# guangkun0818/speech2text

Measured on AMD Instinct MI355X. Metric: audio-seconds/sec (train step, zipformer pruned-RNN-T), higher is better.
Workload: dtype f32; 1 GPU; C3 zipformer pruned-RNN-T train step: chunk_size -1, 500 BPE, prune_range 5 (fbank+fwd+bwd+allreduce+ScaledAdam); accumulate_grad_batches=1, gemm_arith=bf16x2/3, per_gpu_batch=64, global_batch=64, labels_per_utt=50, parallelism=dp1

## Files before the change

### include/s2t_mi355.h

```cpp
#ifndef S2T_MI355_H_
#define S2T_MI355_H_

#ifdef __cplusplus
extern "C" {
#endif

int s2t_fbank_f32(const float* pcm, long pcm_stride, const long* num_samples, int batch,
                  const float* window400, const float* twiddle512, const int* mel_off,
                  const int* mel_k0, const float* mel_w, int nnz, int num_mel, float eps,
                  float scale_in, const float* cmvn_mean, const float* cmvn_istd, float* out,
                  int max_frames, long* out_frames, void* stream);

#define S2T_CTC_MAX_LABELS 1023
long s2t_ctc_workspace_floats(int B, int T, int Umax);
int s2t_ctc_loss_fwd_bwd(const float* logits, const long* targets, long tgt_stride,
                         const long* in_len, const long* tgt_len, int B, int T, int V, int Umax,
                         int blank, int zero_infinity, const float* grad_scale, float* workspace,
                         float* loss_per_utt, float* grad_logits, void* stream);

int s2t_fill_f32(float* p, long n, float v, void* stream);
int s2t_rnnt_row_exp(const float* x, long rows, int C, float* probs, float* rowmax, void* stream);
int s2t_rnnt_simple_pxpy(const float* am, const float* lm, const float* am_max,
                         const float* lm_max, const float* nrm, const long* symbols,
                         const long* boundary, int B, int S, int T, int C, int blank, float* px,
                         float* py, void* stream);
int s2t_rnnt_simple_w(const float* dpx, const float* dpy, const float* nrm, const float* gscale,
                      int B, int S, int T, float* W, void* stream);
int s2t_rnnt_simple_bwd(const float* am_probs, const float* lm_probs, const float* G_am,
                        const float* G_lm, const float* dpx, const float* dpy,
                        const float* gscale, const long* symbols, int B, int S, int T, int C,
                        int blank, float* d_am, float* d_lm, int accumulate, void* stream);
#define S2T_RNNT_SMOOTH_LM_SLAB 64
#define S2T_RNNT_SMOOTH_AM_SLAB 32
#define S2T_RNNT_SMOOTH_MAX_C 2048
int s2t_rnnt_smooth_stats(const float* am_probs, const float* lm_probs, int B, int S, int T, int C,
                          float mu, float* lm_sum, float* u_part, float* u, float* log_u,
                          float* am_dot, void* stream);
int s2t_rnnt_smooth_pxpy(const float* am, const float* lm, const float* am_max,
                         const float* lm_max, const float* nrm, const float* lm_sum,
                         const float* am_dot, const float* log_u, const long* symbols,
                         const long* boundary, int B, int S, int T, int C, int blank, float lam,
                         float mu, float* px, float* py, void* stream);
int s2t_rnnt_smooth_bwd(const float* am_probs, const float* lm_probs, const float* G_am,
                        const float* G_lm, const float* dpx, const float* dpy,
                        const float* gscale, const long* symbols, const float* lm_sum,
                        const float* am_dot, const float* u, int B, int S, int T, int C, int blank,
                        float lam, float mu, float* dlogu_part, float* v, float* d_am, float* d_lm,
                        void* stream);
#define S2T_RNNT_REGULAR 0
#define S2T_RNNT_MODIFIED 1
#define S2T_RNNT_CONSTRAINED 2
int s2t_mutual_info_fwd(const float* px, const float* py, const long* boundary, int B, int S,
                        int T, int rnnt_type, float* p, float* ans, void* stream);
int s2t_mutual_info_bwd(const float* px, const float* py, const long* boundary, const float* p,
                        const float* ans_grad, int B, int S, int T, int rnnt_type, float* px_grad,
                        float* py_grad, void* stream);
int s2t_rnnt_prune_ranges(const float* px_grad, const float* py_grad, const long* boundary, int B,
                          int S, int T, int s_range, long* ranges, void* stream);
int s2t_rnnt_pruned_fwd(const float* am, const float* lm, const long* ranges,
                        const long* symbols, const long* boundary, int B, int S, int T, int C,
                        int R, int blank, int act, int rnnt_type, float delay_penalty, float* px,
                        float* py, float* lse, void* stream);
int s2t_rnnt_pruned_bwd(const float* am, const float* lm, const long* ranges,
                        const long* symbols, const float* lse, const float* dpx, const float* dpy,
                        const float* gscale, int B, int S, int T, int C, int R, int blank, int act,
                        int rnnt_type, float* d_am, float* d_lm, int accumulate, void* stream);
int s2t_rnnt_lattice_fwd(const float* logits, const long* ranges, const long* symbols,
                         const long* boundary, int B, int S, int T, int V, int R, int blank,
                         int rnnt_type, float delay_penalty, float* px, float* py, float* lse,
                         void* stream);
int s2t_rnnt_lattice_bwd(const float* logits, const long* ranges, const long* symbols,
                         const float* lse, const float* dpx, const float* dpy,
                         const float* gscale, int B, int S, int T, int V, int R, int blank,
                         int rnnt_type, float* d_logits, void* stream);


int s2t_swoosh_fwd(const float* x, float* y, long n, float offset, float constant, void* stream);
int s2t_swoosh_bwd(const float* x, const float* g, float* d, long n, float offset, void* stream);
int s2t_biasnorm_fwd(const float* x, const float* bias, const float* log_scale, long rows, int D,
                     float* y, float* scales, void* stream);
int s2t_biasnorm_fwd_tb(const float* x, const float* bias, const float* log_scale, int T, int B, int D,
                        float* y, float* scales, void* stream);
int s2t_biasnorm_bwd_tb(const float* x, const float* bias, const float* scales, const float* g, int T,
                        int B, int D, float* dx, float* dbias, float* dls, void* stream);
int s2t_norm_bypass_fwd(const float* x, const float* bias, const float* log_scale, const float* orig,
                        const float* bypass_scale, const float* fm, int B, long rows, int D, float* out,
                        float* scales, void* stream);
int s2t_norm_bypass_bwd(const float* x, const float* bias, const float* scales, const float* orig,
                        const float* bypass_scale, const float* g, const float* fm, int B, long rows, int D,
                        float* dx, float* d_orig, float* d_bypass_scale, float* dbias, float* dls,
                        void* stream);
int s2t_biasnorm_bwd(const float* x, const float* bias, const float* scales, const float* g,
                     long rows, int D, float* dx, float* dbias, float* dls, void* stream);
long s2t_balancer_bwd_workspace_floats(void);
int s2t_balancer_bwd(const float* x, long ldx, const float* g, long ldg, long rows, int C,
                     float min_mean, float max_mean, float min_rms, float max_rms,
                     float grad_scale, float* out, long ldo, float* workspace, int parity,
                     float act_off, void* stream);
int s2t_balancer_stats(const float* x, long ldx, long rows, int C, float* stats, void* stream);
int s2t_balancer_apply(const float* x, long ldx, const float* g, long ldg, long rows, int C,
                       float min_mean, float max_mean, float min_rms, float max_rms,
                       float grad_scale, float* out, long ldo, const float* stats, float act_off,
                       void* stream);


int s2t_zipconv_fwd(const float* u, long ld, int gate_off, const unsigned char* mask, int T, int B,
                    int C, int K, int chunk, const float* wc, const float* bc, const float* wk,
                    const float* bk, const float* scale, float* y, void* stream);
int s2t_zipconv_fwd_act(const float* u, long ld, int gate_off, const unsigned char* mask, int T, int B,
                        int C, int K, int chunk, const float* wc, const float* bc, const float* wk,
                        const float* bk, const float* scale, float* y, float* y_act, int act_kind,
                        void* stream);
int s2t_zipconv_bwd(const float* u, long ld, int gate_off, const unsigned char* mask, int T, int B,
                    int C, int K, int chunk, const float* wc, const float* wk, const float* bk,
                    const float* scale, const float* dy, float* du, float* dwc, float* dbc,
                    float* dwk, float* dbk, float* dscale, float* workspace, void* stream);
int s2t_zipconv_bwd_data(const float* u, long ld, int gate_off, const unsigned char* mask, int T,
                         int B, int C, int K, int chunk, const float* wc, const float* wk,
                         const float* bk, const float* scale, const float* dy, float* du,
                         void* stream);
int s2t_zipconv_bwd_params(const float* u, long ld, int gate_off, const unsigned char* mask, int T,
                           int B, int C, int K, int chunk, const float* wc, const float* wk,
                           const float* bk, const float* scale, const float* dy, float* dwc,
                           float* dbc, float* dwk, float* dbk, float* dscale, float* workspace,
                           void* stream);
long s2t_zipconv_bwd_workspace_floats(int T, int B, int C, int K);


int s2t_relpos_attn_fwd(const float* qkp, const float* pos, const unsigned char* kpm,
                        const unsigned char* amask, int T, int B, int H, int qd, int pd, float* W,
                        void* stream);
int s2t_relpos_attn_fwd_flag(const float* qkp, const float* pos, const unsigned char* kpm,
                             const unsigned char* amask, int T, int B, int H, int qd, int pd,
                             float* W, float pen_limit, float* pen_flag, void* stream);
int s2t_relpos_attn_bwd(const float* qkp, const float* pos, const unsigned char* kpm,
                        const unsigned char* amask, int T, int B, int H, int qd, int pd,
                        const float* W, const float* dW, const float* dW0, const float* dO1,
                        const float* V1, int dv1, const float* dO2, const float* V2, int dv2,
                        int delta_given, float* delta_ws, float* dqkp, float* dpos,
                        float* workspace, void* stream);
long s2t_relpos_attn_bwd_workspace_floats(int T, int B, int H, int pd);
int s2t_attn_apply(const float* W, const float* v, int T, int B, int H, int dv, int transpose,
                   float* out, void* stream);


long s2t_linear_wgrad_workspace_floats(int R, int N, int M);
int s2t_linear_wgrad(const float* g, long ldg, const float* a, long lda, int R, int N, int M,
                     float* dW, float* db, int accumulate, float* workspace, void* stream);

int s2t_whiten_metric(float* xtx, float* colsum, long n, int G, int cg, float* cov, float* mean,
                      float* scal, float* host_metric, float* workspace, void* stream);
int s2t_whiten_prep(const float* cov, const float* mean, const float* scal, int G, int cg, float* dcov,
                    float* bias, float* sums64, void* stream);
int s2t_gemm_x3p_sq(const float* A, long lda, const unsigned short* Bp, int N, int K, float* C, long ldc,
                    int M, const float* bias, const float* other, long ld_other, float* sums, int tile,
                    void* stream);
int s2t_sumsq64(const float* g, long numel, float* sums64, void* stream);
int s2t_whiten_combine64(const float* g, const float* pg, long numel, float grad_scale,
                         const float* sums64, float* out, void* stream);
int s2t_whiten_dcov(const float* cov, const float* mean, const float* scal, int G, int cg,
                    float* dcov, float* bias, float* sums, void* stream);
int s2t_whiten_apply(const float* g, const float* pg, long numel, float grad_scale, float* sums,
                     float* out, void* stream);
int s2t_limit_param_grad(const float* x, const float* g, float lo, float hi, long n, float* out,
                         void* stream);

int s2t_bestrq_labels(const float* feats, int B, int T, int F, const float* proj, int D,
                      const float* codebooks, int ncb, int K, int T2, long* labels, void* stream);


int s2t_col2im3x3_nhwc(const float* dc, int B, int H, int W, int C, int Ho, int Wo, int sh, int sw,
                       float* dx, void* stream);

int s2t_conv3x3_c1(int mode, const float* x, const float* w, const float* bias, const float* g, int B,
                   int H, int W, int pw, int CO, float* y, float* dw, float* db, float* dx,
                   void* stream);

int s2t_conv3x3_s2(int mode, const float* x, const float* w, const float* bias, const float* g, int B,
                   int H, int W, int CI, int CO, float* y, float* dx, void* stream);

int s2t_conv3x3_gemm(int mode, const float* x, int B, int H, int W, int C, int sh, int sw, int CO,
                     const float* w2_or_g, const float* bias, float* out, float* db, void* stream);

int s2t_dwconv2d_nhwc_fwd(const float* x, const float* wgt, const float* bias, int N, int H, int W,
                          int C, int KH, int KW, int flip, float* y, void* stream);
int s2t_dwconv2d_nhwc_fwd_add(const float* x, const float* wgt, const float* bias, const float* add,
                              int N, int H, int W, int C, int KH, int KW, int flip, float* y,
                              void* stream);
long s2t_dwconv2d_wgrad_workspace_floats(int N, int H, int C, int KH, int KW);
int s2t_dwconv2d_nhwc_wgrad(const float* x, const float* dy, int N, int H, int W, int C, int KH,
                            int KW, float* workspace, float* dw, float* db, void* stream);

int s2t_optim_chunk_elems(void);
int s2t_optim_segc_floats(void);
int s2t_seg_stats(const float* p, const float* g, const int* chunk_off, const int* chunk_len,
                  int nchunks, float* partial, void* stream);
int s2t_scaled_adam_coef(const float* partial, const int* seg_chunk_begin, const int* seg_len,
                         int nchunks_all, int seg_lo, int seg_hi, float lr, float beta1,
                         float beta2, float eps, float scalar_lr_scale, float param_min_rms,
                         float param_max_rms, float scalar_max, float clip_val,
                         float clipping_scale, int step, int size_update_period,
                         int clipping_update_period, float bc2, float bc2_size, float beta2c,
                         float* param_rms, float* scale_exp_avg_sq, float* scale_grads,
                         float* model_norms, float* fstate, int* istate, float* segstat,
                         float* segc, const float* skip, void* stream);
int s2t_scaled_adam_apply(float* p, float* g, float* delta, float* exp_avg_sq,
                          const int* chunk_off, const int* chunk_len, const int* chunk_seg,
                          int nchunks, const float* segc, int zero_grad, void* stream);

int s2t_gemm_f32(int mode, const float* A, long lda, const float* B, long ldb, float* C, long ldc,
                 int M, int N, int K, const float* bias, const float* resid, long ldr,
                 const float* act_src, long lds, int act_kind, int pro_a, int pro_b, float* colsum,
                 int accumulate, void* stream);

int s2t_gemm_f32_batched(int mode, const float* A, long lda, long sA, const float* B, long ldb, long sB,
                         float* C, long ldc, long sC, int M, int N, int K, int batch, void* stream);

int s2t_gemm_f32_sq(int mode, const float* A, long lda, const float* B, long ldb, float* C, long ldc,
                    int M, int N, int K, const float* bias, const float* other, long ld_other,
                    float* sums, void* stream);
int s2t_whiten_combine(const float* g, const float* pg, long numel, float grad_scale, const float* sums,
                       float* out, void* stream);

int s2t_gemm_f32_tiled(int mode, const float* A, long lda, const float* B, long ldb, float* C,
                       long ldc, int M, int N, int K, const float* bias, const float* resid,
                       long ldr, int tile, void* stream);

int s2t_tn_x3(int set);
int s2t_tn_w(int set);
int s2t_nn_x3(int set);

int s2t_gemm_xtx(const float* x, long ldx, int R, int C, int cg, float* xtx, long ldc,
                 float* colsum, void* stream);

typedef struct S2tTnProblem {
  const float* A;
  long lda;
  const float* B;
  long ldb;
  float* C;
  long ldc;
  int M, N, K;
  float* colsum;
  float alpha;
// ... 16 lines not shown
                              long* tokens, long* out_len, void* stream);

long s2t_rnnt_beam_workspace_bytes(int B, int T, int V, int beam_size);
int s2t_rnnt_beam_stateless(const float* am, const long* lengths, const float* emb,
                            const float* conv_w, const float* lin_w, const float* lin_b,
                            const float* pre_w, const float* pre_b, int B, int T, int V, int E,
                            int D, int ctx, int act, int blank, int beam_size, int cutoff_top_k,
                            void* workspace, long* tokens, long* frames, long* out_len,
                            float* score, void* stream);

long s2t_rnnt_stream_state_bytes(int B, int V, int ctx, int beam_size, int max_tokens);
int s2t_rnnt_stream_reset(void* state, const int* rows, int B, int V, int ctx, int beam_size,
                          int max_tokens, int blank, void* stream);
int s2t_rnnt_greedy_stateless_chunk(const float* am, const long* chunk_len, const float* emb,
                                    const float* conv_w, const float* lin_w, const float* lin_b,
                                    const float* pre_w, const float* pre_b, int B, int Tc, int V,
                                    int E, int D, int ctx, int act, int max_token_step,
                                    int max_tokens, int blank, void* state, long* tokens,
                                    long* out_len, int* overflow, void* stream);
int s2t_rnnt_beam_stateless_chunk(const float* am, const long* chunk_len, const float* emb,
                                  const float* conv_w, const float* lin_w, const float* lin_b,
                                  const float* pre_w, const float* pre_b, int B, int Tc, int V, int E,
                                  int D, int ctx, int act, int blank, int beam_size,
                                  int cutoff_top_k, int max_tokens, void* state, long* tokens,
                                  long* frames, long* out_len, float* score, long* stable_len,
                                  int* overflow, void* stream);

#define S2T_RNNT_LSTM_MAX_HIDDEN 1024
#define S2T_RNNT_LSTM_MAX_LAYERS 8
#define S2T_RNNT_LSTM_MAX_VOCAB 8192
#define S2T_RNNT_LSTM_MAX_BEAM 16
typedef struct S2tLstmLayer {
  const float* x2g_w;
  const float* x2g_b;
  const float* p2g_w;
  const float *g_gamma, *g_beta;
  const float *c_gamma, *c_beta;
} S2tLstmLayer;
typedef struct S2tRnntLstmDesc {
  int V, E, H, D, inner, num_layers, layer_norm, act;
  float in_eps, lstm_eps, out_eps;
  int pad_;
  const float* emb;
  const float *in_gamma, *in_beta;
  S2tLstmLayer layers[S2T_RNNT_LSTM_MAX_LAYERS];
  const float *lin_w, *lin_b;
  const float *out_gamma, *out_beta;
  const float *pre_w, *pre_b;
  const float *out1_w, *out1_b;
  const float *out2_w, *out2_b;
} S2tRnntLstmDesc;
long s2t_rnnt_lstm_workspace_bytes(const S2tRnntLstmDesc* desc, int B, int T, int beam_size);
int s2t_lstm_pred_step(const S2tRnntLstmDesc* desc, int R, const int* tokens, const int* emit,
                       const int* parent, const float* h_in, const float* c_in, const float* lm_in,
                       float* h_out, float* c_out, float* lm_out, void* workspace, void* stream);
int s2t_rnnt_greedy_lstm(const S2tRnntLstmDesc* desc, const float* am, const long* lengths, int B,
                         int T, int max_token_step, void* workspace, long* tokens, long* out_len,
                         void* stream);
int s2t_rnnt_beam_lstm(const S2tRnntLstmDesc* desc, const float* am, const long* lengths, int B,
                       int T, int beam_size, int cutoff_top_k, void* workspace, long* tokens,
                       long* frames, long* out_len, float* score, void* stream);

typedef struct S2tRnnLmDesc {
  int V, E, H, num_layers;
  const float* emb;
  S2tLstmLayer layers[S2T_RNNT_LSTM_MAX_LAYERS];
  const float *out_w, *out_b;
} S2tRnnLmDesc;
long s2t_rnn_lm_step_workspace_bytes(const S2tRnnLmDesc* lm, int R);
int s2t_rnn_lm_step(const S2tRnnLmDesc* lm, int R, const int* tokens, const int* emit,
                    const int* parent, const float* h_in, const float* c_in, const float* q_in,
                    float* h_out, float* c_out, float* q_out, void* workspace, void* stream);
long s2t_rnnt_beam_lstm_lm_workspace_bytes(const S2tRnntLstmDesc* desc, const S2tRnnLmDesc* lm, int B,
                                           int T, int beam_size);
int s2t_rnnt_beam_lstm_lm(const S2tRnntLstmDesc* desc, const S2tRnnLmDesc* lm, const float* am,
                          const long* lengths, int B, int T, int beam_size, int cutoff_top_k,
                          float lm_weight, int lm_start_token, void* workspace, long* tokens,
                          long* frames, long* out_len, float* score, float* lm_score, void* stream);

long s2t_rnnt_lstm_stream_state_bytes(const S2tRnntLstmDesc* desc, int B, int beam_size,
                                      int max_tokens);
long s2t_rnnt_lstm_stream_workspace_bytes(const S2tRnntLstmDesc* desc, int B, int Tc, int beam_size);
int s2t_rnnt_lstm_stream_reset(const S2tRnntLstmDesc* desc, void* state, const int* rows, int B,
                               int beam_size, int max_tokens, void* workspace, void* stream);
int s2t_rnnt_greedy_lstm_chunk(const S2tRnntLstmDesc* desc, const float* am, const long* chunk_len,
                               int B, int Tc, int max_token_step, int max_tokens, int host_poll,
                               void* state, void* workspace, long* tokens, long* out_len,
                               int* overflow, void* stream);
int s2t_rnnt_beam_lstm_chunk(const S2tRnntLstmDesc* desc, const float* am, const long* chunk_len,
                             int B, int Tc, int beam_size, int cutoff_top_k, int max_tokens,
                             void* state, void* workspace, long* tokens, long* frames,
                             long* out_len, float* score, long* stable_len, int* overflow,
                             void* stream);

int s2t_row_energy(const float* x, long stride, const long* len, int B, int D, int mode, float* out,
                   void* stream);
int s2t_mix(const float* src, long sstride, const long* slen, const float* noise, long nstride,
            const long* nlen, const long* start, const float* snr, const float* src_e,
            const float* noise_e, int B, long rows_max, int D, int mode, float max_gain_db,
            float* out, void* stream);
int s2t_specaug(float* feats, int B, int T, int F, const int* tspan, int nt, const int* fspan,
                int nf, void* stream);
int s2t_pad_rows(const float* packed, const long* offsets, int B, long Lmax, int D, float* out,
                 void* stream);

int s2t_linear_lt(int mode, const float* X, long ldx, const float* W, long ldw, const float* bias,
                  const float* C, long ldc, float beta, float* D, long ldd, int M, int N, int K,
                  void* workspace, long ws_bytes, void* stream);
int s2t_linear_lt_stats(int* plans, int* timed);
long s2t_linear_lt_own_calls(void);

int s2t_bypass_fwd(const float* orig, const float* src, const float* scale, long rows, int C,
                   float* out, void* stream);
int s2t_bypass_bwd(const float* orig, const float* src, const float* scale, const float* g,
                   long rows, int C, float* d_orig, float* d_src, float* d_scale, void* stream);
int s2t_bypass_bwd_acc(const float* orig, const float* src, const float* scale, const float* g,
                       const float* acc_in, long rows, int C, float* d_orig, float* d_src,
                       float* d_scale, void* stream);
int s2t_attn_delta_pairs(const float* W, const float* dW0, const float* dO1, const float* O1,
                         int dv1, const float* dO2, const float* O2, int dv2, int T, int B, int H,
                         float* delta, void* stream);
int s2t_bypass_fwd_mask(const float* orig, const float* src, const float* scale, const float* fm,
                        int B, long rows, int C, float* out, void* stream);
int s2t_bypass_bwd_mask(const float* orig, const float* src, const float* scale, const float* g,
                        const float* fm, int B, long rows, int C, float* d_orig, float* d_src,
                        float* d_scale, void* stream);
int s2t_downsample_fwd(const float* src, const float* w, int ds, int T, int B, int C, float* out,
                       void* stream);
int s2t_downsample_bwd(const float* src, const float* w, const float* g, int ds, int T, int B, int C,
                       float* d_src, float* dw, void* stream);
int s2t_downsample_fwd_bt(const float* src, const float* w, int ds, int T, int B, int C, float* out,
                          void* stream);
int s2t_downsample_bwd_bt(const float* src, const float* w, const float* g, int ds, int T, int B, int C,
                          float* d_src, float* dw, void* stream);
int s2t_bypass_up_fwd(const float* orig, const float* src, const float* scale, int up, int T, int B,
                      int C, float* out, void* stream);
int s2t_bypass_up_bwd(const float* orig, const float* src, const float* scale, const float* g, int up,
                      int T, int B, int C, float* d_orig, float* d_src, float* d_scale, void* stream);
typedef struct S2tCommit {
  const float* x;
  float* d;
  float* grad;
  float lo, hi;
  int limit;
  long n;
} S2tCommit;
int s2t_param_grad_commit_n(int n, const S2tCommit* items, void* stream);
int s2t_nonlin_gate_fwd(const float* u, int T, int B, int C, float* xs, void* stream);
int s2t_nonlin_out_fwd(const float* z, const float* u, int T, int B, int C, float* o, void* stream);
int s2t_nonlin_out_bwd(const float* g, const float* z, const float* u, int T, int B, int C, float* dz,
                       float* du, void* stream);
int s2t_nonlin_gate_bwd(const float* dxs, const float* u, int T, int B, int C, float* du,
                        void* stream);

int s2t_layernorm_fwd(const float* x, const float* y, float alpha, const float* gamma,
                      const float* beta, long rows, int C, float eps, float* xsum, float* out,
                      float* stats, void* stream);
typedef struct S2tLnFold {
  const float* partial;
  long rows;
  float* dgamma;
  float* dbeta;
} S2tLnFold;
long s2t_layernorm_bwd_partial_floats(long rows, int C);
int s2t_layernorm_bwd(const float* x, const float* stats, const float* gamma, const float* dy,
                      const float* resid, long rows, int C, float* dx, float* partial,
                      void* stream);
int s2t_layernorm_param_grad(int n, const S2tLnFold* items, int C, void* stream);
int s2t_silu_fwd(const float* h, long n, float* a, void* stream);
int s2t_silu_bwd(const float* h, const float* da, long n, float scale, float* dh, void* stream);
int s2t_dropout_add(const float* x, const float* y, long n, float alpha, float p,
                    unsigned long long seed, float* out, void* stream);
int s2t_silu_drop_fwd(const float* h, long n, float p, unsigned long long seed, float* a,
                      void* stream);
int s2t_silu_drop_bwd(const float* h, const float* da, long n, float scale, float p,
                      unsigned long long seed, float* dh, void* stream);
#define S2T_BN_PARTIALS 128
long s2t_bn_workspace_floats(int C);
int s2t_bn_silu_fwd(const float* x, const float* gamma, const float* beta, float eps,
                    float momentum, float* running_mean, float* running_var, long* num_batches,
                    long rows, int C, float* y, float* save_mean, float* save_rstd,
                    float* workspace, void* stream);
int s2t_bn_silu_apply(const float* x, const float* mean, const float* rstd, const float* gamma,
                      const float* beta, long rows, int C, float* y, void* stream);
int s2t_bn_silu_bwd(const float* x, const float* ds, const float* save_mean,
                    const float* save_rstd, const float* gamma, const float* beta, long rows, int C,
                    float* dx, float* dgamma, float* dbeta, float* workspace, void* stream);
int s2t_mhsa_fwd(const float* qkv, long ld, int qoff, int koff, int voff, const long* lens, int T,
                 int B, int H, int dh, float scale, float dropout_p, unsigned long seed, float* o,
                 long ldo, float* lse, void* stream);
int s2t_mhsa_bwd(const float* qkv, long ld, int qoff, int koff, int voff, const long* lens, int T,
                 int B, int H, int dh, float scale, float dropout_p, unsigned long seed,
                 const float* o, const float* d_o, long ldo, const float* lse, float* delta,
                 float* dqkv, void* stream);

long s2t_conv1_relu_workspace_floats(int C);
int s2t_conv1_relu_fwd(const float* x, const float* w, const float* bias, int B, int T, int F,
                       int C, float* out, void* stream);
int s2t_conv1_relu_wgrad(const float* x, const float* w, const float* bias, const float* d_out,
                         int B, int T, int F, int C, float* dw, float* db, float* workspace,
                         void* stream);

#define S2T_ADAM_MAX_GROUPS 8
typedef struct S2tAdamGroup {
  int chunk_hi;
  float lr, beta1, beta2, eps, weight_decay;
  float bias_correction1;
  float sqrt_bias_correction2;
  int decoupled;
} S2tAdamGroup;
int s2t_clip_coef(const float* partial, int nchunks, float clip_val, float* out, void* stream);
int s2t_adam_apply(float* p, float* g, float* exp_avg, float* exp_avg_sq, const int* chunk_off,
                   const int* chunk_len, int nchunks, int ngroups, const S2tAdamGroup* groups,
                   const float* coef, int zero_grad, const float* skip, void* stream);

int s2t_lnlstm_fwd(const float* gx, const float* wp_t, const float* g_gamma, const float* g_beta,
                   const float* c_gamma, const float* c_beta, const float* h0, const float* c0,
                   int T, int B, int H, float eps, float* hs, float* ghat, float* chat,
                   float* rstd, float* hT, float* cT, void* stream);
int s2t_lnlstm_bwd(const float* wp, const float* g_gamma, const float* g_beta,
                   const float* c_gamma, const float* c_beta, const float* c0, int T, int B, int H,
                   const float* ghat, const float* chat, const float* rstd, const float* dhs,
                   float* dgx, float* d_g_gamma, float* d_g_beta, float* d_c_gamma,
                   float* d_c_beta, void* stream);

int s2t_lstm_seq_fwd(const float* gx, const float* whh, const float* h0, const float* c0, int T,
                     int B, int H, float* hs, float* gates, float* cells, float* hT, float* cT,
                     void* stream);
int s2t_lstm_seq_bwd(const float* whh_t, const float* c0, int T, int B, int H, const float* gates,
                     const float* cells, const float* dhs, float* dgx, float* dc_ws, void* stream);

int s2t_predictor_ctx_fwd(const int* tokens, const float* emb, const float* w, int B, int L, int K,
                          int D, int V, float* out, void* stream);
int s2t_predictor_ctx_bwd(const int* tokens, const float* emb, const float* w, const float* g, int B,
                          int L, int K, int D, int V, float* d_emb, float* d_w, void* stream);

int s2t_gemm_arith(void);
int s2t_gemm_arith_of(int cls);
int s2t_gemm_class_set(int cls);
int s2t_gemm_arith_set(int arith);
typedef struct {
  long src_off;
  long dst_off;
  int N, K, ld, transposed;
  unsigned blk_begin;
  int pad_;
} S2tPlaneDesc;
long s2t_x3p_plane_elems(int N, int K);
long s2t_x3p_split_blocks(int N, int K);
int s2t_x3p_split(const float* base, const void* tab, int n, int total_blocks, unsigned short* dst,
                  void* stream);
int s2t_gemm_x3p(const float* A, long lda, const unsigned short* Bp, int N, int K, float* C, long ldc,
                 int M, const float* bias, const float* resid, long ldr, const float* act_src,
                 long ld_act, int act_kind, float* C2, long ldc2, int act2, const float* resid_b,
                 long ldrb, int tile, void* stream);
#define S2T_X3P_BAL_COEF_READY (1 << 20)
int s2t_balancer_coef(float* bal_stats, int N, long rows, float min_mean, float max_mean, float min_rms,
                      float max_rms, float grad_scale, void* stream);
int s2t_gemm_x3p_bal(const float* A, long lda, const unsigned short* Bp, int N, int K, float* C, long ldc,
                     int M, const float* resid, long ldr, const float* act_src, long ld_act, int act_kind,
                     int tile, float* bal_stats, float min_mean, float max_mean, float min_rms,
                     float max_rms, float grad_scale, void* stream);

typedef struct S2tRowMap {
  int hw, w;
  long sb, sh, sw, base;
} S2tRowMap;
int s2t_gemm_x3p_map(const float* A, const S2tRowMap* amap, int seg, int nseg, const long* segoff,
                     const unsigned short* Bp, int N, float* C, long ldc, const S2tRowMap* cmap,
                     long c_elems, int M, const float* bias, int tile, void* stream);

void* s2t_side_stream(void);
int s2t_stream_order(void* from, void* to);

int s2t_x3p_sample_begin(int every);
int s2t_x3p_sample_end(long* launches, double* total_ms, double* bytes, double* flops);
int s2t_x3p_sample_min_bytes(double* bytes_min);
long s2t_gemm_x3p_calls(void);
long s2t_linear_lt_calls(void);
int s2t_prof_pair_create(void** start, void** stop);
int s2t_prof_pair_arm(void* start, void* stop);
int s2t_prof_pair_consumed(void);
int s2t_prof_pair_ms(void* start, void* stop, float* ms);
int s2t_prof_pair_destroy(void* start, void* stop);


int s2t_add_f32(const float* a, const float* b, float* out, long n, void* stream);
int s2t_balancer_next_parity(void);

int s2t_bmm_lt(int mode, const float* A, const float* B, float* C, int batch, int M, int N, int K,
               void* workspace, long ws_bytes, void* stream);

#define S2T_ZL_NDEC 32
#define S2T_ZL_NWHITEN 11
typedef struct S2tZlLin {
  const float* w;
  const float* b;
  float* gw;
  float* gb;
  const unsigned short* pf;
  const unsigned short* pb;
  int N, K;
} S2tZlLin;
typedef struct S2tZlBal {
  float min_mean, max_mean, min_rms, max_rms, grad_scale;
} S2tZlBal;
// ... 104 lines not shown
```

### speech2text_amd/csrc/common.h

```cpp
#pragma once
#include <hip/hip_runtime.h>
#include <stdint.h>

extern thread_local hipEvent_t s2t_prof_start, s2t_prof_stop;

#include <stdio.h>
#include <stdlib.h>
#include <string.h>
static inline int s2t_debug_env(const char* name) {
  const char* e = getenv(name);
  if (!e || atoi(e) == 0) return 0;
  const char* gate = getenv("S2T_DEBUG_KERNELS");
  if (gate && strcmp(gate, "1") == 0) return atoi(e);
  fprintf(stderr, "[s2t] %s=%s ignored: ablation switches need S2T_DEBUG_KERNELS=1\n", name, e);
  return 0;
}

#define S2T_GEMM_ARITH_DEFAULT 2
#define S2T_GEMM_ARITH_DEFAULT_F 2
#define S2T_GEMM_ARITH_DEFAULT_D 2
#define S2T_GEMM_ARITH_DEFAULT_W 2
#define S2T_GEMM_ARITH_DEFAULT_S 3
extern "C" int s2t_gemm_arith(void);
extern "C" int s2t_gemm_arith_of(int cls);
extern "C" int s2t_gemm_class_set(int cls);
struct S2tGemmClass {
  int prev;
  explicit S2tGemmClass(int cls) : prev(s2t_gemm_class_set(cls)) {}
  ~S2tGemmClass() { s2t_gemm_class_set(prev); }
};

#define S2T_WAVE 64
#define S2T_NEG_INF (-__builtin_huge_valf())

#define S2T_CHECK_LAUNCH()                         \
  do {                                             \
    hipError_t e__ = hipGetLastError();            \
    if (e__ != hipSuccess) return (int)e__;        \
  } while (0)

__device__ __forceinline__ float wave_sum(float v) {
#pragma unroll
  for (int o = 32; o > 0; o >>= 1) v += __shfl_xor(v, o, 64);
  return v;
}
__device__ __forceinline__ float wave_max(float v) {
#pragma unroll
  for (int o = 32; o > 0; o >>= 1) v = fmaxf(v, __shfl_xor(v, o, 64));
  return v;
}
__device__ __forceinline__ double wave_sum_d(double v) {
#pragma unroll
  for (int o = 32; o > 0; o >>= 1) v += __shfl_xor(v, o, 64);
  return v;
}

__device__ __forceinline__ float log_add(float a, float b) {
  float m = fmaxf(a, b);
  if (m == S2T_NEG_INF) return S2T_NEG_INF;
  float d = fminf(a, b) - m;
  return m + log1pf(__expf(d));
}
__device__ __forceinline__ float log_add_precise(float a, float b) {
  float m = fmaxf(a, b);
  if (m == S2T_NEG_INF) return S2T_NEG_INF;
  float d = fminf(a, b) - m;
  return m + log1pf(expf(d));
}

__device__ __forceinline__ float log_add_comp(float a, float b) {
  const float m = fmaxf(a, b);
  if (m == S2T_NEG_INF) return S2T_NEG_INF;
  const float e = __expf(fminf(a, b) - m);
  const float u = 1.f + e;
  return m + (u == 1.f ? e : __logf(u) * __fdividef(e, u - 1.f));
}

__device__ __forceinline__ float block_sum(float v, float* scratch) {
  v = wave_sum(v);
  const int w = threadIdx.x >> 6, l = threadIdx.x & 63, nw = (blockDim.x + 63) >> 6;
  __syncthreads();
  if (l == 0) scratch[w] = v;
  __syncthreads();
  float r = 0.f;
  for (int i = 0; i < nw; ++i) r += scratch[i];
  return r;
}
__device__ __forceinline__ float block_max(float v, float* scratch) {
  v = wave_max(v);
  const int w = threadIdx.x >> 6, l = threadIdx.x & 63, nw = (blockDim.x + 63) >> 6;
  __syncthreads();
  if (l == 0) scratch[w] = v;
  __syncthreads();
  float r = S2T_NEG_INF;
  for (int i = 0; i < nw; ++i) r = fmaxf(r, scratch[i]);
  return r;
}
```

### speech2text_amd/csrc/gemm_x3p.hip

```cpp
#include "common.h"
#include "../../include/s2t_mi355.h"
#include <hip/hip_ext.h>
#include <algorithm>
#include <cstdint>
#include <cstdlib>
#include <utility>
#include <vector>

namespace {

typedef float f32x16 __attribute__((ext_vector_type(16)));
typedef float f32x2 __attribute__((ext_vector_type(2)));
typedef __bf16 bf16x2 __attribute__((ext_vector_type(2)));
typedef __bf16 bf16x8 __attribute__((ext_vector_type(8)));
typedef float f32x4 __attribute__((ext_vector_type(4)));
typedef unsigned u32x4 __attribute__((ext_vector_type(4)));
typedef const __attribute__((address_space(1))) float* gf32p;
typedef const __attribute__((address_space(1))) f32x4* gf32x4p;
typedef const __attribute__((address_space(1))) u32x4* gu32x4p;

__device__ __forceinline__ void split_pair(float x0, float x1, unsigned& p0, unsigned& p1,
                                           unsigned& p2) {
  f32x2 x = {x0, x1};
  p0 = __builtin_bit_cast(unsigned, __builtin_convertvector(x, bf16x2));
  f32x2 h = {__uint_as_float(p0 << 16), __uint_as_float(p0 & 0xFFFF0000u)};
  x = x - h;
  p1 = __builtin_bit_cast(unsigned, __builtin_convertvector(x, bf16x2));
  f32x2 h1 = {__uint_as_float(p1 << 16), __uint_as_float(p1 & 0xFFFF0000u)};
  x = x - h1;
  p2 = __builtin_bit_cast(unsigned, __builtin_convertvector(x, bf16x2));
}
__device__ __forceinline__ void split8(const f32x4 v0, const f32x4 v1, u32x4& q0, u32x4& q1,
                                       u32x4& q2) {
  unsigned a0, a1, a2, b0, b1, b2, c0, c1, c2, d0, d1, d2;
  split_pair(v0.x, v0.y, a0, a1, a2);
  split_pair(v0.z, v0.w, b0, b1, b2);
  split_pair(v1.x, v1.y, c0, c1, c2);
  split_pair(v1.z, v1.w, d0, d1, d2);
  q0 = u32x4{a0, b0, c0, d0};
  q1 = u32x4{a1, b1, c1, d1};
  q2 = u32x4{a2, b2, c2, d2};
}

__device__ __forceinline__ void split_pair2(float x0, float x1, unsigned& p0, unsigned& p1) {
  f32x2 x = {x0, x1};
  p0 = __builtin_bit_cast(unsigned, __builtin_convertvector(x, bf16x2));
  f32x2 h = {__uint_as_float(p0 << 16), __uint_as_float(p0 & 0xFFFF0000u)};
  x = x - h;
  p1 = __builtin_bit_cast(unsigned, __builtin_convertvector(x, bf16x2));
}
template <int NP>
__device__ __forceinline__ void split8n(const f32x4 v0, const f32x4 v1, u32x4 (&q)[3]) {
  if (NP == 3) {
    split8(v0, v1, q[0], q[1], q[2]);
  } else {
    unsigned a0, a1, b0, b1, c0, c1, d0, d1;
    split_pair2(v0.x, v0.y, a0, a1);
    split_pair2(v0.z, v0.w, b0, b1);
    split_pair2(v1.x, v1.y, c0, c1);
    split_pair2(v1.z, v1.w, d0, d1);
    q[0] = u32x4{a0, b0, c0, d0};
    q[1] = u32x4{a1, b1, c1, d1};
  }
}

enum { ACT_NONE = 0, ACT_SWOOSH_L = 1, ACT_SWOOSH_R = 2 };

__device__ __forceinline__ float log1p_fast(float e) {
  const float u = 1.f + e;
  return u == 1.f ? e : __logf(u) * __fdividef(e, u - 1.f);
}
__device__ __forceinline__ float swoosh(float x, int kind) {
  const float off = kind == ACT_SWOOSH_L ? 4.f : 1.f;
  const float c = kind == ACT_SWOOSH_L ? 0.035f : 0.313261687f;
  const float z = x - off;
  return fmaxf(z, 0.f) + log1p_fast(__expf(-fabsf(z))) - 0.08f * x - c;
}
__device__ __forceinline__ float swoosh_deriv(float x, int kind) {
  const float off = kind == ACT_SWOOSH_L ? 4.f : 1.f;
  return __fdividef(1.f, 1.f + __expf(off - x)) - 0.08f;
}

struct X3PMap {
  int on, hw, w;
  long sb, sh, sw, base;
};
__device__ __forceinline__ long x3p_maprow(const X3PMap& m, int r) {
  const int b = r / m.hw, q = r - b * m.hw, i = q / m.w, j = q - i * m.w;
  return m.base + b * m.sb + i * m.sh + j * m.sw;
}

struct X3P {
  const float* A;
  long lda;
  const unsigned short* Bp;
  int NT, KB;
  float* C;
  long ldc;
  int M, N, K;
  const float* bias;
  const float* op[2];
  long ldop[2];
  int role[2];
  int act_kind;
  float* C2;
  long ldc2;
  int act2;
  int tiles_m, tiles_n;
  int wgs_per_cu;
  int prio;
  const float* bal_stats;
  float bal_n, bal_min_mean, bal_max_mean, bal_min_rms, bal_max_rms, bal_gs;
  float* sq_sums;
  float sq_pad_;
  X3PMap amap, cmap;
  int seg16, nseg;
  long segoff[4];
  long c_elems;
};

__device__ __forceinline__ void x3p_set_prio(int on) {
  if (!on) return;
  if (on == 2) { __builtin_amdgcn_s_setprio(3); return; }
  const unsigned tg = __builtin_amdgcn_s_getreg(((4 - 1) << 11) | (16 << 6) | 4) & 15u;
  if (tg == 0) __builtin_amdgcn_s_setprio(3);
  else if (tg == 1) __builtin_amdgcn_s_setprio(2);
  else if (tg == 2) __builtin_amdgcn_s_setprio(1);
}

struct EpiOps {
  f32x4 v[2][2];
};
struct EpiRs {
  __amdgpu_buffer_rsrc_t c, c2, op[2];
};
constexpr unsigned kOob = 0xFFFFFFF0u;

__device__ __forceinline__ __amdgpu_buffer_rsrc_t x3p_rsrc(const float* p, long ld, int rows) {
  return __builtin_amdgcn_make_buffer_rsrc(const_cast<float*>(p), 0,
                                           p ? (int)((long)rows * ld * 4) : 0, 0x00020000);
}
__device__ __forceinline__ EpiRs x3p_epi_rsrc(const X3P& g) {
  EpiRs r;
  r.c = x3p_rsrc(g.C, g.ldc, g.M);
  r.c2 = x3p_rsrc(g.C2, g.ldc2, g.M);
  r.op[0] = x3p_rsrc(g.op[0], g.ldop[0], g.M);
  r.op[1] = x3p_rsrc(g.op[1], g.ldop[1], g.M);
  return r;
}
__device__ __forceinline__ f32x4 x3p_bload(__amdgpu_buffer_rsrc_t rs, unsigned off) {
  return __builtin_bit_cast(f32x4, __builtin_amdgcn_raw_buffer_load_b128(rs, off, 0, 0));
}
__device__ __forceinline__ void x3p_bstore(__amdgpu_buffer_rsrc_t rs, unsigned off, f32x4 v) {
  __builtin_amdgcn_raw_buffer_store_b128(__builtin_bit_cast(u32x4, v), rs, off, 0, 0);
}

__device__ __forceinline__ f32x4 x3p_epi_bias(const X3P& g, int j, int n0, int wcb, int lane) {
  const int col = n0 + 32 * (wcb + j) + (lane & 7) * 4;
  f32x4 b = {0.f, 0.f, 0.f, 0.f};
  if (g.bias && col < g.N) b = *reinterpret_cast<const f32x4*>(g.bias + col);
  return b;
}

__device__ __forceinline__ void x3p_epi_load(const X3P& g, const EpiRs& rs, EpiOps& o, int i, int j,
                                             int h, int m0, int n0, int wrb, int wcb, int lane) {
  const int er = lane >> 3, ec = (lane & 7) * 4;
  const int col = n0 + 32 * (wcb + j) + ec;
  const f32x4 z = {0.f, 0.f, 0.f, 0.f};
#pragma unroll
  for (int q = 0; q < 2; ++q) {
    const int row = m0 + 32 * (wrb + i) + 16 * h + er + 8 * q;
    const bool ok = row < g.M && col < g.N;
#pragma unroll
    for (int k = 0; k < 2; ++k) {
      o.v[q][k] = z;
      if (g.role[k])
        o.v[q][k] = x3p_bload(rs.op[k], ok ? (unsigned)(row * (int)g.ldop[k] + col) * 4u : kOob);
    }
  }
}

struct BalQ {
  f32x4 a, b;
};
__device__ __forceinline__ BalQ x3p_epi_balcoef(const X3P& g, int j, int n0, int wcb, int lane) {
  BalQ r;
  r.a = r.b = f32x4{0.f, 0.f, 0.f, 0.f};
  const int col = n0 + 32 * (wcb + j) + (lane & 7) * 4;
  if (col >= g.N) return r;
  r.a = *reinterpret_cast<const f32x4*>(g.bal_stats + 2048 + col);
  r.b = *reinterpret_cast<const f32x4*>(g.bal_stats + 3072 + col);
  return r;
}

__global__ __launch_bounds__(256) void bal_coef_kernel(const float* __restrict__ stats, float* __restrict__ coef,
                                                        int N, float n, float min_mean, float max_mean,
                                                        float min_rms, float max_rms, float gs) {
  const int c = blockIdx.x * 256 + threadIdx.x;
  if (c >= N) return;
  const float inv_n = 1.f / n;
  const float mean = stats[c] * inv_n, uvar = stats[1024 + c] * inv_n;
  const float raw_var = uvar - mean * mean;
  const bool live_v = raw_var > 1.0e-20f, live_r = uvar > 1.0e-20f;
  const float var = fmaxf(raw_var, 1.0e-20f);
  const float sd = sqrtf(var);
  const float rms = sqrtf(fmaxf(uvar, 1.0e-20f));
  const float m = mean / sd;
  const float mc = fminf(fmaxf(m, min_mean), max_mean);
  const float s_m = (m > mc) ? 1.f : ((m < mc) ? -1.f : 0.f);
  const float rc = fminf(fmaxf(rms, min_rms), max_rms);
  const float lq = logf(rc / rms);
  const float s_r = (lq > 0.f) ? -1.f : ((lq < 0.f) ? 1.f : 0.f);
  const float a = s_m * inv_n * (live_v ? (1.f / sd + mean * mean / (sd * var)) : 1.f / sd);
  const float b = (live_v ? -s_m * inv_n * mean / (sd * var) : 0.f) + (live_r ? s_r * inv_n / (rms * rms) : 0.f);
  const float lg_rms = fmaxf(sqrtf(fmaxf(a * a + 2.f * a * b * mean + b * b * uvar, 0.f)), 1.0e-20f);
  const float k = gs / lg_rms;
  coef[c] = a * k;
  coef[1024 + c] = b * k;
}

template <bool BAL = false>
__device__ __forceinline__ void x3p_epi_xform(const X3P& g, f32x16& a, float* scr, const EpiOps& o,
                                              const f32x4 bq, int h, int lane, const BalQ& bal = BalQ{}) {
  const int hi = lane >> 5, lo = lane & 31;
  const int er = lane >> 3, ec = (lane & 7) * 4;
#pragma unroll
  for (int r = 0; r < 8; ++r) scr[((r & 3) + 8 * (r >> 2) + 4 * hi) * 36 + lo] = a[8 * h + r];
  __builtin_amdgcn_fence(__ATOMIC_RELEASE, "workgroup", "local");
  __builtin_amdgcn_wave_barrier();
#pragma unroll
  for (int q = 0; q < 2; ++q) {
    f32x4 v = *reinterpret_cast<const f32x4*>(scr + (er + 8 * q) * 36 + ec);
    v += bq;
#pragma unroll
    for (int k = 0; k < 2; ++k) {
      const f32x4 x = o.v[q][k];
      if (g.role[k] == 1) {
        v.x *= swoosh_deriv(x.x, g.act_kind);
        v.y *= swoosh_deriv(x.y, g.act_kind);
        v.z *= swoosh_deriv(x.z, g.act_kind);
        v.w *= swoosh_deriv(x.w, g.act_kind);
        if (BAL) {
          v.x += fabsf(v.x) * fmaf(bal.b.x, x.x, bal.a.x);
          v.y += fabsf(v.y) * fmaf(bal.b.y, x.y, bal.a.y);
          v.z += fabsf(v.z) * fmaf(bal.b.z, x.z, bal.a.z);
          v.w += fabsf(v.w) * fmaf(bal.b.w, x.w, bal.a.w);
        }
      } else if (g.role[k] == 2 || (g.role[k] == 3 && g.act2 != 3)) {
        v += x;
      }
    }
    a[8 * h + 4 * q + 0] = v.x;
    a[8 * h + 4 * q + 1] = v.y;
    a[8 * h + 4 * q + 2] = v.z;
    a[8 * h + 4 * q + 3] = v.w;
  }
  __builtin_amdgcn_fence(__ATOMIC_RELEASE, "workgroup", "local");
  __builtin_amdgcn_wave_barrier();
}

struct EpiSq {
  float o = 0.f, c = 0.f;
};
template <bool CMAP = false>
__device__ __forceinline__ void x3p_epi_store(const X3P& g, const EpiRs& rs, const f32x16& a,
                                              const EpiOps& o, int i, int j, int h, int m0, int n0,
                                              int wrb, int wcb, int lane, EpiSq& sq) {
  const int er = lane >> 3, ec = (lane & 7) * 4;
  const int col = n0 + 32 * (wcb + j) + ec;
#pragma unroll
  for (int q = 0; q < 2; ++q) {
    const int row = m0 + 32 * (wrb + i) + 16 * h + er + 8 * q;
    const bool ok = row < g.M && col < g.N;
    const f32x4 v = {a[8 * h + 4 * q], a[8 * h + 4 * q + 1], a[8 * h + 4 * q + 2], a[8 * h + 4 * q + 3]};
    if (CMAP) {
      x3p_bstore(rs.c, ok ? (unsigned)(x3p_maprow(g.cmap, min(row, g.M - 1)) + col) * 4u : kOob, v);
      continue;
    }
    x3p_bstore(rs.c, ok ? (unsigned)(row * (int)g.ldc + col) * 4u : kOob, v);
    if (g.sq_sums && ok) {
      sq.c += (v.x * v.x + v.y * v.y) + (v.z * v.z + v.w * v.w);
      const f32x4 t = g.role[0] == 4 ? o.v[q][0] : o.v[q][1];
      sq.o += (t.x * t.x + t.y * t.y) + (t.z * t.z + t.w * t.w);
    }
    if (g.act2 == 3) {
      const f32x4 u = v + (g.role[0] == 3 ? o.v[q][0] : o.v[q][1]);
      x3p_bstore(rs.c2, ok ? (unsigned)(row * (int)g.ldc2 + col) * 4u : kOob, u);
    } else if (g.act2) {
      const f32x4 u = {swoosh(v.x, g.act2), swoosh(v.y, g.act2), swoosh(v.z, g.act2), swoosh(v.w, g.act2)};
      x3p_bstore(rs.c2, ok ? (unsigned)(row * (int)g.ldc2 + col) * 4u : kOob, u);
    }
  }
}

template <int TM, int TN, bool LEAN = false, bool BAL = false, bool CMAP = false>
__device__ __forceinline__ void x3p_epilogue(const X3P& g, f32x16 (&acc)[TM][TN], unsigned char* smem,
                                             int m0, int n0, int wrb, int wcb, int wave, int lane,
                                             bool sync = true) {
  if (sync) __syncthreads();
  float* scr = reinterpret_cast<float*>(smem) + wave * (16 * 36);
  EpiRs rs = x3p_epi_rsrc(g);
  if (CMAP) rs.c = __builtin_amdgcn_make_buffer_rsrc(g.C, 0, (int)(g.c_elems * 4), 0x00020000);
  EpiSq sq;
  auto sq_commit = [&]() {
    if (!g.sq_sums) return;
    const float so = wave_sum(sq.o), sc = wave_sum(sq.c);
    if (lane == 0) {
      const int slot = (blockIdx.x * 4 + wave) & 63;
      atomicAdd(g.sq_sums + slot, so);
      atomicAdd(g.sq_sums + 64 + slot, sc);
    }
  };
  if (LEAN) {
#pragma unroll
    for (int j = 0; j < TN; ++j) {
      const f32x4 bqj = x3p_epi_bias(g, j, n0, wcb, lane);
      const BalQ balj = BAL ? x3p_epi_balcoef(g, j, n0, wcb, lane) : BalQ{};
#pragma unroll
      for (int i = 0; i < TM; ++i)
#pragma unroll
        for (int h = 0; h < 2; ++h) {
          EpiOps o;
          x3p_epi_load(g, rs, o, i, j, h, m0, n0, wrb, wcb, lane);
          x3p_epi_xform<BAL>(g, acc[i][j], scr, o, bqj, h, lane, balj);
          x3p_epi_store<CMAP>(g, rs, acc[i][j], o, i, j, h, m0, n0, wrb, wcb, lane, sq);
        }
    }
    sq_commit();
    return;
  }
  f32x4 bq[TN];
#pragma unroll
  for (int j = 0; j < TN; ++j) bq[j] = x3p_epi_bias(g, j, n0, wcb, lane);
#pragma unroll
  for (int i = 0; i < TM; ++i) {
    EpiOps ops[2 * TN];
#pragma unroll
    for (int t = 0; t < 2 * TN; ++t) x3p_epi_load(g, rs, ops[t], i, t / 2, t & 1, m0, n0, wrb, wcb, lane);
#pragma unroll
    for (int t = 0; t < 2 * TN; ++t) x3p_epi_xform(g, acc[i][t / 2], scr, ops[t], bq[t / 2], t & 1, lane);
#pragma unroll
    for (int t = 0; t < 2 * TN; ++t)
      x3p_epi_store(g, rs, acc[i][t / 2], ops[t], i, t / 2, t & 1, m0, n0, wrb, wcb, lane, sq);
    __builtin_amdgcn_sched_barrier(0);
  }
  sq_commit();
}

template <int TM, int TN, bool BAL = false, int NP = 3>
__global__ __launch_bounds__(256, TM * TN == 4 ? 2 : (TM * TN == 2 ? 3 : 4))
void x3p_db_kernel(X3P g) {
  constexpr int BM = 64 * TM, BN = 64 * TN;
  constexpr int A_ST = 2 * TM * NP * 1024, B_ST = 2 * TN * NP * 1024, ST = A_ST + B_ST;
  constexpr int NAU = (128 * TM + 255) / 256;
  constexpr int NBP = 2 * TN * NP * 64;
  constexpr int NBU = (NBP + 255) / 256;
  constexpr int SCR = 4 * 16 * 36 * 4;
  __shared__ __attribute__((aligned(1024))) unsigned char smem[2 * ST > SCR ? 2 * ST : SCR];

  const int total = g.tiles_m * g.tiles_n;
  const int per_xcd = (total + 7) / 8;
  const int xcd = blockIdx.x & 7, stride = gridDim.x >> 3;
  int loc = blockIdx.x >> 3;
  if (loc >= per_xcd || xcd * per_xcd + loc >= total) return;
  const int tid = threadIdx.x, lane = tid & 63, wave = tid >> 6;
  const int wrb = (wave >> 1) * TM, wcb = (wave & 1) * TN;
  x3p_set_prio(g.prio);

  int a_r[NAU], a_k[NAU];
  unsigned a_dst[NAU];
  bool a_on[NAU];
// ... 781 lines not shown
```

### speech2text_amd/csrc/zip_elem.hip

```cpp
#include "common.h"
#include <algorithm>
#include <stdlib.h>

namespace {

__device__ __forceinline__ float log1p_fast(float e) {
  const float u = 1.f + e;
  return u == 1.f ? e : __logf(u) * __fdividef(e, u - 1.f);
}

__device__ __forceinline__ float swoosh_f(float x, float off, float c) {
  const float z = x - off;
  return fmaxf(z, 0.f) + log1p_fast(__expf(-fabsf(z))) - 0.08f * x - c;
}
__device__ __forceinline__ float swoosh_d(float x, float off) {
  return __fdividef(1.f, 1.f + __expf(off - x)) - 0.08f;
}

__global__ __launch_bounds__(256) void swoosh_fwd_kernel(const float* __restrict__ x,
                                                         float* __restrict__ y, long n, float off,
                                                         float c) {
  const long n4 = n >> 2;
  const long stride = (long)gridDim.x * blockDim.x;
  const float4* x4 = reinterpret_cast<const float4*>(x);
  float4* y4 = reinterpret_cast<float4*>(y);
  for (long i = (long)blockIdx.x * blockDim.x + threadIdx.x; i < n4; i += stride) {
    float4 v = x4[i];
    v.x = swoosh_f(v.x, off, c);
    v.y = swoosh_f(v.y, off, c);
    v.z = swoosh_f(v.z, off, c);
    v.w = swoosh_f(v.w, off, c);
    y4[i] = v;
  }
  for (long i = (n4 << 2) + (long)blockIdx.x * blockDim.x + threadIdx.x; i < n; i += stride)
    y[i] = swoosh_f(x[i], off, c);
}

__global__ __launch_bounds__(256) void swoosh_bwd_kernel(const float* __restrict__ x,
                                                         const float* __restrict__ g,
                                                         float* __restrict__ d, long n,
                                                         float off) {
  const long n4 = n >> 2;
  const long stride = (long)gridDim.x * blockDim.x;
  const float4* x4 = reinterpret_cast<const float4*>(x);
  const float4* g4 = reinterpret_cast<const float4*>(g);
  float4* d4 = reinterpret_cast<float4*>(d);
  for (long i = (long)blockIdx.x * blockDim.x + threadIdx.x; i < n4; i += stride) {
    const float4 v = x4[i], gg = g4[i];
    float4 o;
    o.x = gg.x * swoosh_d(v.x, off);
    o.y = gg.y * swoosh_d(v.y, off);
    o.z = gg.z * swoosh_d(v.z, off);
    o.w = gg.w * swoosh_d(v.w, off);
    d4[i] = o;
  }
  for (long i = (n4 << 2) + (long)blockIdx.x * blockDim.x + threadIdx.x; i < n; i += stride)
    d[i] = g[i] * swoosh_d(x[i], off);
}

__global__ __launch_bounds__(256) void biasnorm_fwd_kernel(
    const float* __restrict__ x, const float* __restrict__ bias, const float* __restrict__ ls,
    long rows, int D, float* __restrict__ y, float* __restrict__ scales, int tbT, int tbB) {
  const long row = (long)blockIdx.x * 4 + (threadIdx.x >> 6);
  const int lane = threadIdx.x & 63;
  if (row >= rows) return;
  const float* xr = x + row * D;
  float acc = 0.f;
  for (int c = lane; c < D; c += 64) {
    const float d = xr[c] - bias[c];
    acc = fmaf(d, d, acc);
  }
  acc = wave_sum(acc);
  const float s = rsqrtf(acc / D) * expf(ls[0]);
  if (lane == 0) scales[row] = s;
  const long orow = tbT > 0 ? (row % tbT) * tbB + row / tbT : row;
  float* yr = y + orow * D;
  for (int c = lane; c < D; c += 64) yr[c] = xr[c] * s;
}

template <int CPL>
__global__ __launch_bounds__(256) void biasnorm_bwd_kernel(
    const float* __restrict__ x, const float* __restrict__ bias, const float* __restrict__ scales,
    const float* __restrict__ g, long rows, int D, float* __restrict__ dx,
    float* __restrict__ dbias, float* __restrict__ dls, int tbT, int tbB) {
  const int lane = threadIdx.x & 63;
  const long wave = (long)blockIdx.x * 4 + (threadIdx.x >> 6);
  const long nwaves = (long)gridDim.x * 4;
  float b[CPL], db[CPL];
#pragma unroll
  for (int j = 0; j < CPL; ++j) {
    const int c = lane + 64 * j;
    b[j] = c < D ? bias[c] : 0.f;
    db[j] = 0.f;
  }
  float dl = 0.f;
  for (long row = wave; row < rows; row += 2 * nwaves) {
    const long row2 = row + nwaves;
    const bool has2 = row2 < rows;
    const long rowb = has2 ? row2 : row;
    const float* xr = x + row * D;
    const float* gr = g + (tbT > 0 ? (row % tbT) * tbB + row / tbT : row) * D;
    const float* xr2 = x + rowb * D;
    const float* gr2 = g + (tbT > 0 ? (rowb % tbT) * tbB + rowb / tbT : rowb) * D;
    float xv[CPL], gv[CPL], xw[CPL], gw[CPL];
#pragma unroll
    for (int j = 0; j < CPL; ++j) {
      const int c = lane + 64 * j;
      xv[j] = c < D ? xr[c] : 0.f;
      gv[j] = c < D ? gr[c] : 0.f;
      xw[j] = c < D ? xr2[c] : 0.f;
      gw[j] = c < D ? gr2[c] : 0.f;
    }
    float A = 0.f, ss = 0.f, A2 = 0.f, ss2 = 0.f;
#pragma unroll
    for (int j = 0; j < CPL; ++j) {
      const int c = lane + 64 * j;
      A = fmaf(gv[j], xv[j], A);
      A2 = fmaf(gw[j], xw[j], A2);
      const float d = c < D ? xv[j] - b[j] : 0.f, d2 = c < D ? xw[j] - b[j] : 0.f;
      ss = fmaf(d, d, ss);
      ss2 = fmaf(d2, d2, ss2);
    }
    A = wave_sum(A);
    ss = wave_sum(ss);
    A2 = wave_sum(A2);
    ss2 = wave_sum(ss2);
    const float s = scales[row], s2 = has2 ? scales[row2] : 0.f;
    const float coef = s * A / ss, coef2 = has2 ? s2 * A2 / ss2 : 0.f;
    dl += A * s + (has2 ? A2 * s2 : 0.f);
    float* dr = dx + row * D;
    float* dr2 = dx + row2 * D;
#pragma unroll
    for (int j = 0; j < CPL; ++j) {
      const int c = lane + 64 * j;
      if (c < D) {
        const float t = coef * (xv[j] - b[j]);
        dr[c] = s * gv[j] - t;
        db[j] += t;
        if (has2) {
          const float t2 = coef2 * (xw[j] - b[j]);
          dr2[c] = s2 * gw[j] - t2;
          db[j] += t2;
        }
      }
    }
  }
  __shared__ float s_db[4][64 * CPL];
  __shared__ float s_dl[4];
  const int wv = threadIdx.x >> 6;
#pragma unroll
  for (int j = 0; j < CPL; ++j) s_db[wv][lane + 64 * j] = db[j];
  if (lane == 0) s_dl[wv] = dl;
  __syncthreads();
// ... 4 lines not shown
      const float t = (s_db[0][c] + s_db[1][c]) + (s_db[2][c] + s_db[3][c]);
      if (c < D && t != 0.f) atomicAdd(&dbias[c], t);
    }
    const float tl = (s_dl[0] + s_dl[1]) + (s_dl[2] + s_dl[3]);
    if (lane == 0 && tl != 0.f) atomicAdd(dls, tl);
  }
}

__device__ __forceinline__ float mul_rounded(float x, float y) {
#pragma clang fp contract(off)
  const float p = x * y;
  return p;
}

__global__ __launch_bounds__(256) void norm_bypass_fwd_kernel(
    const float* __restrict__ x, const float* __restrict__ bias, const float* __restrict__ ls,
    const float* __restrict__ orig, const float* __restrict__ bscale, const float* __restrict__ fm,
    int B, long rows, int D, float* __restrict__ out, float* __restrict__ scales) {
  const long row = (long)blockIdx.x * 4 + (threadIdx.x >> 6);
  const int lane = threadIdx.x & 63;
  if (row >= rows) return;
  const float* xr = x + row * D;
  float acc = 0.f;
  for (int c = lane; c < D; c += 64) {
    const float d = xr[c] - bias[c];
    acc = fmaf(d, d, acc);
  }
  acc = wave_sum(acc);
  const float s = rsqrtf(acc / D) * expf(ls[0]);
  if (lane == 0) scales[row] = s;
  const float* orow = orig + row * D;
  const float* mrow = fm ? fm + (row % B) * D : nullptr;
  float* yr = out + row * D;
  for (int c = lane; c < D; c += 64) {
    const float a = orow[c];
    float v = fmaf(mul_rounded(xr[c], s) - a, bscale[c], a);
    if (mrow) v *= mrow[c];
    yr[c] = v;
  }
}

template <int CPL>
__global__ __launch_bounds__(256) void norm_bypass_bwd_kernel(
    const float* __restrict__ x, const float* __restrict__ bias, const float* __restrict__ scales,
    const float* __restrict__ orig, const float* __restrict__ bscale, const float* __restrict__ g,
    const float* __restrict__ fm, int B, long rows, int D, float* __restrict__ dx,
    float* __restrict__ d_orig, float* __restrict__ d_bscale, float* __restrict__ dbias,
    float* __restrict__ dls) {
  const int lane = threadIdx.x & 63;
  const long wave = (long)blockIdx.x * 4 + (threadIdx.x >> 6);
  const long nwaves = (long)gridDim.x * 4;
  float b[CPL], k[CPL], db[CPL], dk[CPL];
#pragma unroll
  for (int j = 0; j < CPL; ++j) {
    const int c = lane + 64 * j;
    b[j] = c < D ? bias[c] : 0.f;
    k[j] = c < D ? bscale[c] : 0.f;
    db[j] = 0.f;
    dk[j] = 0.f;
  }
  float dl = 0.f;
  for (long row = wave; row < rows; row += 2 * nwaves) {
    const long row2 = row + nwaves;
    const bool has2 = row2 < rows;
    const long ra = row, rb = has2 ? row2 : row;
    float xv[CPL], gv[CPL], ov[CPL], xw[CPL], gw[CPL], ow[CPL];
#pragma unroll
    for (int j = 0; j < CPL; ++j) {
      const int c = lane + 64 * j;
      const bool ok = c < D;
      xv[j] = ok ? x[ra * D + c] : 0.f;
      gv[j] = ok ? g[ra * D + c] : 0.f;
      ov[j] = ok ? orig[ra * D + c] : 0.f;
      xw[j] = ok ? x[rb * D + c] : 0.f;
      gw[j] = ok ? g[rb * D + c] : 0.f;
      ow[j] = ok ? orig[rb * D + c] : 0.f;
      if (fm) {
        gv[j] *= ok ? fm[(ra % B) * D + c] : 0.f;
        gw[j] *= ok ? fm[(rb % B) * D + c] : 0.f;
      }
    }
    const float s = scales[ra], s2 = scales[rb];
    float A = 0.f, ss = 0.f, A2 = 0.f, ss2 = 0.f;
    float* d0 = d_orig + ra * D;
    float* d02 = d_orig + rb * D;
#pragma unroll
    for (int j = 0; j < CPL; ++j) {
      const int c = lane + 64 * j;
      if (c < D) {
        const float t = gv[j] * k[j];
        dk[j] = fmaf(gv[j], mul_rounded(xv[j], s) - ov[j], dk[j]);
        d0[c] = gv[j] - t;
        gv[j] = t;
        if (has2) {
          const float t2 = gw[j] * k[j];
          dk[j] = fmaf(gw[j], mul_rounded(xw[j], s2) - ow[j], dk[j]);
          d02[c] = gw[j] - t2;
          gw[j] = t2;
        }
      }
      A = fmaf(gv[j], xv[j], A);
      A2 = fmaf(gw[j], xw[j], A2);
      const float d = c < D ? xv[j] - b[j] : 0.f, d2 = c < D ? xw[j] - b[j] : 0.f;
      ss = fmaf(d, d, ss);
      ss2 = fmaf(d2, d2, ss2);
    }
    A = wave_sum(A);
    ss = wave_sum(ss);
    A2 = wave_sum(A2);
    ss2 = wave_sum(ss2);
    const float coef = s * A / ss, coef2 = has2 ? s2 * A2 / ss2 : 0.f;
    dl += A * s + (has2 ? A2 * s2 : 0.f);
    float* dr = dx + ra * D;
    float* dr2 = dx + rb * D;
#pragma unroll
    for (int j = 0; j < CPL; ++j) {
      const int c = lane + 64 * j;
      if (c < D) {
        const float t = coef * (xv[j] - b[j]);
        dr[c] = s * gv[j] - t;
        db[j] += t;
        if (has2) {
          const float t2 = coef2 * (xw[j] - b[j]);
          dr2[c] = s2 * gw[j] - t2;
          db[j] += t2;
        }
      }
    }
  }
  __shared__ float s_db[4][64 * CPL], s_dk[4][64 * CPL];
  __shared__ float s_dl[4];
  const int wv = threadIdx.x >> 6;
#pragma unroll
  for (int j = 0; j < CPL; ++j) {
    s_db[wv][lane + 64 * j] = db[j];
    s_dk[wv][lane + 64 * j] = dk[j];
  }
  if (lane == 0) s_dl[wv] = dl;
  __syncthreads();
  if (wv == 0) {
#pragma unroll
    for (int j = 0; j < CPL; ++j) {
      const int c = lane + 64 * j;
      const float t = (s_db[0][c] + s_db[1][c]) + (s_db[2][c] + s_db[3][c]);
      const float u = (s_dk[0][c] + s_dk[1][c]) + (s_dk[2][c] + s_dk[3][c]);
      if (c < D && t != 0.f) atomicAdd(&dbias[c], t);
      if (c < D && u != 0.f) atomicAdd(&d_bscale[c], u);
    }
    const float tl = (s_dl[0] + s_dl[1]) + (s_dl[2] + s_dl[3]);
    if (lane == 0 && tl != 0.f) atomicAdd(dls, tl);
  }
}

template <int Q, int RT>
__global__ __launch_bounds__(256) void norm_bypass_bwd16_kernel(
    const float* __restrict__ x, const float* __restrict__ bias, const float* __restrict__ scales,
    const float* __restrict__ orig, const float* __restrict__ bscale, const float* __restrict__ g,
    const float* __restrict__ fm, int B, long rows, int D, float* __restrict__ dx,
    float* __restrict__ d_orig, float* __restrict__ d_bscale, float* __restrict__ dbias,
    float* __restrict__ dls) {
  const int lane = threadIdx.x & 63, wv = threadIdx.x >> 6;
  const long wave = (long)blockIdx.x * 4 + wv;
  const long nwaves = (long)gridDim.x * 4;
  const int D4 = D >> 2;
  const float4 z4 = make_float4(0.f, 0.f, 0.f, 0.f);
  const float4* x4 = reinterpret_cast<const float4*>(x);
  const float4* g4 = reinterpret_cast<const float4*>(g);
  const float4* o4 = reinterpret_cast<const float4*>(orig);
  const float4* f4 = reinterpret_cast<const float4*>(fm);
  float4 b[Q], k[Q], db[Q], dk[Q];
#pragma unroll
  for (int q = 0; q < Q; ++q) {
    const int cq = lane + 64 * q;
    b[q] = cq < D4 ? reinterpret_cast<const float4*>(bias)[cq] : z4;
    k[q] = cq < D4 ? reinterpret_cast<const float4*>(bscale)[cq] : z4;
    db[q] = z4;
    dk[q] = z4;
  }
  float dl = 0.f;
  for (long r0 = wave; r0 < rows; r0 += RT * nwaves) {
    float4 xv[RT][Q], gv[RT][Q], ov[RT][Q];
    float sc[RT];
#pragma unroll
    for (int i = 0; i < RT; ++i) {
      const long row = r0 + i * nwaves;
      const long rr = row < rows ? row : r0;
      sc[i] = scales[rr];
#pragma unroll
      for (int q = 0; q < Q; ++q) {
        const int cq = lane + 64 * q;
        const bool ok = cq < D4;
        const long idx = rr * D4 + (ok ? cq : 0);
        xv[i][q] = x4[idx];
        gv[i][q] = g4[idx];
        ov[i][q] = o4[idx];
        if (fm) {
          const float4 m = f4[(rr % B) * D4 + (ok ? cq : 0)];
          gv[i][q].x *= m.x; gv[i][q].y *= m.y; gv[i][q].z *= m.z; gv[i][q].w *= m.w;
        }
        if (!ok) { xv[i][q] = z4; gv[i][q] = z4; ov[i][q] = z4; }
      }
    }
#pragma unroll
    for (int i = 0; i < RT; ++i) {
      const long row = r0 + i * nwaves;
      if (row >= rows) break;
      const float s = sc[i];
      float A = 0.f, ss = 0.f;
#pragma unroll
      for (int q = 0; q < Q; ++q) {
        const int cq = lane + 64 * q;
        float* xe = reinterpret_cast<float*>(&xv[i][q]);
        float* ge = reinterpret_cast<float*>(&gv[i][q]);
        const float* oe = reinterpret_cast<const float*>(&ov[i][q]);
        const float* ke = reinterpret_cast<const float*>(&k[q]);
        const float* be = reinterpret_cast<const float*>(&b[q]);
        float* dke = reinterpret_cast<float*>(&dk[q]);
        float4 d0;
        float* d0e = reinterpret_cast<float*>(&d0);
#pragma unroll
        for (int e = 0; e < 4; ++e) {
          const float t = mul_rounded(ge[e], ke[e]);
          dke[e] = fmaf(ge[e], mul_rounded(xe[e], s) - oe[e], dke[e]);
          d0e[e] = fmaf(-ge[e], ke[e], ge[e]);
          ge[e] = t;
          A = fmaf(t, xe[e], A);
          const float d = xe[e] - be[e];
          ss = fmaf(d, d, ss);
        }
        if (cq < D4) reinterpret_cast<float4*>(d_orig)[row * D4 + cq] = d0;
      }
      A = wave_sum(A);
      ss = wave_sum(ss);
      const float coef = s * A / ss;
      dl += A * s;
#pragma unroll
      for (int q = 0; q < Q; ++q) {
        const int cq = lane + 64 * q;
        const float* xe = reinterpret_cast<const float*>(&xv[i][q]);
        const float* ge = reinterpret_cast<const float*>(&gv[i][q]);
        const float* be = reinterpret_cast<const float*>(&b[q]);
        float* dbe = reinterpret_cast<float*>(&db[q]);
        float4 o;
        float* oe = reinterpret_cast<float*>(&o);
#pragma unroll
        for (int e = 0; e < 4; ++e) {
          const float t = coef * (xe[e] - be[e]);
          oe[e] = s * ge[e] - t;
          dbe[e] += t;
        }
        if (cq < D4) reinterpret_cast<float4*>(dx)[row * D4 + cq] = o;
      }
    }
  }
  __shared__ float4 s_db[4][64 * Q], s_dk[4][64 * Q];
  __shared__ float s_dl[4];
#pragma unroll
  for (int q = 0; q < Q; ++q) {
    s_db[wv][lane + 64 * q] = db[q];
    s_dk[wv][lane + 64 * q] = dk[q];
  }
  if (lane == 0) s_dl[wv] = dl;
  __syncthreads();
  for (int c = threadIdx.x; c < D; c += 256) {
    const float* p0 = reinterpret_cast<const float*>(&s_db[0][0]);
    const float* p1 = reinterpret_cast<const float*>(&s_dk[0][0]);
    const int W = 256 * Q;
    const float t = (p0[c] + p0[W + c]) + (p0[2 * W + c] + p0[3 * W + c]);
    const float u = (p1[c] + p1[W + c]) + (p1[2 * W + c] + p1[3 * W + c]);
    if (t != 0.f) atomicAdd(&dbias[c], t);
    if (u != 0.f) atomicAdd(&d_bscale[c], u);
  }
  if (threadIdx.x == 0) {
    const float tl = (s_dl[0] + s_dl[1]) + (s_dl[2] + s_dl[3]);
    if (tl != 0.f) atomicAdd(dls, tl);
  }
}

__global__ __launch_bounds__(256) void col_stats_kernel(const float* __restrict__ x, long rows,
                                                        int C, long ld, float* __restrict__ sum,
                                                        float* __restrict__ sumsq) {
  for (int c0 = blockIdx.y * 64; c0 < C; c0 += gridDim.y * 64) {
    const int c = c0 + threadIdx.x;
    float s = 0.f, q = 0.f;
    if (c < C) {
      const long step = (long)gridDim.x * 4;
      long r = (long)blockIdx.x * 4 + threadIdx.y;
      for (; r + 7 * step < rows; r += 8 * step) {
        float v[8];
#pragma unroll
        for (int u = 0; u < 8; ++u) v[u] = x[(r + u * step) * ld + c];
#pragma unroll
        for (int u = 0; u < 8; ++u) {
          s += v[u];
          q = fmaf(v[u], v[u], q);
        }
      }
      for (; r < rows; r += step) {
        const float v = x[r * ld + c];
        s += v;
        q = fmaf(v, v, q);
      }
    }
    __shared__ float sh[2][4][64];
    sh[0][threadIdx.y][threadIdx.x] = s;
    sh[1][threadIdx.y][threadIdx.x] = q;
    __syncthreads();
    if (threadIdx.y == 0 && c < C) {
      s = sh[0][0][threadIdx.x] + sh[0][1][threadIdx.x] + sh[0][2][threadIdx.x] +
          sh[0][3][threadIdx.x];
      q = sh[1][0][threadIdx.x] + sh[1][1][threadIdx.x] + sh[1][2][threadIdx.x] +
          sh[1][3][threadIdx.x];
      atomicAdd(&sum[c], s);
      atomicAdd(&sumsq[c], q);
    }
    __syncthreads();
  }
}

__global__ __launch_bounds__(256) void col_stats_small_kernel(const float* __restrict__ x, long nquads, int C,
                                                              float* __restrict__ sum,
                                                              float* __restrict__ sumsq) {
  const int cq = C >> 2;
  float4 s = make_float4(0.f, 0.f, 0.f, 0.f), q = s;
  const float4* x4 = reinterpret_cast<const float4*>(x);
  const long step = (long)gridDim.x * 256;
  long i = (long)blockIdx.x * 256 + threadIdx.x;
  for (; i + 3 * step < nquads; i += 4 * step) {
    float4 v[4];
#pragma unroll
    for (int u = 0; u < 4; ++u) v[u] = x4[i + u * step];
#pragma unroll
    for (int u = 0; u < 4; ++u) {
      s.x += v[u].x; s.y += v[u].y; s.z += v[u].z; s.w += v[u].w;
      q.x = fmaf(v[u].x, v[u].x, q.x); q.y = fmaf(v[u].y, v[u].y, q.y);
      q.z = fmaf(v[u].z, v[u].z, q.z); q.w = fmaf(v[u].w, v[u].w, q.w);
    }
  }
  for (; i < nquads; i += step) {
    const float4 v = x4[i];
    s.x += v.x; s.y += v.y; s.z += v.z; s.w += v.w;
    q.x = fmaf(v.x, v.x, q.x); q.y = fmaf(v.y, v.y, q.y); q.z = fmaf(v.z, v.z, q.z); q.w = fmaf(v.w, v.w, q.w);
  }
#pragma unroll
  for (int o = 32; o >= 1; o >>= 1) {
    if (o >= cq) {
      s.x += __shfl_xor(s.x, o, 64); s.y += __shfl_xor(s.y, o, 64);
      s.z += __shfl_xor(s.z, o, 64); s.w += __shfl_xor(s.w, o, 64);
      q.x += __shfl_xor(q.x, o, 64); q.y += __shfl_xor(q.y, o, 64);
      q.z += __shfl_xor(q.z, o, 64); q.w += __shfl_xor(q.w, o, 64);
    }
  }
  __shared__ float4 sh[2][4][8];
  const int lane = threadIdx.x & 63, wave = threadIdx.x >> 6;
  if (lane < cq) {
    sh[0][wave][lane] = s;
    sh[1][wave][lane] = q;
  }
  __syncthreads();
  if (threadIdx.x < C) {
    const int c = threadIdx.x;
    const float* f0 = reinterpret_cast<const float*>(&sh[0][0][0]);
    const float* f1 = reinterpret_cast<const float*>(&sh[1][0][0]);
    atomicAdd(&sum[c], (f0[c] + f0[32 + c]) + (f0[64 + c] + f0[96 + c]));
    atomicAdd(&sumsq[c], (f1[c] + f1[32 + c]) + (f1[64 + c] + f1[96 + c]));
  }
}

__global__ __launch_bounds__(256) void balancer_apply_small_kernel(
    const float* __restrict__ x, const float* __restrict__ g, const float* __restrict__ stats,
    float* __restrict__ stats_next, float n, float min_mean, float max_mean, float min_rms, float max_rms,
    float grad_scale, long nquads, int C, float* __restrict__ out, float act_off) {
  __shared__ __attribute__((aligned(16))) float s_a[32], s_b[32];
  const float inv_n = 1.f / n;
  if (threadIdx.x < C) {
    const int c = threadIdx.x;
    const float mean = stats[c] * inv_n, uvar = stats[1024 + c] * inv_n;
    const float raw_var = uvar - mean * mean;
    const bool live_v = raw_var > 1.0e-20f, live_r = uvar > 1.0e-20f;
    const float var = fmaxf(raw_var, 1.0e-20f);
    const float sd = sqrtf(var);
    const float rms = sqrtf(fmaxf(uvar, 1.0e-20f));
    const float m = mean / sd;
    const float mc = fminf(fmaxf(m, min_mean), max_mean);
    const float s_m = (m > mc) ? 1.f : ((m < mc) ? -1.f : 0.f);
    const float rc = fminf(fmaxf(rms, min_rms), max_rms);
    const float lq = logf(rc / rms);
    const float s_r = (lq > 0.f) ? -1.f : ((lq < 0.f) ? 1.f : 0.f);
    const float a = s_m * inv_n * (live_v ? (1.f / sd + mean * mean / (sd * var)) : 1.f / sd);
    const float b = (live_v ? -s_m * inv_n * mean / (sd * var) : 0.f) +
                    (live_r ? s_r * inv_n / (rms * rms) : 0.f);
    const float lg_rms =
        fmaxf(sqrtf(fmaxf(a * a + 2.f * a * b * mean + b * b * uvar, 0.f)), 1.0e-20f);
    const float coef = grad_scale / lg_rms;
    s_a[c] = a * coef;
    s_b[c] = b * coef;
  }
  if (blockIdx.x == 0 && stats_next != nullptr)
    for (int c = threadIdx.x; c < 2 * 1024; c += 256) stats_next[c] = 0.f;
  __syncthreads();
  const int cq = C >> 2;
  const float4 a4 = *reinterpret_cast<const float4*>(&s_a[4 * (threadIdx.x & (cq - 1))]);
  const float4 b4 = *reinterpret_cast<const float4*>(&s_b[4 * (threadIdx.x & (cq - 1))]);
  const float4* x4 = reinterpret_cast<const float4*>(x);
  const float4* g4 = reinterpret_cast<const float4*>(g);
  float4* o4 = reinterpret_cast<float4*>(out);
  const long step = (long)gridDim.x * 256;
  for (long i = (long)blockIdx.x * 256 + threadIdx.x; i < nquads; i += 2 * step) {
    const bool two = i + step < nquads;
    float4 xv[2], gv[2];
    xv[0] = x4[i];
    gv[0] = g4[i];
    xv[1] = x4[two ? i + step : i];
    gv[1] = g4[two ? i + step : i];
#pragma unroll
    for (int u = 0; u < 2; ++u) {
      if (u == 1 && !two) break;
      float4 gg = gv[u];
      if (act_off >= 0.f) {
        gg.x *= swoosh_d(xv[u].x, act_off);
        gg.y *= swoosh_d(xv[u].y, act_off);
        gg.z *= swoosh_d(xv[u].z, act_off);
        gg.w *= swoosh_d(xv[u].w, act_off);
      }
      o4[i + u * step] = make_float4(gg.x + fabsf(gg.x) * fmaf(b4.x, xv[u].x, a4.x),
                                     gg.y + fabsf(gg.y) * fmaf(b4.y, xv[u].y, a4.y),
                                     gg.z + fabsf(gg.z) * fmaf(b4.z, xv[u].z, a4.z),
                                     gg.w + fabsf(gg.w) * fmaf(b4.w, xv[u].w, a4.w));
    }
  }
}

__global__ __launch_bounds__(256) void balancer_apply_fused_kernel(
    const float* __restrict__ x, long ldx, const float* __restrict__ g, long ldg,
    const float* __restrict__ stats, float* __restrict__ stats_next, float n, float min_mean,
    float max_mean, float min_rms, float max_rms, float grad_scale, long rows, int C,
    float* __restrict__ out, long ldo, float act_off) {
  __shared__ float s_a[1024], s_b[1024];
  const float inv_n = 1.f / n;
  for (int c = threadIdx.x; c < C; c += 256) {
    const float mean = stats[c] * inv_n, uvar = stats[1024 + c] * inv_n;
    const float raw_var = uvar - mean * mean;
    const bool live_v = raw_var > 1.0e-20f, live_r = uvar > 1.0e-20f;
    const float var = fmaxf(raw_var, 1.0e-20f);
    const float sd = sqrtf(var);
    const float rms = sqrtf(fmaxf(uvar, 1.0e-20f));
    const float m = mean / sd;
    const float mc = fminf(fmaxf(m, min_mean), max_mean);
    const float s_m = (m > mc) ? 1.f : ((m < mc) ? -1.f : 0.f);
    const float rc = fminf(fmaxf(rms, min_rms), max_rms);
    const float lq = logf(rc / rms);
    const float s_r = (lq > 0.f) ? -1.f : ((lq < 0.f) ? 1.f : 0.f);
    const float a = s_m * inv_n * (live_v ? (1.f / sd + mean * mean / (sd * var)) : 1.f / sd);
    const float b = (live_v ? -s_m * inv_n * mean / (sd * var) : 0.f) +
                    (live_r ? s_r * inv_n / (rms * rms) : 0.f);
    const float lg_rms =
        fmaxf(sqrtf(fmaxf(a * a + 2.f * a * b * mean + b * b * uvar, 0.f)), 1.0e-20f);
    const float coef = grad_scale / lg_rms;
    s_a[c] = a * coef;
    s_b[c] = b * coef;
  }
  if (blockIdx.x == 0 && stats_next != nullptr)
    for (int c = threadIdx.x; c < 2 * 1024; c += 256) stats_next[c] = 0.f;
  __syncthreads();
  const int tx = threadIdx.x & 63, ty = threadIdx.x >> 6;
  const long step = (long)gridDim.x * 4;
  for (int c0 = 0; c0 < C; c0 += 64) {
    const int c = c0 + tx;
    if (c >= C) continue;
    const float a = s_a[c], b = s_b[c];
    long r = (long)blockIdx.x * 4 + ty;
    for (; r + 3 * step < rows; r += 4 * step) {
      float gv[4], xv[4];
#pragma unroll
      for (int u = 0; u < 4; ++u) {
        gv[u] = g[(r + u * step) * ldg + c];
        xv[u] = x[(r + u * step) * ldx + c];
      }
#pragma unroll
      for (int u = 0; u < 4; ++u) {
        if (act_off >= 0.f) gv[u] *= swoosh_d(xv[u], act_off);
        out[(r + u * step) * ldo + c] = gv[u] + fabsf(gv[u]) * fmaf(b, xv[u], a);
      }
    }
    for (; r < rows; r += step) {
      const float xs = x[r * ldx + c];
      float gv = g[r * ldg + c];
      if (act_off >= 0.f) gv *= swoosh_d(xs, act_off);
      out[r * ldo + c] = gv + fabsf(gv) * fmaf(b, xs, a);
    }
  }
}

inline unsigned grid_for(long n, int per_block) {
  long b = (n + per_block - 1) / per_block;
  if (b > 256 * 16) b = 256 * 16;
  if (b < 1) b = 1;
  return (unsigned)b;
}

}

extern "C" int s2t_swoosh_fwd(const float* x, float* y, long n, float offset, float constant,
                              void* stream) {
  if (n <= 0) return 0;
  hipLaunchKernelGGL(swoosh_fwd_kernel, dim3(grid_for(n, 1024)), dim3(256), 0,
                     (hipStream_t)stream, x, y, n, offset, constant);
  S2T_CHECK_LAUNCH();
  return 0;
}

namespace {
__global__ __launch_bounds__(256) void add_kernel(const float* a, const float* b, float* out, long n) {
  const long n4 = n >> 2;
  const long stride = (long)gridDim.x * blockDim.x;
  const float4* a4 = reinterpret_cast<const float4*>(a);
  const float4* b4 = reinterpret_cast<const float4*>(b);
  float4* o4 = reinterpret_cast<float4*>(out);
  for (long i = (long)blockIdx.x * blockDim.x + threadIdx.x; i < n4; i += stride) {
    const float4 u = a4[i], v = b4[i];
    o4[i] = make_float4(u.x + v.x, u.y + v.y, u.z + v.z, u.w + v.w);
  }
  for (long i = (n4 << 2) + (long)blockIdx.x * blockDim.x + threadIdx.x; i < n; i += stride)
    out[i] = a[i] + b[i];
}
}

extern "C" int s2t_add_f32(const float* a, const float* b, float* out, long n, void* stream) {
  if (n <= 0) return 0;
  if (!a || !b || !out || ((reinterpret_cast<uintptr_t>(a) | reinterpret_cast<uintptr_t>(b) |
                            reinterpret_cast<uintptr_t>(out)) & 15))
    return -1;
  hipLaunchKernelGGL(add_kernel, dim3(grid_for(n, 1024)), dim3(256), 0, (hipStream_t)stream, a, b,
                     out, n);
  S2T_CHECK_LAUNCH();
  return 0;
}

static int g_bal_parity = 0;
extern "C" int s2t_balancer_next_parity(void) {
  g_bal_parity ^= 1;
  return g_bal_parity;
}

extern "C" int s2t_swoosh_bwd(const float* x, const float* g, float* d, long n, float offset,
                              void* stream) {
  if (n <= 0) return 0;
  hipLaunchKernelGGL(swoosh_bwd_kernel, dim3(grid_for(n, 1024)), dim3(256), 0,
                     (hipStream_t)stream, x, g, d, n, offset);
  S2T_CHECK_LAUNCH();
  return 0;
}

extern "C" int s2t_biasnorm_fwd(const float* x, const float* bias, const float* log_scale,
                                long rows, int D, float* y, float* scales, void* stream) {
  if (rows <= 0) return 0;
  hipLaunchKernelGGL(biasnorm_fwd_kernel, dim3((unsigned)((rows + 3) / 4)), dim3(256), 0,
                     (hipStream_t)stream, x, bias, log_scale, rows, D, y, scales, 0, 0);
  S2T_CHECK_LAUNCH();
  return 0;
}

extern "C" int s2t_biasnorm_fwd_tb(const float* x, const float* bias, const float* log_scale, int T,
                                   int B, int D, float* y, float* scales, void* stream) {
  if (T <= 0 || B <= 0) return 0;
  const long rows = (long)T * B;
  hipLaunchKernelGGL(biasnorm_fwd_kernel, dim3((unsigned)((rows + 3) / 4)), dim3(256), 0,
                     (hipStream_t)stream, x, bias, log_scale, rows, D, y, scales, T, B);
  S2T_CHECK_LAUNCH();
  return 0;
}

extern "C" int s2t_norm_bypass_fwd(const float* x, const float* bias, const float* log_scale,
                                   const float* orig, const float* bypass_scale, const float* fm, int B,
                                   long rows, int D, float* out, float* scales, void* stream) {
  if (rows <= 0) return 0;
  if (D <= 0 || B <= 0) return -1;
  hipLaunchKernelGGL(norm_bypass_fwd_kernel, dim3((unsigned)((rows + 3) / 4)), dim3(256), 0,
                     (hipStream_t)stream, x, bias, log_scale, orig, bypass_scale, fm, B, rows, D, out, scales);
  S2T_CHECK_LAUNCH();
  return 0;
}

extern "C" int s2t_norm_bypass_bwd(const float* x, const float* bias, const float* scales,
                                   const float* orig, const float* bypass_scale, const float* g,
                                   const float* fm, int B, long rows, int D, float* dx, float* d_orig,
                                   float* d_bypass_scale, float* dbias, float* dls, void* stream) {
  if (rows <= 0) return 0;
  if (D <= 0 || D > 1024 || B <= 0) return -1;
  hipStream_t st = (hipStream_t)stream;
  const uintptr_t al = reinterpret_cast<uintptr_t>(x) | reinterpret_cast<uintptr_t>(bias) |
                       reinterpret_cast<uintptr_t>(orig) | reinterpret_cast<uintptr_t>(bypass_scale) |
                       reinterpret_cast<uintptr_t>(g) | reinterpret_cast<uintptr_t>(fm) |
                       reinterpret_cast<uintptr_t>(dx) | reinterpret_cast<uintptr_t>(d_orig);
  if ((D & 3) == 0 && (al & 15) == 0) {
    constexpr unsigned cap16 = 512u;
    const unsigned nb16 = std::min(grid_for(rows, 4 * (rows >= 8192 ? 16 : 8)), cap16);
#define NB_BWD16(Q, RT)                                                                                  \
  hipLaunchKernelGGL((norm_bypass_bwd16_kernel<Q, RT>), dim3(nb16), dim3(256), 0, st, x, bias, scales,   \
                     orig, bypass_scale, g, fm, B, rows, D, dx, d_orig, d_bypass_scale, dbias, dls)
    if (D <= 256) NB_BWD16(1, 4);
    else if (D <= 512) NB_BWD16(2, 2);
    else NB_BWD16(4, 1);
#undef NB_BWD16
    S2T_CHECK_LAUNCH();
    return 0;
  }
  const unsigned nb = std::min(grid_for(rows, 4 * 8), 1024u);
#define NB_BWD(CPL)                                                                                    \
  hipLaunchKernelGGL(norm_bypass_bwd_kernel<CPL>, dim3(nb), dim3(256), 0, st, x, bias, scales, orig,   \
                     bypass_scale, g, fm, B, rows, D, dx, d_orig, d_bypass_scale, dbias, dls)
  if (D <= 64) NB_BWD(1);
  else if (D <= 128) NB_BWD(2);
  else if (D <= 256) NB_BWD(4);
  else if (D <= 512) NB_BWD(8);
  else NB_BWD(16);
#undef NB_BWD
  S2T_CHECK_LAUNCH();
  return 0;
}

static int biasnorm_bwd_launch(const float* x, const float* bias, const float* scales, const float* g,
                               long rows, int D, float* dx, float* dbias, float* dls, int tbT, int tbB,
                               hipStream_t st) {
  const unsigned nb = std::min(grid_for(rows, 4 * 8), 1024u);
#define BN_BWD(CPL)                                                                                  \
  hipLaunchKernelGGL(biasnorm_bwd_kernel<CPL>, dim3(nb), dim3(256), 0, st, x, bias, scales, g, rows, \
                     D, dx, dbias, dls, tbT, tbB)
  if (D <= 64) BN_BWD(1);
  else if (D <= 128) BN_BWD(2);
  else if (D <= 256) BN_BWD(4);
  else if (D <= 512) BN_BWD(8);
  else if (D <= 1024) BN_BWD(16);
  else return -1;
#undef BN_BWD
  S2T_CHECK_LAUNCH();
  return 0;
}

extern "C" int s2t_biasnorm_bwd(const float* x, const float* bias, const float* scales,
                                const float* g, long rows, int D, float* dx, float* dbias,
                                float* dls, void* stream) {
  if (rows <= 0) return 0;
  return biasnorm_bwd_launch(x, bias, scales, g, rows, D, dx, dbias, dls, 0, 0, (hipStream_t)stream);
}

extern "C" int s2t_biasnorm_bwd_tb(const float* x, const float* bias, const float* scales, const float* g,
                                   int T, int B, int D, float* dx, float* dbias, float* dls, void* stream) {
  if (T <= 0 || B <= 0) return 0;
  return biasnorm_bwd_launch(x, bias, scales, g, (long)T * B, D, dx, dbias, dls, T, B, (hipStream_t)stream);
}

static bool bal_small(int C, const float* x, long ldx, const float* g, long ldg, const float* out, long ldo) {
  auto al = [](const void* p) { return (reinterpret_cast<uintptr_t>(p) & 15) == 0; };
  return (C == 4 || C == 8 || C == 16 || C == 32) && ldx == C && al(x) && (!g || (ldg == C && al(g))) &&
         (!out || (ldo == C && al(out)));
}
static unsigned bal_small_grid(long nquads) {
  return (unsigned)std::min<long>(2048, std::max<long>(1, (nquads + 256 * 8 - 1) / (256 * 8)));
}

constexpr int BAL_MAXC = 1024;
extern "C" long s2t_balancer_bwd_workspace_floats(void) { return 4L * BAL_MAXC; }

extern "C" int s2t_balancer_bwd(const float* x, long ldx, const float* g, long ldg, long rows,
                                int C, float min_mean, float max_mean, float min_rms,
                                float max_rms, float grad_scale, float* out, long ldo,
                                float* workspace, int parity, float act_off, void* stream) {
  if (rows <= 0 || C <= 0) return 0;
  if (C > BAL_MAXC || !workspace) return -1;
  hipStream_t st = (hipStream_t)stream;
  float* cur = workspace + (parity & 1) * 2 * BAL_MAXC;
  float* nxt = workspace + ((parity + 1) & 1) * 2 * BAL_MAXC;
  if (bal_small(C, x, ldx, g, ldg, out, ldo)) {
    const long nq = rows * C / 4;
    hipLaunchKernelGGL(col_stats_small_kernel, dim3(bal_small_grid(nq)), dim3(256), 0, st, x, nq, C, cur,
                       cur + BAL_MAXC);
    S2T_CHECK_LAUNCH();
    hipLaunchKernelGGL(balancer_apply_small_kernel, dim3(bal_small_grid(nq)), dim3(256), 0, st, x, g, cur, nxt,
                       (float)rows, min_mean, max_mean, min_rms, max_rms, grad_scale, nq, C, out, act_off);
    S2T_CHECK_LAUNCH();
    return 0;
  }
  int gy = (C + 63) / 64;
  if (gy > 16) gy = 16;
  long gx = (rows + 4 * 16 - 1) / (4 * 16);
  gx = gx > 256 ? 256 : (gx < 1 ? 1 : gx);
  hipLaunchKernelGGL(col_stats_kernel, dim3((unsigned)gx, gy), dim3(64, 4), 0, st, x, rows, C, ldx,
                     cur, cur + BAL_MAXC);
  S2T_CHECK_LAUNCH();
  hipLaunchKernelGGL(balancer_apply_fused_kernel, dim3((unsigned)std::min<long>((rows + 15) / 16, 2048)), dim3(256), 0, st,
                     x, ldx, g, ldg, cur, nxt, (float)rows, min_mean, max_mean, min_rms, max_rms,
                     grad_scale, rows, C, out, ldo, act_off);
  S2T_CHECK_LAUNCH();
  return 0;
}

extern "C" int s2t_balancer_stats(const float* x, long ldx, long rows, int C, float* stats,
                                  void* stream) {
  if (rows <= 0 || C <= 0) return 0;
  if (C > BAL_MAXC || !stats) return -1;
  if (bal_small(C, x, ldx, nullptr, 0, nullptr, 0)) {
    const long nq = rows * C / 4;
    hipLaunchKernelGGL(col_stats_small_kernel, dim3(bal_small_grid(nq)), dim3(256), 0, (hipStream_t)stream, x,
                       nq, C, stats, stats + BAL_MAXC);
    S2T_CHECK_LAUNCH();
    return 0;
  }
  int gy = (C + 63) / 64;
  if (gy > 16) gy = 16;
  long gx = (rows + 4 * 16 - 1) / (4 * 16);
  gx = gx > 256 ? 256 : (gx < 1 ? 1 : gx);
  hipLaunchKernelGGL(col_stats_kernel, dim3((unsigned)gx, gy), dim3(64, 4), 0, (hipStream_t)stream, x,
                     rows, C, ldx, stats, stats + BAL_MAXC);
  S2T_CHECK_LAUNCH();
  return 0;
}

extern "C" int s2t_balancer_apply(const float* x, long ldx, const float* g, long ldg, long rows,
                                  int C, float min_mean, float max_mean, float min_rms,
                                  float max_rms, float grad_scale, float* out, long ldo,
                                  const float* stats, float act_off, void* stream) {
  if (rows <= 0 || C <= 0) return 0;
  if (C > BAL_MAXC || !stats) return -1;
  if (bal_small(C, x, ldx, g, ldg, out, ldo)) {
    const long nq = rows * C / 4;
    hipLaunchKernelGGL(balancer_apply_small_kernel, dim3(bal_small_grid(nq)), dim3(256), 0, (hipStream_t)stream,
                       x, g, stats, (float*)nullptr, (float)rows, min_mean, max_mean, min_rms, max_rms, grad_scale,
                       nq, C, out, act_off);
    S2T_CHECK_LAUNCH();
    return 0;
  }
  hipLaunchKernelGGL(balancer_apply_fused_kernel, dim3((unsigned)std::min<long>((rows + 15) / 16, 2048)),
                     dim3(256), 0, (hipStream_t)stream, x, ldx, g, ldg, stats, (float*)nullptr,
                     (float)rows, min_mean, max_mean, min_rms, max_rms, grad_scale, rows, C, out, ldo,
                     act_off);
  S2T_CHECK_LAUNCH();
  return 0;
}
```

### speech2text_amd/csrc/zip_glue.hip

```cpp
#include "common.h"
#include "../../include/s2t_mi355.h"

namespace {

constexpr int RB = 64;

__global__ __launch_bounds__(256) void bypass_fwd_kernel(const float* __restrict__ orig,
                                                         const float* __restrict__ src,
                                                         const float* __restrict__ scale, long n4,
                                                         int C4, float* __restrict__ out) {
  const float4* o4 = reinterpret_cast<const float4*>(orig);
  const float4* s4 = reinterpret_cast<const float4*>(src);
  const float4* sc4 = reinterpret_cast<const float4*>(scale);
  float4* y4 = reinterpret_cast<float4*>(out);
  for (long i = (long)blockIdx.x * 256 + threadIdx.x; i < n4; i += (long)gridDim.x * 256) {
    const float4 a = o4[i], b = s4[i], k = sc4[i % C4];
    y4[i] = make_float4(fmaf(b.x - a.x, k.x, a.x), fmaf(b.y - a.y, k.y, a.y),
                        fmaf(b.z - a.z, k.z, a.z), fmaf(b.w - a.w, k.w, a.w));
  }
}

__global__ __launch_bounds__(256) void bypass_bwd_kernel(const float* __restrict__ orig,
                                                         const float* __restrict__ src,
                                                         const float* __restrict__ scale,
                                                         const float* __restrict__ g, long rows,
                                                         int C, float* __restrict__ d_orig,
                                                         float* __restrict__ d_src,
                                                         float* __restrict__ d_scale) {
  const long r0 = (long)blockIdx.x * RB, r1 = min(rows, r0 + RB);
  for (int c = threadIdx.x; c < C; c += 256) {
    const float k = scale[c];
    float acc = 0.f;
    long r = r0;
    for (; r + 3 < r1; r += 4) {
      float gq[4], sq[4], oq[4];
#pragma unroll
      for (int u = 0; u < 4; ++u) {
        const long i = (r + u) * C + c;
        gq[u] = g[i];
        sq[u] = src[i];
        oq[u] = orig[i];
      }
#pragma unroll
      for (int u = 0; u < 4; ++u) {
        const long i = (r + u) * C + c;
        const float ds = gq[u] * k;
        d_src[i] = ds;
        d_orig[i] = gq[u] - ds;
        acc = fmaf(gq[u], sq[u] - oq[u], acc);
      }
    }
    for (; r < r1; ++r) {
      const long i = r * C + c;
      const float gv = g[i], ds = gv * k;
      d_src[i] = ds;
      d_orig[i] = gv - ds;
      acc = fmaf(gv, src[i] - orig[i], acc);
    }
    atomicAdd(d_scale + c, acc);
  }
}

__global__ __launch_bounds__(256) void bypass_bwd_acc_kernel(const float* __restrict__ orig,
                                                             const float* __restrict__ src,
                                                             const float* __restrict__ scale,
                                                             const float* __restrict__ g,
                                                             const float* __restrict__ acc_in,
                                                             long rows, int C,
                                                             float* __restrict__ d_orig,
                                                             float* __restrict__ d_src,
                                                             float* __restrict__ d_scale) {
  const long r0 = (long)blockIdx.x * RB, r1 = min(rows, r0 + RB);
  for (int c = threadIdx.x; c < C; c += 256) {
    const float k = scale[c];
    float acc = 0.f;
    long r = r0;
    for (; r + 3 < r1; r += 4) {
      float gq[4], sq[4], oq[4], aq[4];
#pragma unroll
      for (int u = 0; u < 4; ++u) {
        const long i = (r + u) * C + c;
        gq[u] = g[i];
        sq[u] = src[i];
        oq[u] = orig[i];
        aq[u] = acc_in[i];
      }
#pragma unroll
      for (int u = 0; u < 4; ++u) {
        const long i = (r + u) * C + c;
        const float ds = gq[u] * k;
        d_src[i] = ds;
        d_orig[i] = gq[u] - ds + aq[u];
        acc = fmaf(gq[u], sq[u] - oq[u], acc);
      }
    }
    for (; r < r1; ++r) {
      const long i = r * C + c;
      const float gv = g[i], ds = gv * k;
      d_src[i] = ds;
      d_orig[i] = gv - ds + acc_in[i];
      acc = fmaf(gv, src[i] - orig[i], acc);
    }
    atomicAdd(d_scale + c, acc);
  }
}

__global__ __launch_bounds__(256) void attn_delta_pairs_kernel(
    const float* __restrict__ W, const float* __restrict__ dW0, const float* __restrict__ dO1,
    const float* __restrict__ O1, int dv1, const float* __restrict__ dO2,
    const float* __restrict__ O2, int dv2, int T, int B, int H, float* __restrict__ delta) {
  const long row = (long)blockIdx.x * 4 + (threadIdx.x >> 6);
  const int lane = threadIdx.x & 63;
  if (row >= (long)H * B * T) return;
  const int i = (int)(row % T);
  const int b = (int)((row / T) % B);
  const int h = (int)(row / ((long)T * B));
  float acc = 0.f;
  if (dO1 && lane < dv1) {
    const long o = ((long)i * B + b) * H * dv1 + (long)h * dv1 + lane;
    acc = dO1[o] * O1[o];
  }
  if (dO2 && lane < dv2) {
    const long o = ((long)i * B + b) * H * dv2 + (long)h * dv2 + lane;
    acc = fmaf(dO2[o], O2[o], acc);
  }
  if (h == 0 && dW0) {
    const float* w = W + ((long)b * T + i) * T;
    const float* d = dW0 + ((long)b * T + i) * T;
    for (int j = lane; j < T; j += 64) acc = fmaf(w[j], d[j], acc);
  }
  acc = wave_sum(acc);
  if (lane == 0) delta[row] = acc;
}

__global__ __launch_bounds__(256) void bypass_fwd_mask_kernel(const float* __restrict__ orig,
                                                              const float* __restrict__ src,
                                                              const float* __restrict__ scale,
                                                              const float* __restrict__ fm, int B,
                                                              long n4, int C4,
                                                              float* __restrict__ out) {
  const float4* o4 = reinterpret_cast<const float4*>(orig);
  const float4* s4 = reinterpret_cast<const float4*>(src);
  const float4* sc4 = reinterpret_cast<const float4*>(scale);
  const float4* m4 = reinterpret_cast<const float4*>(fm);
  float4* y4 = reinterpret_cast<float4*>(out);
  for (long i = (long)blockIdx.x * 256 + threadIdx.x; i < n4; i += (long)gridDim.x * 256) {
    const int c = (int)(i % C4);
    const int b = (int)((i / C4) % B);
    const float4 a = o4[i], v = s4[i], k = sc4[c], m = m4[(long)b * C4 + c];
    y4[i] = make_float4(fmaf(v.x - a.x, k.x, a.x) * m.x, fmaf(v.y - a.y, k.y, a.y) * m.y,
                        fmaf(v.z - a.z, k.z, a.z) * m.z, fmaf(v.w - a.w, k.w, a.w) * m.w);
  }
}
// ... 137 lines not shown
  for (int tt = blockIdx.x; tt < dT; tt += gridDim.x) {
    const float4* g4 = reinterpret_cast<const float4*>(g + (btC4 > 0 ? 0 : (long)tt * rowlen));
    for (long e = (long)blockIdx.y * 256 + threadIdx.x; e < n4; e += (long)gridDim.y * 256) {
      const float4 gv = btC4 > 0 ? g4[((e / btC4) * dT + tt) * btC4 + (e % btC4)] : g4[e];
      float4 sv[8];
#pragma unroll
      for (int k = 0; k < 8; ++k)
        if (k < ds) {
          const long tc = min((long)tt * ds + k, (long)T - 1);
          sv[k] = reinterpret_cast<const float4*>(src + tc * rowlen)[e];
        }
      float4 last = make_float4(0.f, 0.f, 0.f, 0.f);
#pragma unroll
      for (int k = 0; k < 8; ++k)
        if (k < ds) {
          const long t = (long)tt * ds + k;
          pw[k] += gv.x * sv[k].x + gv.y * sv[k].y + gv.z * sv[k].z + gv.w * sv[k].w;
          const float4 o = make_float4(wk[k] * gv.x, wk[k] * gv.y, wk[k] * gv.z, wk[k] * gv.w);
          if (t < T - 1) {
            reinterpret_cast<float4*>(d_src + t * rowlen)[e] = o;
          } else {
            last.x += o.x; last.y += o.y; last.z += o.z; last.w += o.w;
          }
        }
      if ((long)tt * ds + ds - 1 >= T - 1)
        reinterpret_cast<float4*>(d_src + (long)(T - 1) * rowlen)[e] = last;
    }
  }
#pragma unroll
  for (int k = 0; k < 8; ++k) {
    const float v = wave_sum(pw[k]);
    if ((threadIdx.x & 63) == 0) s_dw[k][threadIdx.x >> 6] = v;
  }
  __syncthreads();
  if ((int)threadIdx.x < ds)
    atomicAdd(dw + threadIdx.x, (s_dw[threadIdx.x][0] + s_dw[threadIdx.x][1]) +
                                    (s_dw[threadIdx.x][2] + s_dw[threadIdx.x][3]));
}

__global__ __launch_bounds__(256) void bypass_up_fwd_kernel(const float* __restrict__ orig,
                                                            const float* __restrict__ src,
                                                            const float* __restrict__ scale,
                                                            int up, int Bn, long n4, int C4,
                                                            float* __restrict__ out) {
  const float4* o4 = reinterpret_cast<const float4*>(orig);
  const float4* s4 = reinterpret_cast<const float4*>(src);
  const float4* sc4 = reinterpret_cast<const float4*>(scale);
  float4* y4 = reinterpret_cast<float4*>(out);
  const long frame4 = (long)Bn * C4;
  for (long i = (long)blockIdx.x * 256 + threadIdx.x; i < n4; i += (long)gridDim.x * 256) {
    const long t = i / frame4, e = i - t * frame4;
    const float4 a = o4[i], v = s4[(t / up) * frame4 + e], k = sc4[e % C4];
    y4[i] = make_float4(fmaf(v.x - a.x, k.x, a.x), fmaf(v.y - a.y, k.y, a.y),
                        fmaf(v.z - a.z, k.z, a.z), fmaf(v.w - a.w, k.w, a.w));
  }
}

__global__ __launch_bounds__(256) void bypass_up_bwd_kernel(const float* __restrict__ orig,
                                                            const float* __restrict__ src,
                                                            const float* __restrict__ scale,
                                                            const float* __restrict__ g, int up,
                                                            int T, int Bn, int C,
                                                            float* __restrict__ d_orig,
                                                            float* __restrict__ d_src,
                                                            float* __restrict__ d_scale) {
  const int tt = blockIdx.x;
  const int b0 = blockIdx.y * 16, b1 = min(Bn, b0 + 16);
  for (int c = threadIdx.x; c < C; c += 256) {
    const float k = scale[c];
    float acc = 0.f;
    for (int b = b0; b < b1; ++b) {
      const float sv = src[((long)tt * Bn + b) * C + c];
      float ds_ = 0.f;
      for (int u = 0; u < up; ++u) {
        const long t = (long)tt * up + u;
        if (t >= T) break;
        const long i = (t * Bn + b) * C + c;
        const float gv = g[i];
        d_orig[i] = gv * (1.f - k);
        ds_ = fmaf(gv, k, ds_);
        acc = fmaf(gv, sv - orig[i], acc);
      }
      d_src[((long)tt * Bn + b) * C + c] = ds_;
    }
    atomicAdd(d_scale + c, acc);
  }
}

template <int UP, int IU>
__global__ __launch_bounds__(256) void bypass_up_bwd4_kernel(const float4* __restrict__ o4,
                                                             const float4* __restrict__ s4,
                                                             const float4* __restrict__ sc4,
                                                             const float4* __restrict__ g4, int T, long F,
                                                             int C4, long n, float4* __restrict__ do4,
                                                             float4* __restrict__ ds4,
                                                             float* __restrict__ d_scale) {
  __shared__ float s_acc[1024];
  for (int i = threadIdx.x; i < 4 * C4; i += 256) s_acc[i] = 0.f;
  __syncthreads();
  const long stride = (long)gridDim.x * 256;
  const long w0 = (long)blockIdx.x * 256 + threadIdx.x;
  const int c4 = (int)(w0 % C4);
  const float4 k = sc4[c4];
  float4 acc = make_float4(0.f, 0.f, 0.f, 0.f);
  for (long wb = w0; wb < n; wb += stride * IU) {
    float4 sv[IU], gv[IU][UP], ov[IU][UP];
#pragma unroll
    for (int j = 0; j < IU; ++j) {
      const long w = wb + j * stride < n ? wb + j * stride : wb;
      const long tt = w / F, e = w - tt * F;
      sv[j] = s4[w];
#pragma unroll
      for (int u = 0; u < UP; ++u) {
        const long t = tt * UP + u;
        const long i = (t < T ? t : tt * UP) * F + e;
        gv[j][u] = g4[i];
        ov[j][u] = o4[i];
      }
    }
#pragma unroll
    for (int j = 0; j < IU; ++j) {
      const long w = wb + j * stride;
      if (w < n) {
        const long tt = w / F, e = w - tt * F;
        float4 ds = make_float4(0.f, 0.f, 0.f, 0.f);
#pragma unroll
        for (int u = 0; u < UP; ++u) {
          const long t = tt * UP + u;
          if (t < T) {
            const float4 gq = gv[j][u], oq = ov[j][u], sq = sv[j];
            do4[t * F + e] =
                make_float4(gq.x * (1.f - k.x), gq.y * (1.f - k.y), gq.z * (1.f - k.z), gq.w * (1.f - k.w));
            ds = make_float4(fmaf(gq.x, k.x, ds.x), fmaf(gq.y, k.y, ds.y), fmaf(gq.z, k.z, ds.z),
                             fmaf(gq.w, k.w, ds.w));
            acc = make_float4(fmaf(gq.x, sq.x - oq.x, acc.x), fmaf(gq.y, sq.y - oq.y, acc.y),
                              fmaf(gq.z, sq.z - oq.z, acc.z), fmaf(gq.w, sq.w - oq.w, acc.w));
          }
        }
        ds4[w] = ds;
      }
    }
  }
  atomicAdd(&s_acc[4 * c4 + 0], acc.x);
  atomicAdd(&s_acc[4 * c4 + 1], acc.y);
  atomicAdd(&s_acc[4 * c4 + 2], acc.z);
  atomicAdd(&s_acc[4 * c4 + 3], acc.w);
  __syncthreads();
  for (int i = threadIdx.x; i < 4 * C4; i += 256) {
    const float v = s_acc[i];
    if (v != 0.f) atomicAdd(d_scale + i, v);
  }
}

__global__ __launch_bounds__(256) void nonlin_gate_fwd_kernel(const float* __restrict__ u, int T,
                                                              int B, int C,
                                                              float* __restrict__ xs) {
  const long n = (long)T * B * C;
  for (long i = (long)blockIdx.x * 256 + threadIdx.x; i < n; i += (long)gridDim.x * 256) {
    const int c = (int)(i % C);
    const long tb = i / C;
    const int b = (int)(tb % B);
    const long t = tb / B;
    const float* row = u + tb * 3 * C;
    xs[((long)b * T + t) * C + c] = row[C + c] * tanhf(row[c]);
  }
}

__global__ __launch_bounds__(256) void nonlin_out_fwd_kernel(const float* __restrict__ z,
                                                             const float* __restrict__ u, int T,
                                                             int B, int C, float* __restrict__ o) {
  const long n = (long)T * B * C;
  for (long i = (long)blockIdx.x * 256 + threadIdx.x; i < n; i += (long)gridDim.x * 256) {
    const int c = (int)(i % C);
    const long tb = i / C;
    const int b = (int)(tb % B);
    const long t = tb / B;
    o[i] = z[((long)b * T + t) * C + c] * u[tb * 3 * C + 2 * C + c];
  }
}

__global__ __launch_bounds__(256) void nonlin_out_bwd_kernel(const float* __restrict__ g,
                                                             const float* __restrict__ z,
                                                             const float* __restrict__ u, int T,
                                                             int B, int C, float* __restrict__ dz,
                                                             float* __restrict__ du) {
  const long n = (long)T * B * C;
  for (long i = (long)blockIdx.x * 256 + threadIdx.x; i < n; i += (long)gridDim.x * 256) {
    const int c = (int)(i % C);
    const long tb = i / C;
    const int b = (int)(tb % B);
    const long t = tb / B;
    const long zi = ((long)b * T + t) * C + c;
    const float gv = g[i];
    dz[zi] = gv * u[tb * 3 * C + 2 * C + c];
    du[tb * 3 * C + 2 * C + c] = gv * z[zi];
  }
}

__global__ __launch_bounds__(256) void nonlin_gate_bwd_kernel(const float* __restrict__ dxs,
                                                              const float* __restrict__ u, int T,
                                                              int B, int C,
                                                              float* __restrict__ du) {
  const long n = (long)T * B * C;
  for (long i = (long)blockIdx.x * 256 + threadIdx.x; i < n; i += (long)gridDim.x * 256) {
    const int c = (int)(i % C);
    const long tb = i / C;
    const int b = (int)(tb % B);
    const long t = tb / B;
    const float d = dxs[((long)b * T + t) * C + c];
    const float* row = u + tb * 3 * C;
    const float th = tanhf(row[c]);
    du[tb * 3 * C + c] = d * row[C + c] * (1.f - th * th);
    du[tb * 3 * C + C + c] = d * th;
  }
}

inline unsigned grid1(long n) {
  long g = (n + 255) / 256;
  return (unsigned)(g > 4096 ? 4096 : (g < 1 ? 1 : g));
}

}

extern "C" int s2t_bypass_fwd(const float* orig, const float* src, const float* scale, long rows,
                              int C, float* out, void* stream) {
  if (rows <= 0) return 0;
  if (C <= 0 || (C & 3)) return -1;
  const long n4 = rows * C / 4;
  hipLaunchKernelGGL(bypass_fwd_kernel, dim3(grid1(n4)), dim3(256), 0, (hipStream_t)stream, orig,
                     src, scale, n4, C / 4, out);
  S2T_CHECK_LAUNCH();
  return 0;
}

extern "C" int s2t_bypass_bwd(const float* orig, const float* src, const float* scale,
                              const float* g, long rows, int C, float* d_orig, float* d_src,
                              float* d_scale, void* stream) {
  if (rows <= 0) return 0;
  if (C <= 0) return -1;
  hipLaunchKernelGGL(bypass_bwd_kernel, dim3((unsigned)((rows + RB - 1) / RB)), dim3(256), 0,
                     (hipStream_t)stream, orig, src, scale, g, rows, C, d_orig, d_src, d_scale);
  S2T_CHECK_LAUNCH();
  return 0;
}

extern "C" int s2t_bypass_bwd_acc(const float* orig, const float* src, const float* scale,
                                  const float* g, const float* acc_in, long rows, int C,
                                  float* d_orig, float* d_src, float* d_scale, void* stream) {
  if (rows <= 0) return 0;
  if (C <= 0 || !acc_in) return -1;
  hipLaunchKernelGGL(bypass_bwd_acc_kernel, dim3((unsigned)((rows + RB - 1) / RB)), dim3(256), 0,
                     (hipStream_t)stream, orig, src, scale, g, acc_in, rows, C, d_orig, d_src,
                     d_scale);
  S2T_CHECK_LAUNCH();
  return 0;
}

extern "C" int s2t_attn_delta_pairs(const float* W, const float* dW0, const float* dO1,
                                    const float* O1, int dv1, const float* dO2, const float* O2,
                                    int dv2, int T, int B, int H, float* delta, void* stream) {
  if (T <= 0 || B <= 0 || H <= 0) return 0;
  if (dv1 > 64 || dv2 > 64 || dv1 < 0 || dv2 < 0) return -1;
  const long rows = (long)H * B * T;
  hipLaunchKernelGGL(attn_delta_pairs_kernel, dim3((unsigned)((rows + 3) / 4)), dim3(256), 0,
                     (hipStream_t)stream, W, dW0, dO1, O1, dv1, dO2, O2, dv2, T, B, H, delta);
  S2T_CHECK_LAUNCH();
  return 0;
}

extern "C" int s2t_bypass_fwd_mask(const float* orig, const float* src, const float* scale,
                                   const float* fm, int B, long rows, int C, float* out,
                                   void* stream) {
  if (rows <= 0) return 0;
  if (C <= 0 || (C & 3) || B <= 0 || !fm) return -1;
  const long n4 = rows * C / 4;
  hipLaunchKernelGGL(bypass_fwd_mask_kernel, dim3(grid1(n4)), dim3(256), 0, (hipStream_t)stream,
                     orig, src, scale, fm, B, n4, C / 4, out);
  S2T_CHECK_LAUNCH();
  return 0;
}

extern "C" int s2t_bypass_bwd_mask(const float* orig, const float* src, const float* scale,
                                   const float* g, const float* fm, int B, long rows, int C,
                                   float* d_orig, float* d_src, float* d_scale, void* stream) {
  if (rows <= 0) return 0;
  if (C <= 0 || B <= 0 || !fm) return -1;
  hipLaunchKernelGGL(bypass_bwd_mask_kernel, dim3((unsigned)((rows + RB - 1) / RB)), dim3(256), 0,
                     (hipStream_t)stream, orig, src, scale, g, fm, B, rows, C, d_orig, d_src,
                     d_scale);
  S2T_CHECK_LAUNCH();
  return 0;
}

extern "C" int s2t_param_grad_commit_n(int n, const S2tCommit* items, void* stream) {
  if (n <= 0) return 0;
  if (n > 8 || !items) return -1;
  CommitGroup grp;
  grp.n = n;
  long longest = 1;
  for (int i = 0; i < n; ++i) {
    grp.it[i] = items[i];
    longest = items[i].n > longest ? items[i].n : longest;
  }
  hipLaunchKernelGGL(param_grad_commit_n_kernel, dim3((unsigned)((longest + 255) / 256)), dim3(256),
                     0, (hipStream_t)stream, grp);
  S2T_CHECK_LAUNCH();
  return 0;
}

static int downsample_fwd_impl(const float* src, const float* w, int ds, int T, int B, int C, float* out,
                               int bt, void* stream) {
  if (T <= 0 || B <= 0 || C <= 0) return 0;
  if (ds < 1 || ds > 8) return -1;
  const int dT = (T + ds - 1) / ds;
  const long rowlen = (long)B * C, n_out = (long)dT * rowlen;
  hipLaunchKernelGGL(downsample_fwd_kernel, dim3(grid1(n_out)), dim3(256), 0, (hipStream_t)stream,
                     src, w, ds, T, rowlen, n_out, out, bt ? C : 0, dT);
  S2T_CHECK_LAUNCH();
  return 0;
}
static int downsample_bwd_impl(const float* src, const float* w, const float* g, int ds, int T, int B, int C,
                               float* d_src, float* dw, int bt, void* stream);

extern "C" int s2t_downsample_fwd(const float* src, const float* w, int ds, int T, int B, int C,
                                  float* out, void* stream) {
  return downsample_fwd_impl(src, w, ds, T, B, C, out, 0, stream);
}
extern "C" int s2t_downsample_fwd_bt(const float* src, const float* w, int ds, int T, int B, int C,
                                     float* out, void* stream) {
  return downsample_fwd_impl(src, w, ds, T, B, C, out, 1, stream);
}
extern "C" int s2t_downsample_bwd(const float* src, const float* w, const float* g, int ds, int T,
                                  int B, int C, float* d_src, float* dw, void* stream) {
  return downsample_bwd_impl(src, w, g, ds, T, B, C, d_src, dw, 0, stream);
}
extern "C" int s2t_downsample_bwd_bt(const float* src, const float* w, const float* g, int ds, int T,
                                     int B, int C, float* d_src, float* dw, void* stream) {
  return downsample_bwd_impl(src, w, g, ds, T, B, C, d_src, dw, 1, stream);
}

static int downsample_bwd_impl(const float* src, const float* w, const float* g, int ds, int T, int B, int C,
                               float* d_src, float* dw, int bt, void* stream) {
  if (T <= 0 || B <= 0 || C <= 0) return 0;
  if (ds < 1 || ds > 8) return -1;
  const int dT = (T + ds - 1) / ds;
  const long rowlen = (long)B * C;
  if ((rowlen & 3) || (C & 3) || ((reinterpret_cast<uintptr_t>(src) | reinterpret_cast<uintptr_t>(g) |
                                  reinterpret_cast<uintptr_t>(d_src)) & 15)) {
    long blocks = ((long)dT * rowlen + 1023) / 1024;
    blocks = blocks > 1024 ? 1024 : (blocks < 1 ? 1 : blocks);
    hipLaunchKernelGGL(downsample_bwd_any_kernel, dim3((unsigned)blocks), dim3(256), 0,
                       (hipStream_t)stream, src, w, g, ds, T, dT, rowlen, d_src, dw, bt ? C : 0);
    S2T_CHECK_LAUNCH();
    return 0;
  }
  constexpr long cap = 512;
  int gy = (int)std::min<long>((rowlen / 4 + 255) / 256, std::max<long>(1, cap / dT));
  if (gy < 1) gy = 1;
  const int gx = (int)std::min<long>(dT, std::max<long>(1, cap / gy));
  hipLaunchKernelGGL(downsample_bwd_kernel, dim3(gx, gy), dim3(256), 0,
                     (hipStream_t)stream, src, w, g, ds, T, dT, rowlen, d_src, dw, bt ? C / 4 : 0);
  S2T_CHECK_LAUNCH();
  return 0;
}

extern "C" int s2t_bypass_up_fwd(const float* orig, const float* src, const float* scale, int up,
                                 int T, int B, int C, float* out, void* stream) {
  if (T <= 0 || B <= 0) return 0;
  if (C <= 0 || (C & 3) || up < 1) return -1;
  const long n4 = (long)T * B * C / 4;
  hipLaunchKernelGGL(bypass_up_fwd_kernel, dim3(grid1(n4)), dim3(256), 0, (hipStream_t)stream,
                     orig, src, scale, up, B, n4, C / 4, out);
  S2T_CHECK_LAUNCH();
  return 0;
}

extern "C" int s2t_bypass_up_bwd(const float* orig, const float* src, const float* scale,
                                 const float* g, int up, int T, int B, int C, float* d_orig,
                                 float* d_src, float* d_scale, void* stream) {
  if (T <= 0 || B <= 0) return 0;
  if (C <= 0 || up < 1) return -1;
  const int Ts = (T + up - 1) / up;
  const uintptr_t al = reinterpret_cast<uintptr_t>(orig) | reinterpret_cast<uintptr_t>(src) |
                       reinterpret_cast<uintptr_t>(scale) | reinterpret_cast<uintptr_t>(g) |
                       reinterpret_cast<uintptr_t>(d_orig) | reinterpret_cast<uintptr_t>(d_src);
  if ((C & 3) == 0 && C <= 1024 && (al & 15) == 0 && (up == 2 || up == 4 || up == 8)) {
    const int C4 = C / 4;
    const long F = (long)B * C4, n = (long)Ts * F;
    int gc = C4, r = 256;
    while (r) { const int t = gc % r; gc = r; r = t; }
    const long m = C4 / gc;
    constexpr long cap = 256;
    long nb = (n + 255) / 256;
    if (nb > cap) nb = cap;
    nb = (nb + m - 1) / m * m;
#define BUP4(UP, IU)                                                                                          \
  hipLaunchKernelGGL((bypass_up_bwd4_kernel<UP, IU>), dim3((unsigned)nb), dim3(256), 0, (hipStream_t)stream,  \
                     reinterpret_cast<const float4*>(orig), reinterpret_cast<const float4*>(src),             \
                     reinterpret_cast<const float4*>(scale), reinterpret_cast<const float4*>(g), T, F, C4, n, \
                     reinterpret_cast<float4*>(d_orig), reinterpret_cast<float4*>(d_src), d_scale)
    if (up == 2) BUP4(2, 4);
    else if (up == 4) BUP4(4, 2);
    else BUP4(8, 1);
#undef BUP4
    S2T_CHECK_LAUNCH();
    return 0;
  }
  hipLaunchKernelGGL(bypass_up_bwd_kernel, dim3(Ts, (B + 15) / 16), dim3(256), 0,
                     (hipStream_t)stream, orig, src, scale, g, up, T, B, C, d_orig, d_src, d_scale);
  S2T_CHECK_LAUNCH();
  return 0;
}

extern "C" int s2t_nonlin_gate_fwd(const float* u, int T, int B, int C, float* xs, void* stream) {
  if (T <= 0 || B <= 0 || C <= 0) return 0;
  hipLaunchKernelGGL(nonlin_gate_fwd_kernel, dim3(grid1((long)T * B * C)), dim3(256), 0,
                     (hipStream_t)stream, u, T, B, C, xs);
  S2T_CHECK_LAUNCH();
  return 0;
}

extern "C" int s2t_nonlin_out_fwd(const float* z, const float* u, int T, int B, int C, float* o,
                                  void* stream) {
  if (T <= 0 || B <= 0 || C <= 0) return 0;
  hipLaunchKernelGGL(nonlin_out_fwd_kernel, dim3(grid1((long)T * B * C)), dim3(256), 0,
                     (hipStream_t)stream, z, u, T, B, C, o);
  S2T_CHECK_LAUNCH();
  return 0;
}

extern "C" int s2t_nonlin_out_bwd(const float* g, const float* z, const float* u, int T, int B,
                                  int C, float* dz, float* du, void* stream) {
  if (T <= 0 || B <= 0 || C <= 0) return 0;
  hipLaunchKernelGGL(nonlin_out_bwd_kernel, dim3(grid1((long)T * B * C)), dim3(256), 0,
                     (hipStream_t)stream, g, z, u, T, B, C, dz, du);
  S2T_CHECK_LAUNCH();
  return 0;
}

extern "C" int s2t_nonlin_gate_bwd(const float* dxs, const float* u, int T, int B, int C,
                                   float* du, void* stream) {
  if (T <= 0 || B <= 0 || C <= 0) return 0;
  hipLaunchKernelGGL(nonlin_gate_bwd_kernel, dim3(grid1((long)T * B * C)), dim3(256), 0,
                     (hipStream_t)stream, dxs, u, T, B, C, du);
  S2T_CHECK_LAUNCH();
  return 0;
}
```

### speech2text_amd/csrc/zip_layer.hip

```cpp
#include <hip/hip_runtime.h>

#include <cmath>
#include <cstdint>
#include <cstdio>
#include <cstring>
#include <atomic>
#include <functional>
#include <mutex>
#include <unordered_map>
#include <vector>

#include "../../include/s2t_mi355.h"
#include "common.h"

namespace {

constexpr int kMagic = 0x5a4c3532;
constexpr float kPenLimit = 25.0f;
constexpr int kMaxProb = 48;

thread_local char g_err[256] = "";

std::mutex g_mu;
float* g_pin = nullptr;
// ... 396 lines not shown
  const int parity = s2t_balancer_next_parity();
  RUN(s2t_balancer_bwd(x, ldx, g, ldg, R, C, b.min_mean, b.max_mean, b.min_rms, b.max_rms, b.grad_scale,
                       out, ldo, c.c.bal_ws, parity, act_off, (void*)c.st));
  return 0;
}

int wgrad(Ctx& c, const S2tZlLin& L, const float* g2, long ldg, const float* a2, long lda, long R) {
  if (c.s.nprob >= kMaxProb) return fail(-1, "wgrad: too many problems");
  S2tTnProblem& q = c.s.probs[c.s.nprob++];
  q.A = g2;
  q.lda = ldg;
  q.B = a2;
  q.ldb = lda;
  q.C = L.gw;
  q.ldc = L.K;
  q.M = L.N;
  q.N = L.K;
  q.K = (int)R;
  q.colsum = L.gb;
  q.alpha = 1.0f;
  return 0;
}

int copy2d(Ctx& c, float* dst, long ldd, const float* src, long lds, int cols, long rows) {
  HIPRUN(hipMemcpy2DAsync(dst, ldd * 4, src, lds * 4, (size_t)cols * 4, (size_t)rows, hipMemcpyDeviceToDevice, c.st));
  return 0;
}

int bal_stats_fwd(Ctx& c, int site, const float* x, long ldx, long R, int C, int n = 2048,
                  const S2tZlBal* coef = nullptr) {
  c.s.bst[site] = nullptr;
  if (!c.c.bal_fwd_side || (!c.dry && !c.side) || C > 1024) return 0;
  float* st = c.ar.alloc(n);
  c.s.bst[site] = st;
  if (c.dry) return 0;
  c.s.bal_fwd = 1;
  return side_run(c, [&c, st, x, ldx, R, C, coef]() -> int {
    HIPRUN(hipMemsetAsync(st, 0, 2048 * sizeof(float), c.side));
    RUN(s2t_balancer_stats(x, ldx, R, C, st, (void*)c.side));
    if (coef)
      RUN(s2t_balancer_coef(st, C, R, coef->min_mean, coef->max_mean, coef->min_rms, coef->max_rms, coef->grad_scale,
                            (void*)c.side));
    return 0;
  });
}

int out_proj(Ctx& c, const S2tZlLin& L, const float* a, long R, const float* x_in, bool need_y, float** y,
             float** out) {
  const int D = c.d.D;
  *out = c.ar.alloc(R * D);
  Epi e;
  e.bias = L.b;
  if (!need_y) {
    *y = nullptr;
    e.resid2 = x_in;
    return lt_matmul(c, 0, a, L.K, R, L, e, *out);
  }
  *y = c.ar.alloc(R * D);
  e.act2 = 3;
  e.out2 = *out;
  e.resid_b = x_in;
  return lt_matmul(c, 0, a, L.K, R, L, e, *y);
}

int ff_fwd(Ctx& c, int i, int d0, const float* x_in, const float** x_out) {
  const S2tZlFf& m = c.d.ff[i];
  FfS& sv = c.s.ff[i];
  const bool fw = dec(c, d0 + 1), fp = dec(c, d0 + 2);
  const long R = c.R;
  const int F = m.in.N;
  sv.h = c.ar.alloc(R * F);
  sv.a = c.ar.alloc(R * F);
  Epi e;
  e.bias = m.in.b;
  e.act2 = 1;
  e.out2 = sv.a;
  TRY(lt_matmul(c, 0, x_in, c.d.D, R, m.in, e, sv.h));
  c.s.bst[3 + i] = nullptr;
  if (dec(c, d0)) TRY(bal_stats_fwd(c, 3 + i, sv.h, F, R, F, 4096, &m.hidden));
  float* out;
  TRY(out_proj(c, m.out, sv.a, R, x_in, fw || fp, &sv.y, &out));
  c.s.bst[i] = nullptr;
  if (fp) TRY(bal_stats_fwd(c, i, sv.y, c.d.D, R, c.d.D));
  sv.st.on = 0;
  if (fw) TRY(whiten_stats(c, sv.st, sv.y, c.d.D, R, c.d.D, m.out_wh.groups));
  *x_out = out;
  return 0;
}

int sa_fwd(Ctx& c, int i, int dfw, const float* x_in, const float** x_out) {
  const S2tZlSa& m = c.d.sa[i];
  SaS& sv = c.s.sa[i];
  const bool fw = dec(c, dfw);
  const long R = c.R;
  const int HD = m.in.N, H = c.d.H;
  sv.dv = HD / H;
  sv.v = c.ar.alloc(R * HD);
  Epi e;
  e.bias = m.in.b;
  TRY(lt_matmul(c, 0, x_in, c.d.D, R, m.in, e, sv.v));
  sv.o = c.ar.alloc(R * HD);
  RUN(s2t_attn_apply(c.s.W, sv.v, c.c.T, c.c.B, H, sv.dv, 0, sv.o, (void*)c.st));
  float* out;
  TRY(out_proj(c, m.out, sv.o, R, x_in, fw, &sv.y, &out));
  sv.st.on = 0;
  if (fw) TRY(whiten_stats(c, sv.st, sv.y, c.d.D, R, c.d.D, m.wh.groups));
  *x_out = out;
  return 0;
}

int conv_fwd(Ctx& c, int i, int d0, const float* x_in, const float** x_out) {
  const S2tZlConv& m = c.d.cv[i];
  CvS& sv = c.s.cv[i];
  const bool fw = dec(c, d0 + 2);
  const long R = c.R;
  const int D = c.d.D, T = c.c.T, B = c.c.B;
  if (c.c.chunk_size >= 0 && !m.causal) return fail(-1, "conv module: chunk_size needs causal=True");
  sv.u = c.ar.alloc(R * 2 * D);
  Epi e;
  e.bias = m.in.b;
  TRY(lt_matmul(c, 0, x_in, D, R, m.in, e, sv.u));
  c.s.bst[6 + i] = c.s.bst[8 + i] = nullptr;
  if (dec(c, d0)) TRY(bal_stats_fwd(c, 6 + i, sv.u + D, 2 * D, R, D));
  sv.chunk = (c.c.chunk_size < 0 || c.c.chunk_size > T) ? T : c.c.chunk_size;
  sv.y = c.ar.alloc(R * D);
  sv.a = c.ar.alloc(R * D);
  RUN(s2t_zipconv_fwd_act(sv.u, 2 * D, D, c.c.k8, T, B, D, m.K, sv.chunk, m.wc, m.bc, m.wk, m.bk, m.scale, sv.y,
                          sv.a, 2, (void*)c.st));
  if (dec(c, d0 + 1)) TRY(bal_stats_fwd(c, 8 + i, sv.y, D, R, D, 4096, &m.bal2));
  sv.st.on = 0;
  if (fw) TRY(whiten_stats(c, sv.st, sv.y, D, R, D, m.wh.groups));
  float* out = c.ar.alloc(R * D);
  Epi e2;
  e2.bias = m.out.b;
  e2.resid2 = x_in;
  TRY(lt_matmul(c, 0, sv.a, D, R, m.out, e2, out));
  *x_out = out;
  return 0;
}

int na_fwd(Ctx& c, const float* x_in, const float** x_out) {
  const S2tZlNa& m = c.d.na;
  NaS& sv = c.s.na;
  const bool fw1 = dec(c, 8), fw2 = dec(c, 9), fp = dec(c, 10);
  const long R = c.R;
  const int D = c.d.D, T = c.c.T, B = c.c.B;
  const int C = m.in.N / 3;
  sv.C = C;
  sv.u = c.ar.alloc(R * 3 * C);
  Epi e;
  e.bias = m.in.b;
  TRY(lt_matmul(c, 0, x_in, D, R, m.in, e, sv.u));
  c.s.bst[10] = c.s.bst[11] = nullptr;
  if (dec(c, 7)) TRY(bal_stats_fwd(c, 11, sv.u, 3 * C, R, C));
  sv.xs = c.ar.alloc(R * C);
  RUN(s2t_nonlin_gate_fwd(sv.u, T, B, C, sv.xs, (void*)c.st));
  sv.z = c.ar.alloc(R * C);
  { const S2tGemmClass cls(0); TRY(bmm(c, 1, c.s.W, sv.xs, sv.z, B, T, C, T)); }
  sv.o = c.ar.alloc(R * C);
  RUN(s2t_nonlin_out_fwd(sv.z, sv.u, T, B, C, sv.o, (void*)c.st));
  sv.st1.on = 0;
  if (fw1) TRY(whiten_stats(c, sv.st1, sv.u + C, 3 * C, R, C, m.wh1.groups));
  float* out;
  TRY(out_proj(c, m.out, sv.o, R, x_in, fw2 || fp, &sv.y, &out));
  if (fp) TRY(bal_stats_fwd(c, 10, sv.y, D, R, D));
  sv.st2.on = 0;
  if (fw2) TRY(whiten_stats(c, sv.st2, sv.y, D, R, D, m.wh2.groups));
  *x_out = out;
  return 0;
}

int layer_fwd(Ctx& c) {
  const S2tZipLayerDesc& d = c.d;
  State& s = c.s;
  const int T = c.c.T, B = c.c.B, D = d.D, H = d.H, qd = d.qd, pd = d.pd;
  const long R = c.R;
  const int Dp = d.attn_in.N;
  s.magic = kMagic;
  s.T = T;
  s.B = B;
  s.nprob = 0;
  s.x[0] = c.c.x0;
  s.bal_fwd = 0;
  for (int i = 0; i < kBalSites; ++i) s.bst[i] = nullptr;
  s.qkp = c.ar.alloc(R * Dp);
  {
    Epi e;
    e.bias = d.attn_in.b;
    TRY(lt_matmul(c, 0, s.x[0], D, R, d.attn_in, e, s.qkp));
  }
  if (dec(c, 0)) TRY(bal_stats_fwd(c, 14, s.qkp + H * qd, Dp, R, H * qd));
  s.kst.on = 0;
  if (dec(c, 1)) TRY(whiten_stats(c, s.kst, s.qkp + H * qd, Dp, R, H * qd, d.wh_keys.groups));
  s.posp = nullptr;
  s.pos2 = c.c.pos;
  if (dec(c, 2)) {
    s.posp = c.ar.alloc((long)(2 * T - 1) * H * pd);
    Epi e;
    TRY(lt_matmul(c, 0, c.c.pos, d.pos_dim, 2 * T - 1, d.attn_pos, e, s.posp));
  }
  s.W = c.ar.alloc((long)H * B * T * T);
  s.pen_slot = nullptr;
  if (dec(c, 3)) {
    if (!c.dry) {
      s.pen_slot = pinned_slot();
      s.pen_ev = ring_event();
      if (!s.pen_slot || !s.pen_ev) return fail(-1, "penalty flag slot");
      *s.pen_slot = 0.f;
    }
    RUN(s2t_relpos_attn_fwd_flag(s.qkp, s.posp, c.c.k8, c.c.a8, T, B, H, qd, pd, s.W, kPenLimit, s.pen_slot,
                                 (void*)c.st));
    HIPRUN(hipEventRecord(s.pen_ev, c.st));
  } else {
    RUN(s2t_relpos_attn_fwd(s.qkp, s.posp, c.c.k8, c.c.a8, T, B, H, qd, pd, s.W, (void*)c.st));
  }
  TRY(ff_fwd(c, 0, 4, s.x[0], &s.x[1]));
  TRY(na_fwd(c, s.x[1], &s.x[2]));
  TRY(sa_fwd(c, 0, 11, s.x[2], &s.x[3]));
  TRY(conv_fwd(c, 0, 12, s.x[3], &s.x[4]));
  TRY(ff_fwd(c, 1, 15, s.x[4], &s.x[5]));
  float* x6 = c.ar.alloc(R * D);
  RUN(s2t_bypass_fwd(s.x[0], s.x[5], d.byp_mid.x, R, D, x6, (void*)c.st));
  s.x[6] = x6;
  TRY(sa_fwd(c, 1, 19, s.x[6], &s.x[7]));
  TRY(conv_fwd(c, 1, 20, s.x[7], &s.x[8]));
  TRY(ff_fwd(c, 2, 23, s.x[8], &s.x[9]));
  if (dec(c, 26)) TRY(bal_stats_fwd(c, 12, s.x[9], D, R, D));
  s.nscales = c.ar.alloc(R);
  s.x[10] = nullptr;
  s.x[11] = c.c.out;
  s.fm_fused = c.c.fm != nullptr && !(dec(c, 30) || dec(c, 29));
  RUN(s2t_norm_bypass_fwd(s.x[9], d.norm_bias.x, d.norm_ls.x, s.x[0], d.byp.x, s.fm_fused ? c.c.fm : nullptr, B, R,
                          D, c.c.out, s.nscales, (void*)c.st));
  if (dec(c, 29)) TRY(bal_stats_fwd(c, 13, c.c.out, D, R, D));
  s.wst.on = 0;
  if (dec(c, 30)) TRY(whiten_stats(c, s.wst, c.c.out, D, R, D, d.wh_out.groups));
  TRY(flush_side(c));
  if (s.bal_fwd && !c.dry) {
    s.bal_ev = ring_event();
    if (!s.bal_ev) return fail(-1, "balancer statistics event");
    HIPRUN(hipEventRecord(s.bal_ev, c.side));
    s.bal_seq = ++g_bal_seq;
  }
  return 0;
}

int ff_bwd(Ctx& c, int i, int d0, const float* x_in, const float* g, const float** g_out) {
  const S2tZlFf& m = c.d.ff[i];
  FfS& sv = c.s.ff[i];
  const bool fb = dec(c, d0), fw = dec(c, d0 + 1), fp = dec(c, d0 + 2);
  const long R = c.R;
  const int D = c.d.D, F = m.in.N;
  const int site = i == 0 ? 1 : (i == 1 ? 6 : 9);
  const float* gy = g;
  if (fp) {
    float* o = c.ar.alloc(R * D);
    TRY(balancer_bwd(c, m.post, sv.y, D, gy, D, R, D, o, D, -1.0f, c.s.bst[i]));
    gy = o;
  }
  if (fw) TRY(whiten_bwd(c, site, m.out_wh, sv.st, sv.y, D, R, D, gy, &gy));
  TRY(wgrad(c, m.out, gy, D, sv.a, F, R));
  float* dh = c.ar.alloc(R * F);
  if (fb) {
    Epi e;
    e.act_src = sv.h;
    e.act_kind = 1;
    e.bal = &m.hidden;
    e.bal_stats = c.s.bst[3 + i];
    TRY(lt_matmul(c, 1, gy, D, R, m.out, e, dh));
  } else {
    Epi e;
    e.act_src = sv.h;
    e.act_kind = 1;
    TRY(lt_matmul(c, 1, gy, D, R, m.out, e, dh));
  }
  TRY(wgrad(c, m.in, dh, F, x_in, D, R));
  float* gx = c.ar.alloc(R * D);
  Epi e;
  e.resid2 = g;
  TRY(lt_matmul(c, 1, dh, F, R, m.in, e, gx));
  *g_out = gx;
  return 0;
}

int sa_bwd(Ctx& c, int i, int dfw, const float* x_in, const float* g, const float** g_out) {
  const S2tZlSa& m = c.d.sa[i];
  SaS& sv = c.s.sa[i];
  const bool fw = dec(c, dfw);
  const long R = c.R;
  const int D = c.d.D, HD = m.in.N, H = c.d.H;
  const float* gy = g;
  if (fw) TRY(whiten_bwd(c, i == 0 ? 4 : 7, m.wh, sv.st, sv.y, D, R, D, g, &gy));
  TRY(wgrad(c, m.out, gy, D, sv.o, HD, R));
  float* dO = c.ar.alloc(R * HD);
  {
    Epi e;
    TRY(lt_matmul(c, 1, gy, D, R, m.out, e, dO));
  }
  float* dV = c.ar.alloc(R * HD);
  RUN(s2t_attn_apply(c.s.W, dO, c.c.T, c.c.B, H, sv.dv, 1, dV, (void*)c.st));
  c.s.dO[i == 1 ? 0 : 1] = dO;
  TRY(wgrad(c, m.in, dV, HD, x_in, D, R));
  float* gx = c.ar.alloc(R * D);
  Epi e;
  e.resid2 = g;
  TRY(lt_matmul(c, 1, dV, HD, R, m.in, e, gx));
  *g_out = gx;
  return 0;
}

int conv_bwd(Ctx& c, int i, int d0, const float* x_in, const float* g, const float** g_out) {
  const S2tZlConv& m = c.d.cv[i];
  CvS& sv = c.s.cv[i];
  const bool fb1 = dec(c, d0), fb2 = dec(c, d0 + 1), fw = dec(c, d0 + 2);
  const long R = c.R;
  const int D = c.d.D, T = c.c.T, B = c.c.B;
  TRY(wgrad(c, m.out, g, D, sv.a, D, R));
  const float* dy;
  if (fb2 && !fw) {
    float* o = c.ar.alloc(R * D);
    Epi e;
    e.act_src = sv.y;
    e.act_kind = 2;
    e.bal = &m.bal2;
    e.bal_stats = c.s.bst[8 + i];
    TRY(lt_matmul(c, 1, g, D, R, m.out, e, o));
    dy = o;
  } else {
    float* t = c.ar.alloc(R * D);
    Epi e;
    e.act_src = sv.y;
    e.act_kind = 2;
    TRY(lt_matmul(c, 1, g, D, R, m.out, e, t));
    dy = t;
    if (fw) TRY(whiten_bwd(c, i == 0 ? 5 : 8, m.wh, sv.st, sv.y, D, R, D, dy, &dy));
    if (fb2) {
      float* o = c.ar.alloc(R * D);
      TRY(balancer_bwd(c, m.bal2, sv.y, D, dy, D, R, D, o, D, -1.0f, c.s.bst[8 + i]));
      dy = o;
    }
  }
  float* du = c.ar.alloc(R * 2 * D);
  const long wsn = s2t_zipconv_bwd_workspace_floats(T, B, D, m.K);
  float* ws = c.ar.alloc(wsn);
  if (c.c.conv_w_side && c.side) {
    RUN(s2t_zipconv_bwd_data(sv.u, 2 * D, D, c.c.k8, T, B, D, m.K, sv.chunk, m.wc, m.wk, m.bk, m.scale, dy, du,
                             (void*)c.st));
    if (!c.dry)
      TRY(side_run(c, [&c, &m, &sv, dy, ws, T, B, D]() -> int {
        RUN(s2t_zipconv_bwd_params(sv.u, 2 * D, D, c.c.k8, T, B, D, m.K, sv.chunk, m.wc, m.wk, m.bk, m.scale, dy,
                                   m.gwc, m.gbc, m.gwk, m.gbk, m.gscale, ws, (void*)c.side));
        return 0;
      }));
  } else {
    RUN(s2t_zipconv_bwd(sv.u, 2 * D, D, c.c.k8, T, B, D, m.K, sv.chunk, m.wc, m.wk, m.bk, m.scale, dy, du, m.gwc,
                        m.gbc, m.gwk, m.gbk, m.gscale, ws, (void*)c.st));
  }
  if (fb1) TRY(balancer_bwd(c, m.bal1, sv.u + D, 2 * D, du + D, 2 * D, R, D, du + D, 2 * D, -1.0f, c.s.bst[6 + i]));
  TRY(wgrad(c, m.in, du, 2 * D, x_in, D, R));
  float* gx = c.ar.alloc(R * D);
  Epi e;
  e.resid2 = g;
  TRY(lt_matmul(c, 1, du, 2 * D, R, m.in, e, gx));
  *g_out = gx;
  return 0;
}

int na_bwd(Ctx& c, const float* x_in, const float* g, const float** g_out) {
  const S2tZlNa& m = c.d.na;
  NaS& sv = c.s.na;
  const bool fb = dec(c, 7), fw1 = dec(c, 8), fw2 = dec(c, 9), fp = dec(c, 10);
  const long R = c.R;
  const int D = c.d.D, T = c.c.T, B = c.c.B, C = sv.C;
  const float* gy = g;
  if (fp) {
    float* o = c.ar.alloc(R * D);
    TRY(balancer_bwd(c, m.post, sv.y, D, gy, D, R, D, o, D, -1.0f, c.s.bst[10]));
    gy = o;
  }
  if (fw2) TRY(whiten_bwd(c, 3, m.wh2, sv.st2, sv.y, D, R, D, gy, &gy));
  TRY(wgrad(c, m.out, gy, D, sv.o, C, R));
  float* dout = c.ar.alloc(R * C);
  {
    Epi e;
    TRY(lt_matmul(c, 1, gy, D, R, m.out, e, dout));
  }
  float* dz = c.ar.alloc(R * C);
  float* du = c.ar.alloc(R * 3 * C);
  RUN(s2t_nonlin_out_bwd(dout, sv.z, sv.u, T, B, C, dz, du, (void*)c.st));
  float* dxs = c.ar.alloc(R * C);
  const S2tGemmClass cls_d(1);
  TRY(bmm(c, 2, c.s.W, dz, dxs, B, T, C, T));
  c.s.dW0 = c.ar.alloc((long)B * T * T);
  TRY(bmm(c, 0, dz, sv.xs, c.s.dW0, B, T, T, C));
  RUN(s2t_nonlin_gate_bwd(dxs, sv.u, T, B, C, du, (void*)c.st));
  if (fb) TRY(balancer_bwd(c, m.bal, sv.u, 3 * C, du, 3 * C, R, C, du, 3 * C, -1.0f, c.s.bst[11]));
  if (fw1) {
    float* gc = c.ar.alloc(R * C);
    TRY(copy2d(c, gc, C, du + C, 3 * C, C, R));
    const float* o;
    TRY(whiten_bwd(c, 2, m.wh1, sv.st1, sv.u + C, 3 * C, R, C, gc, &o));
    if (o != gc) TRY(copy2d(c, du + C, 3 * C, o, C, C, R));
  }
  TRY(wgrad(c, m.in, du, 3 * C, x_in, D, R));
  float* gx = c.ar.alloc(R * D);
  Epi e;
  e.resid2 = g;
  TRY(lt_matmul(c, 1, du, 3 * C, R, m.in, e, gx));
  *g_out = gx;
  return 0;
}

int layer_bwd(Ctx& c, int phase) {
  const S2tZipLayerDesc& d = c.d;
  State& s = c.s;
  const int T = c.c.T, B = c.c.B, D = d.D, H = d.H, qd = d.qd, pd = d.pd;
  const long R = c.R;
  const int Dp = d.attn_in.N;
  if (phase != 2) {
    s.nprob = 0;
    for (int i = 0; i < S2T_ZL_NWHITEN; ++i) s.wh_active[i] = -1;
    s.pen_active = 0;
    if (s.bal_fwd && !c.dry && !(g_bal_waited_on == (void*)c.st && s.bal_seq <= g_bal_waited)) {
      HIPRUN(hipStreamWaitEvent(c.st, s.bal_ev, 0));
      g_bal_waited_on = (void*)c.st;
      g_bal_waited = s.bal_seq;
    }
    if (dec(c, 3) && !c.dry) {
      if (hipEventSynchronize(s.pen_ev) != hipSuccess) return fail(-1, "penalty flag event");
      s.pen_active = *reinterpret_cast<volatile float*>(s.pen_slot) != 0.f;
    }
    const float* g = c.c.g;
    const float* x11 = s.x[11];
    if (dec(c, 30)) TRY(whiten_bwd(c, 10, d.wh_out, s.wst, x11, D, R, D, g, &g));
    if (dec(c, 29)) {
      float* o = c.ar.alloc(R * D);
      TRY(balancer_bwd(c, d.bal2, x11, D, g, D, R, D, o, D, -1.0f, s.bst[13]));
      g = o;
    }
    float* acc = c.c.layer_acc;
    float* d0 = c.ar.alloc(R * D);
    float* g9w = c.ar.alloc(R * D);
    RUN(s2t_norm_bypass_bwd(s.x[9], d.norm_bias.x, s.nscales, s.x[0], d.byp.x, g, s.fm_fused ? c.c.fm : nullptr, B,
                            R, D, g9w, d0, acc, acc + 2 * D, acc + 3 * D, (void*)c.st));
    const float* g9 = g9w;
    if (dec(c, 26)) {
      float* o = c.ar.alloc(R * D);
      TRY(balancer_bwd(c, d.bal1, s.x[9], D, g9, D, R, D, o, D, -1.0f, s.bst[12]));
      g9 = o;
    }
    const float *g8, *g7, *g6, *g4, *g3, *g2, *g1, *g0;
    TRY(ff_bwd(c, 2, 23, s.x[8], g9, &g8));
    TRY(conv_bwd(c, 1, 20, s.x[7], g8, &g7));
    TRY(sa_bwd(c, 1, 19, s.x[6], g7, &g6));
    float* d0m = c.ar.alloc(R * D);
    float* g5 = c.ar.alloc(R * D);
    RUN(s2t_bypass_bwd_acc(s.x[0], s.x[5], d.byp_mid.x, g6, d0, R, D, d0m, g5, acc + D, (void*)c.st));
    {
      S2tCommit it[4] = {
          {d.byp.x, acc, d.byp.grad, d.byp.lo, d.byp.hi, dec(c, 28) ? 1 : 0, (long)D},
          {d.byp_mid.x, acc + D, d.byp_mid.grad, d.byp_mid.lo, d.byp_mid.hi, dec(c, 18) ? 1 : 0, (long)D},
          {d.norm_bias.x, acc + 2 * D, d.norm_bias.grad, 0.f, 0.f, 0, (long)D},
          {d.norm_ls.x, acc + 3 * D, d.norm_ls.grad, d.norm_ls.lo, d.norm_ls.hi, dec(c, 27) ? 1 : 0, 1L}};
      RUN(s2t_param_grad_commit_n(4, it, (void*)c.st));
    }
    TRY(ff_bwd(c, 1, 15, s.x[4], g5, &g4));
    TRY(conv_bwd(c, 0, 12, s.x[3], g4, &g3));
    TRY(sa_bwd(c, 0, 11, s.x[2], g3, &g2));
    TRY(na_bwd(c, s.x[1], g2, &g1));
    TRY(ff_bwd(c, 0, 4, s.x[0], g1, &g0));
    s.delta = c.ar.alloc((long)H * B * T);
    RUN(s2t_attn_delta_pairs(s.W, s.dW0, s.dO[0], s.sa[1].o, s.sa[1].dv, s.dO[1], s.sa[0].o, s.sa[0].dv, T, B, H,
                             s.delta, (void*)c.st));
    s.dqkp = c.ar.alloc(R * Dp);
    s.dpos = s.posp ? c.ar.alloc((long)(2 * T - 1) * H * pd) : nullptr;
    s.g0 = const_cast<float*>(g0);
    s.d0m = d0m;
    if (phase == 1 || (phase == 0 && s.pen_active)) {
      s.bwd_off = c.ar.off;
      TRY(flush_side(c));
      return s.pen_active ? 1 : 0;
    }
    float* aws = nullptr;
    if (s.posp) aws = c.ar.alloc(s2t_relpos_attn_bwd_workspace_floats(T, B, H, pd));
    RUN(s2t_relpos_attn_bwd(s.qkp, s.posp, c.c.k8, c.c.a8, T, B, H, qd, pd, s.W, nullptr, s.dW0, s.dO[0],
                            s.sa[1].v, s.sa[1].dv, s.dO[1], s.sa[0].v, s.sa[0].dv, 1, s.delta, s.dqkp, s.dpos, aws,
                            (void*)c.st));
  }
  float* dqkp = s.dqkp;
  if (dec(c, 1) || dec(c, 0)) {
    const int Ck = H * qd;
    float* gk = c.ar.alloc(R * Ck);
    TRY(copy2d(c, gk, Ck, dqkp + Ck, Dp, Ck, R));
    const float* cur = gk;
    if (dec(c, 1)) TRY(whiten_bwd(c, 0, d.wh_keys, s.kst, s.qkp + Ck, Dp, R, Ck, cur, &cur));
    if (dec(c, 0)) {
      float* o = c.ar.alloc(R * Ck);
      TRY(balancer_bwd(c, d.bal_keys, s.qkp + Ck, Dp, cur, Ck, R, Ck, o, Ck, -1.0f, s.bst[14]));
      cur = o;
    }
    TRY(copy2d(c, dqkp + Ck, Dp, cur, Ck, Ck, R));
  }
  if (s.dpos) TRY(wgrad(c, d.attn_pos, s.dpos, H * pd, s.pos2, d.pos_dim, 2 * T - 1));
  TRY(wgrad(c, d.attn_in, dqkp, Dp, s.x[0], D, R));
  {
    Epi e;
    e.resid2 = s.g0;
    e.resid_b = s.d0m;
    TRY(lt_matmul(c, 1, dqkp, Dp, R, d.attn_in, e, c.c.gx));
  }
  if (!c.dry && s.nprob > 0) {
    if (c.c.wgrad_side && c.side) {
      TRY(side_run(c, [&c, &s]() -> int {
        RUN(s2t_gemm_tn_grouped(s.nprob, s.probs, (void*)c.side));
        return 0;
      }));
    } else {
      RUN(s2t_gemm_tn_grouped(s.nprob, s.probs, (void*)c.st));
    }
  }
  return flush_side(c);
}

}

extern "C" {

long s2t_zip_layer_state_bytes(void) { return (long)sizeof(State); }

void* s2t_zip_layer_error(void) { return (void*)g_err; }

int s2t_zl_plan_put(int mode, int half_oct, int N, int K, double t_lib_ms, double t_own_ms, int tile) {
  std::lock_guard<std::mutex> lock(g_mu);
  g_plans[plan_key(mode, half_oct, N, K)] = Base{t_lib_ms, t_own_ms, tile};
  return 0;
}
int s2t_zl_plan_clear(void) {
  std::lock_guard<std::mutex> lock(g_mu);
  g_plans.clear();
  return 0;
}
long s2t_zl_plan_count(void) { return (long)g_plans.size(); }
int s2t_zl_plan_choose(int mode, long rows, int N, int K, int epilogue_bits, float margin, int* tile) {
  if (!tile) return -1;
  std::lock_guard<std::mutex> lock(g_mu);
  return plan_choose(mode, rows, N, K, epilogue_bits, margin, tile);
}

long s2t_zip_layer_ws_floats(const S2tZipLayerDesc* desc, const S2tZipLayerCall* call, int backward) {
  if (!desc || !call) return -1;
  State tmp;
  memset(&tmp, 0, sizeof(tmp));
  Ctx c{*desc, *call, tmp, Arena{nullptr, 0, 0}, nullptr, nullptr, true, (long)call->T * call->B};
  if (layer_fwd(c) != 0) return -1;
  const long fwd = c.ar.off;
  if (!backward) return fwd;
  c.ar.off = 0;
  if (layer_bwd(c, 0) != 0) return -1;
  return c.ar.off + 64;
}

int s2t_zip_layer_plans_missing(const S2tZipLayerDesc* desc, int T, int B) {
  if (!desc) return -1;
  const long R = (long)T * B;
  const S2tZlLin* both[] = {&desc->attn_in,   &desc->ff[0].in, &desc->ff[0].out, &desc->ff[1].in, &desc->ff[1].out,
                            &desc->ff[2].in,  &desc->ff[2].out, &desc->na.in,    &desc->na.out,   &desc->sa[0].in,
                            &desc->sa[0].out, &desc->sa[1].in, &desc->sa[1].out, &desc->cv[0].in, &desc->cv[0].out,
                            &desc->cv[1].in,  &desc->cv[1].out};
  std::lock_guard<std::mutex> lock(g_mu);
  for (const S2tZlLin* L : both)
    if (plan_missing(0, R, *L) || plan_missing(1, R, *L)) return 1;
  if (plan_missing(0, 2 * T - 1, desc->attn_pos)) return 1;
  return 0;
}

int s2t_zip_layer_fwd(const S2tZipLayerDesc* desc, const S2tZipLayerCall* call, void* state, float* ws,
                      long ws_floats, void* stream, void* side) {
  if (!desc || !call || !state || !ws || call->T < 4 || call->B < 1 || !call->x0 || !call->out) return -1;
  g_err[0] = 0;
  State& s = *reinterpret_cast<State*>(state);
  memset(&s, 0, sizeof(State));
  Ctx c{*desc, *call, s, Arena{ws, ws_floats, 0}, (hipStream_t)stream, (hipStream_t)side, false,
        (long)call->T * call->B};
  {
    State tmp;
    memset(&tmp, 0, sizeof(tmp));
    Ctx dr{*desc, *call, tmp, Arena{nullptr, 0, 0}, nullptr, nullptr, true, c.R};
    if (layer_fwd(dr) != 0 || dr.ar.off > ws_floats) return fail(-4, "s2t_zip_layer_fwd: workspace too small");
  }
  if (s2t_zip_layer_plans_missing(desc, call->T, call->B) == 1)
    return fail(-5, "s2t_zip_layer_fwd: a product of this shape has not been timed yet");
  return layer_fwd(c);
}

int s2t_zip_layer_bwd(const S2tZipLayerDesc* desc, const S2tZipLayerCall* call, void* state, float* ws,
                      long ws_floats, int phase, void* stream, void* side) {
  if (!desc || !call || !state || !ws || !call->g || !call->gx || phase < 0 || phase > 2) return -1;
  g_err[0] = 0;
  State& s = *reinterpret_cast<State*>(state);
  if (s.magic != kMagic || s.T != call->T || s.B != call->B) return fail(-1, "s2t_zip_layer_bwd: stale state");
  Ctx c{*desc, *call, s, Arena{ws, ws_floats, phase == 2 ? s.bwd_off : 0}, (hipStream_t)stream,
        (hipStream_t)side, false, (long)call->T * call->B};
// ... 30 lines not shown
```

Before: 18430 audio-seconds/sec.

## Fuse balancer gradient update into norm-bypass and nonlin-gate backward kernels

Per-channel balancer coefficients are now computed during the forward stats pass and stored next to the stats buffer. The norm-bypass backward and nonlin-gate backward kernels then apply the balancer gradient update in their epilogue, so the separate balancer_bwd kernel and its extra read/write pass over the gradient are dropped. The nonlinear-attention gate and out kernels also get new float4-vectorized variants, and the shared coefficient math moves into one device header. This adds template variants and a fallback path, and the fused norm kernel uses fewer rows per wave.

```diff
diff --git a/include/s2t_mi355.h b/include/s2t_mi355.h
--- a/include/s2t_mi355.h
+++ b/include/s2t_mi355.h
@@ -90,6 +90,10 @@
                         const float* bypass_scale, const float* g, const float* fm, int B, long rows, int D,
                         float* dx, float* d_orig, float* d_bypass_scale, float* dbias, float* dls,
                         void* stream);
+int s2t_norm_bypass_bwd_bal(const float* x, const float* bias, const float* scales, const float* orig,
+                            const float* bypass_scale, const float* g, const float* fm, int B, long rows,
+                            int D, float* dx, float* d_orig, float* d_bypass_scale, float* dbias, float* dls,
+                            const float* coef, void* stream);
 int s2t_biasnorm_bwd(const float* x, const float* bias, const float* scales, const float* g,
                      long rows, int D, float* dx, float* dbias, float* dls, void* stream);
 long s2t_balancer_bwd_workspace_floats(void);
@@ -412,6 +416,8 @@
                        float* du, void* stream);
 int s2t_nonlin_gate_bwd(const float* dxs, const float* u, int T, int B, int C, float* du,
                         void* stream);
+int s2t_nonlin_gate_bwd_bal(const float* dxs, const float* u, int T, int B, int C, float* du,
+                            const float* coef, void* stream);
 
 int s2t_layernorm_fwd(const float* x, const float* y, float alpha, const float* gamma,
                       const float* beta, long rows, int C, float eps, float* xsum, float* out,
diff --git a/speech2text_amd/csrc/bal_update.h b/speech2text_amd/csrc/bal_update.h
--- /dev/null
+++ b/speech2text_amd/csrc/bal_update.h
@@ -0,0 +1,36 @@
+#pragma once
+#include <hip/hip_runtime.h>
+
+__device__ __forceinline__ void bal_coef_ab(float sum, float sumsq, float inv_n, float min_mean, float max_mean,
+                                            float min_rms, float max_rms, float grad_scale, float& a_out,
+                                            float& b_out) {
+#pragma clang fp contract(off)
+  const float mean = sum * inv_n, uvar = sumsq * inv_n;
+  const float raw_var = uvar - mean * mean;
+  const bool live_v = raw_var > 1.0e-20f, live_r = uvar > 1.0e-20f;
+  const float var = fmaxf(raw_var, 1.0e-20f);
+  const float sd = sqrtf(var);
+  const float rms = sqrtf(fmaxf(uvar, 1.0e-20f));
+  const float m = mean / sd;
+  const float mc = fminf(fmaxf(m, min_mean), max_mean);
+  const float s_m = (m > mc) ? 1.f : ((m < mc) ? -1.f : 0.f);
+  const float rc = fminf(fmaxf(rms, min_rms), max_rms);
+  const float lq = logf(rc / rms);
+  const float s_r = (lq > 0.f) ? -1.f : ((lq < 0.f) ? 1.f : 0.f);
+  const float a = s_m * inv_n * (live_v ? (1.f / sd + mean * mean / (sd * var)) : 1.f / sd);
+  const float b = (live_v ? -s_m * inv_n * mean / (sd * var) : 0.f) +
+                  (live_r ? s_r * inv_n / (rms * rms) : 0.f);
+  const float lg_rms =
+      fmaxf(sqrtf(fmaxf(fmaf(uvar, b * b, fmaf(a, a, 2.f * a * b * mean)), 0.f)), 1.0e-20f);
+  const float coef = grad_scale / lg_rms;
+  a_out = a * coef;
+  b_out = b * coef;
+}
+
+__device__ __forceinline__ float bal_update(float g, float x, float a, float b) {
+  return fmaf(fabsf(g), fmaf(b, x, a), g);
+}
+__device__ __forceinline__ float4 bal_update4(const float4 g, const float4 x, const float4 a, const float4 b) {
+  return make_float4(bal_update(g.x, x.x, a.x, b.x), bal_update(g.y, x.y, a.y, b.y),
+                     bal_update(g.z, x.z, a.z, b.z), bal_update(g.w, x.w, a.w, b.w));
+}
diff --git a/speech2text_amd/csrc/common.h b/speech2text_amd/csrc/common.h
--- a/speech2text_amd/csrc/common.h
+++ b/speech2text_amd/csrc/common.h
@@ -29,6 +29,16 @@
   explicit S2tGemmClass(int cls) : prev(s2t_gemm_class_set(cls)) {}
   ~S2tGemmClass() { s2t_gemm_class_set(prev); }
 };
+
+#define S2T_FUSED_BAL_STORE 1
+#define S2T_FUSED_NONLIN16 4
+static inline int s2t_layer_fused(void) {
+  static const int mask = [] {
+    const char* e = getenv("S2T_LAYER_FUSED");
+    return e ? atoi(e) : (S2T_FUSED_BAL_STORE | S2T_FUSED_NONLIN16);
+  }();
+  return mask;
+}
 
 #define S2T_WAVE 64
 #define S2T_NEG_INF (-__builtin_huge_valf())
diff --git a/speech2text_amd/csrc/gemm_x3p.hip b/speech2text_amd/csrc/gemm_x3p.hip
--- a/speech2text_amd/csrc/gemm_x3p.hip
+++ b/speech2text_amd/csrc/gemm_x3p.hip
@@ -1,4 +1,5 @@
 #include "common.h"
+#include "bal_update.h"
 #include "../../include/s2t_mi355.h"
 #include <hip/hip_ext.h>
 #include <algorithm>
@@ -198,25 +199,7 @@
                                                         float min_rms, float max_rms, float gs) {
   const int c = blockIdx.x * 256 + threadIdx.x;
   if (c >= N) return;
-  const float inv_n = 1.f / n;
-  const float mean = stats[c] * inv_n, uvar = stats[1024 + c] * inv_n;
-  const float raw_var = uvar - mean * mean;
-  const bool live_v = raw_var > 1.0e-20f, live_r = uvar > 1.0e-20f;
-  const float var = fmaxf(raw_var, 1.0e-20f);
-  const float sd = sqrtf(var);
-  const float rms = sqrtf(fmaxf(uvar, 1.0e-20f));
-  const float m = mean / sd;
-  const float mc = fminf(fmaxf(m, min_mean), max_mean);
-  const float s_m = (m > mc) ? 1.f : ((m < mc) ? -1.f : 0.f);
-  const float rc = fminf(fmaxf(rms, min_rms), max_rms);
-  const float lq = logf(rc / rms);
-  const float s_r = (lq > 0.f) ? -1.f : ((lq < 0.f) ? 1.f : 0.f);
-  const float a = s_m * inv_n * (live_v ? (1.f / sd + mean * mean / (sd * var)) : 1.f / sd);
-  const float b = (live_v ? -s_m * inv_n * mean / (sd * var) : 0.f) + (live_r ? s_r * inv_n / (rms * rms) : 0.f);
-  const float lg_rms = fmaxf(sqrtf(fmaxf(a * a + 2.f * a * b * mean + b * b * uvar, 0.f)), 1.0e-20f);
-  const float k = gs / lg_rms;
-  coef[c] = a * k;
-  coef[1024 + c] = b * k;
+  bal_coef_ab(stats[c], stats[1024 + c], 1.f / n, min_mean, max_mean, min_rms, max_rms, gs, coef[c], coef[1024 + c]);
 }
 
 template <bool BAL = false>
diff --git a/speech2text_amd/csrc/zip_elem.hip b/speech2text_amd/csrc/zip_elem.hip
--- a/speech2text_amd/csrc/zip_elem.hip
+++ b/speech2text_amd/csrc/zip_elem.hip
@@ -1,4 +1,5 @@
 #include "common.h"
+#include "bal_update.h"
 #include <algorithm>
 #include <stdlib.h>
 
@@ -309,13 +310,13 @@
   }
 }
 
-template <int Q, int RT>
+template <int Q, int RT, bool BAL>
 __global__ __launch_bounds__(256) void norm_bypass_bwd16_kernel(
     const float* __restrict__ x, const float* __restrict__ bias, const float* __restrict__ scales,
     const float* __restrict__ orig, const float* __restrict__ bscale, const float* __restrict__ g,
     const float* __restrict__ fm, int B, long rows, int D, float* __restrict__ dx,
     float* __restrict__ d_orig, float* __restrict__ d_bscale, float* __restrict__ dbias,
-    float* __restrict__ dls) {
+    float* __restrict__ dls, const float* __restrict__ bcoef) {
   const int lane = threadIdx.x & 63, wv = threadIdx.x >> 6;
   const long wave = (long)blockIdx.x * 4 + wv;
   const long nwaves = (long)gridDim.x * 4;
@@ -390,7 +391,7 @@
       A = wave_sum(A);
       ss = wave_sum(ss);
       const float coef = s * A / ss;
-      dl += A * s;
+      dl = fmaf(A, s, dl);
 #pragma unroll
       for (int q = 0; q < Q; ++q) {
         const int cq = lane + 64 * q;
@@ -402,9 +403,14 @@
         float* oe = reinterpret_cast<float*>(&o);
 #pragma unroll
         for (int e = 0; e < 4; ++e) {
-          const float t = coef * (xe[e] - be[e]);
-          oe[e] = s * ge[e] - t;
+          const float t = mul_rounded(coef, xe[e] - be[e]);
+          oe[e] = fmaf(s, ge[e], -t);
           dbe[e] += t;
+        }
+        if (BAL) {
+          const int cc = cq < D4 ? cq : 0;
+          o = bal_update4(o, xv[i][q], reinterpret_cast<const float4*>(bcoef)[cc],
+                          reinterpret_cast<const float4*>(bcoef)[256 + cc]);
         }
         if (cq < D4) reinterpret_cast<float4*>(dx)[row * D4 + cq] = o;
       }
@@ -532,26 +538,7 @@
   const float inv_n = 1.f / n;
   if (threadIdx.x < C) {
     const int c = threadIdx.x;
-    const float mean = stats[c] * inv_n, uvar = stats[1024 + c] * inv_n;
-    const float raw_var = uvar - mean * mean;
-    const bool live_v = raw_var > 1.0e-20f, live_r = uvar > 1.0e-20f;
-    const float var = fmaxf(raw_var, 1.0e-20f);
-    const float sd = sqrtf(var);
-    const float rms = sqrtf(fmaxf(uvar, 1.0e-20f));
-    const float m = mean / sd;
-    const float mc = fminf(fmaxf(m, min_mean), max_mean);
-    const float s_m = (m > mc) ? 1.f : ((m < mc) ? -1.f : 0.f);
-    const float rc = fminf(fmaxf(rms, min_rms), max_rms);
-    const float lq = logf(rc / rms);
-    const float s_r = (lq > 0.f) ? -1.f : ((lq < 0.f) ? 1.f : 0.f);
-    const float a = s_m * inv_n * (live_v ? (1.f / sd + mean * mean / (sd * var)) : 1.f / sd);
-    const float b = (live_v ? -s_m * inv_n * mean / (sd * var) : 0.f) +
-                    (live_r ? s_r * inv_n / (rms * rms) : 0.f);
-    const float lg_rms =
-        fmaxf(sqrtf(fmaxf(a * a + 2.f * a * b * mean + b * b * uvar, 0.f)), 1.0e-20f);
-    const float coef = grad_scale / lg_rms;
-    s_a[c] = a * coef;
-    s_b[c] = b * coef;
+    bal_coef_ab(stats[c], stats[1024 + c], inv_n, min_mean, max_mean, min_rms, max_rms, grad_scale, s_a[c], s_b[c]);
   }
   if (blockIdx.x == 0 && stats_next != nullptr)
     for (int c = threadIdx.x; c < 2 * 1024; c += 256) stats_next[c] = 0.f;
@@ -580,10 +567,7 @@
         gg.z *= swoosh_d(xv[u].z, act_off);
         gg.w *= swoosh_d(xv[u].w, act_off);
       }
-      o4[i + u * step] = make_float4(gg.x + fabsf(gg.x) * fmaf(b4.x, xv[u].x, a4.x),
-                                     gg.y + fabsf(gg.y) * fmaf(b4.y, xv[u].y, a4.y),
-                                     gg.z + fabsf(gg.z) * fmaf(b4.z, xv[u].z, a4.z),
-                                     gg.w + fabsf(gg.w) * fmaf(b4.w, xv[u].w, a4.w));
+      o4[i + u * step] = bal_update4(gg, xv[u], a4, b4);
     }
   }
 }
@@ -595,28 +579,8 @@
     float* __restrict__ out, long ldo, float act_off) {
   __shared__ float s_a[1024], s_b[1024];
   const float inv_n = 1.f / n;
-  for (int c = threadIdx.x; c < C; c += 256) {
-    const float mean = stats[c] * inv_n, uvar = stats[1024 + c] * inv_n;
-    const float raw_var = uvar - mean * mean;
-    const bool live_v = raw_var > 1.0e-20f, live_r = uvar > 1.0e-20f;
-    const float var = fmaxf(raw_var, 1.0e-20f);
-    const float sd = sqrtf(var);
-    const float rms = sqrtf(fmaxf(uvar, 1.0e-20f));
-    const float m = mean / sd;
-    const float mc = fminf(fmaxf(m, min_mean), max_mean);
-    const float s_m = (m > mc) ? 1.f : ((m < mc) ? -1.f : 0.f);
-    const float rc = fminf(fmaxf(rms, min_rms), max_rms);
-    const float lq = logf(rc / rms);
-    const float s_r = (lq > 0.f) ? -1.f : ((lq < 0.f) ? 1.f : 0.f);
-    const float a = s_m * inv_n * (live_v ? (1.f / sd + mean * mean / (sd * var)) : 1.f / sd);
-    const float b = (live_v ? -s_m * inv_n * mean / (sd * var) : 0.f) +
-                    (live_r ? s_r * inv_n / (rms * rms) : 0.f);
-    const float lg_rms =
-        fmaxf(sqrtf(fmaxf(a * a + 2.f * a * b * mean + b * b * uvar, 0.f)), 1.0e-20f);
-    const float coef = grad_scale / lg_rms;
-    s_a[c] = a * coef;
-    s_b[c] = b * coef;
-  }
+  for (int c = threadIdx.x; c < C; c += 256)
+    bal_coef_ab(stats[c], stats[1024 + c], inv_n, min_mean, max_mean, min_rms, max_rms, grad_scale, s_a[c], s_b[c]);
   if (blockIdx.x == 0 && stats_next != nullptr)
     for (int c = threadIdx.x; c < 2 * 1024; c += 256) stats_next[c] = 0.f;
   __syncthreads();
@@ -637,14 +601,14 @@
 #pragma unroll
       for (int u = 0; u < 4; ++u) {
         if (act_off >= 0.f) gv[u] *= swoosh_d(xv[u], act_off);
-        out[(r + u * step) * ldo + c] = gv[u] + fabsf(gv[u]) * fmaf(b, xv[u], a);
+        out[(r + u * step) * ldo + c] = bal_update(gv[u], xv[u], a, b);
       }
     }
     for (; r < rows; r += step) {
       const float xs = x[r * ldx + c];
       float gv = g[r * ldg + c];
       if (act_off >= 0.f) gv *= swoosh_d(xs, act_off);
-      out[r * ldo + c] = gv + fabsf(gv) * fmaf(b, xs, a);
+      out[r * ldo + c] = bal_update(gv, xs, a, b);
     }
   }
 }
@@ -739,30 +703,39 @@
   return 0;
 }
 
-extern "C" int s2t_norm_bypass_bwd(const float* x, const float* bias, const float* scales,
-                                   const float* orig, const float* bypass_scale, const float* g,
-                                   const float* fm, int B, long rows, int D, float* dx, float* d_orig,
-                                   float* d_bypass_scale, float* dbias, float* dls, void* stream) {
+static int norm_bypass_bwd_launch(const float* x, const float* bias, const float* scales,
+                                  const float* orig, const float* bypass_scale, const float* g,
+                                  const float* fm, int B, long rows, int D, float* dx, float* d_orig,
+                                  float* d_bypass_scale, float* dbias, float* dls, const float* coef,
+                                  void* stream) {
   if (rows <= 0) return 0;
   if (D <= 0 || D > 1024 || B <= 0) return -1;
   hipStream_t st = (hipStream_t)stream;
   const uintptr_t al = reinterpret_cast<uintptr_t>(x) | reinterpret_cast<uintptr_t>(bias) |
                        reinterpret_cast<uintptr_t>(orig) | reinterpret_cast<uintptr_t>(bypass_scale) |
                        reinterpret_cast<uintptr_t>(g) | reinterpret_cast<uintptr_t>(fm) |
-                       reinterpret_cast<uintptr_t>(dx) | reinterpret_cast<uintptr_t>(d_orig);
+                       reinterpret_cast<uintptr_t>(dx) | reinterpret_cast<uintptr_t>(d_orig) |
+                       reinterpret_cast<uintptr_t>(coef);
   if ((D & 3) == 0 && (al & 15) == 0) {
     constexpr unsigned cap16 = 512u;
     const unsigned nb16 = std::min(grid_for(rows, 4 * (rows >= 8192 ? 16 : 8)), cap16);
-#define NB_BWD16(Q, RT)                                                                                  \
-  hipLaunchKernelGGL((norm_bypass_bwd16_kernel<Q, RT>), dim3(nb16), dim3(256), 0, st, x, bias, scales,   \
-                     orig, bypass_scale, g, fm, B, rows, D, dx, d_orig, d_bypass_scale, dbias, dls)
-    if (D <= 256) NB_BWD16(1, 4);
-    else if (D <= 512) NB_BWD16(2, 2);
-    else NB_BWD16(4, 1);
+#define NB_BWD16(Q, RT, BAL)                                                                                  \
+  hipLaunchKernelGGL((norm_bypass_bwd16_kernel<Q, RT, BAL>), dim3(nb16), dim3(256), 0, st, x, bias, scales,   \
+                     orig, bypass_scale, g, fm, B, rows, D, dx, d_orig, d_bypass_scale, dbias, dls, coef)
+    if (coef) {
+      if (D <= 256) NB_BWD16(1, 2, true);
+      else if (D <= 512) NB_BWD16(2, 1, true);
+      else NB_BWD16(4, 1, true);
+    } else {
+      if (D <= 256) NB_BWD16(1, 4, false);
+      else if (D <= 512) NB_BWD16(2, 2, false);
+      else NB_BWD16(4, 1, false);
+    }
 #undef NB_BWD16
     S2T_CHECK_LAUNCH();
     return 0;
   }
+  if (coef) return -2;
   const unsigned nb = std::min(grid_for(rows, 4 * 8), 1024u);
 #define NB_BWD(CPL)                                                                                    \
   hipLaunchKernelGGL(norm_bypass_bwd_kernel<CPL>, dim3(nb), dim3(256), 0, st, x, bias, scales, orig,   \
@@ -775,6 +748,23 @@
 #undef NB_BWD
   S2T_CHECK_LAUNCH();
   return 0;
+}
+
+extern "C" int s2t_norm_bypass_bwd(const float* x, const float* bias, const float* scales,
+                                   const float* orig, const float* bypass_scale, const float* g,
+                                   const float* fm, int B, long rows, int D, float* dx, float* d_orig,
+                                   float* d_bypass_scale, float* dbias, float* dls, void* stream) {
+  return norm_bypass_bwd_launch(x, bias, scales, orig, bypass_scale, g, fm, B, rows, D, dx, d_orig, d_bypass_scale,
+                                dbias, dls, nullptr, stream);
+}
+
+extern "C" int s2t_norm_bypass_bwd_bal(const float* x, const float* bias, const float* scales,
+                                       const float* orig, const float* bypass_scale, const float* g,
+                                       const float* fm, int B, long rows, int D, float* dx, float* d_orig,
+                                       float* d_bypass_scale, float* dbias, float* dls, const float* coef,
+                                       void* stream) {
+  return norm_bypass_bwd_launch(x, bias, scales, orig, bypass_scale, g, fm, B, rows, D, dx, d_orig, d_bypass_scale,
+                                dbias, dls, coef, stream);
 }
 
 static int biasnorm_bwd_launch(const float* x, const float* bias, const float* scales, const float* g,
diff --git a/speech2text_amd/csrc/zip_glue.hip b/speech2text_amd/csrc/zip_glue.hip
--- a/speech2text_amd/csrc/zip_glue.hip
+++ b/speech2text_amd/csrc/zip_glue.hip
@@ -1,4 +1,7 @@
+#include <initializer_list>
+
 #include "common.h"
+#include "bal_update.h"
 #include "../../include/s2t_mi355.h"
 
 namespace {
@@ -442,6 +445,13 @@
   }
 }
 
+__device__ __forceinline__ float na_gate(float s, float x) { return x * tanhf(s); }
+__device__ __forceinline__ void na_gate_bwd(float d, float s, float x, float& ds, float& dx) {
+  const float th = tanhf(s);
+  ds = d * x * fmaf(-th, th, 1.f);
+  dx = d * th;
+}
+
 __global__ __launch_bounds__(256) void nonlin_gate_fwd_kernel(const float* __restrict__ u, int T,
                                                               int B, int C,
                                                               float* __restrict__ xs) {
@@ -452,7 +462,7 @@
     const int b = (int)(tb % B);
     const long t = tb / B;
     const float* row = u + tb * 3 * C;
-    xs[((long)b * T + t) * C + c] = row[C + c] * tanhf(row[c]);
+    xs[((long)b * T + t) * C + c] = na_gate(row[c], row[C + c]);
   }
 }
 
@@ -487,10 +497,12 @@
   }
 }
 
+template <bool BAL>
 __global__ __launch_bounds__(256) void nonlin_gate_bwd_kernel(const float* __restrict__ dxs,
                                                               const float* __restrict__ u, int T,
                                                               int B, int C,
-                                                              float* __restrict__ du) {
+                                                              float* __restrict__ du,
+                                                              const float* __restrict__ coef) {
   const long n = (long)T * B * C;
   for (long i = (long)blockIdx.x * 256 + threadIdx.x; i < n; i += (long)gridDim.x * 256) {
     const int c = (int)(i % C);
@@ -499,9 +511,132 @@
     const long t = tb / B;
     const float d = dxs[((long)b * T + t) * C + c];
     const float* row = u + tb * 3 * C;
-    const float th = tanhf(row[c]);
-    du[tb * 3 * C + c] = d * row[C + c] * (1.f - th * th);
-    du[tb * 3 * C + C + c] = d * th;
+    float ds, dx;
+    na_gate_bwd(d, row[c], row[C + c], ds, dx);
+    if (BAL) ds = bal_update(ds, row[c], coef[c], coef[1024 + c]);
+    du[tb * 3 * C + c] = ds;
+    du[tb * 3 * C + C + c] = dx;
+  }
+}
+
+__device__ __forceinline__ void na_quad(unsigned w, unsigned T, unsigned B, unsigned C4, long& uq, long& zq,
+                                        unsigned& q) {
+  const unsigned tb = w / C4;
+  q = w - tb * C4;
+  const unsigned t = tb / B, b = tb - t * B;
+  uq = (long)tb * (3 * C4) + q;
+  zq = ((long)b * T + t) * C4 + q;
+}
+
+template <int U>
+__global__ __launch_bounds__(256) void nonlin_gate_fwd16_kernel(const float4* __restrict__ u, unsigned T, unsigned B,
+                                                                unsigned C4, float4* __restrict__ xs) {
+  const unsigned n = T * B * C4, step = gridDim.x * 256;
+  for (unsigned w0 = blockIdx.x * 256 + threadIdx.x; w0 < n; w0 += U * step) {
+    long zq[U];
+    float4 s[U], x[U];
+#pragma unroll
+    for (int j = 0; j < U; ++j) {
+      const unsigned w = w0 + j * step;
+      long uq;
+      unsigned q;
+      na_quad(w < n ? w : w0, T, B, C4, uq, zq[j], q);
+      s[j] = u[uq];
+      x[j] = u[uq + C4];
+    }
+#pragma unroll
+    for (int j = 0; j < U; ++j)
+      if (w0 + j * step < n)
+        xs[zq[j]] = make_float4(na_gate(s[j].x, x[j].x), na_gate(s[j].y, x[j].y), na_gate(s[j].z, x[j].z),
+                                na_gate(s[j].w, x[j].w));
+  }
+}
+
+template <int U>
+__global__ __launch_bounds__(256) void nonlin_out_fwd16_kernel(const float4* __restrict__ z, const float4* __restrict__ u,
+                                                               unsigned T, unsigned B, unsigned C4,
+                                                               float4* __restrict__ o) {
+  const unsigned n = T * B * C4, step = gridDim.x * 256;
+  for (unsigned w0 = blockIdx.x * 256 + threadIdx.x; w0 < n; w0 += U * step) {
+    float4 zv[U], y[U];
+#pragma unroll
+    for (int j = 0; j < U; ++j) {
+      const unsigned w = w0 + j * step;
+      long uq, zq;
+      unsigned q;
+      na_quad(w < n ? w : w0, T, B, C4, uq, zq, q);
+      zv[j] = z[zq];
+      y[j] = u[uq + 2 * C4];
+    }
+#pragma unroll
+    for (int j = 0; j < U; ++j)
+      if (w0 + j * step < n)
+        o[w0 + j * step] = make_float4(zv[j].x * y[j].x, zv[j].y * y[j].y, zv[j].z * y[j].z, zv[j].w * y[j].w);
+  }
+}
+
+template <int U>
+__global__ __launch_bounds__(256) void nonlin_out_bwd16_kernel(const float4* __restrict__ g, const float4* __restrict__ z,
+                                                               const float4* __restrict__ u, unsigned T, unsigned B,
+                                                               unsigned C4, float4* __restrict__ dz,
+                                                               float4* __restrict__ du) {
+  const unsigned n = T * B * C4, step = gridDim.x * 256;
+  for (unsigned w0 = blockIdx.x * 256 + threadIdx.x; w0 < n; w0 += U * step) {
+    long uq[U], zq[U];
+    float4 gv[U], zv[U], y[U];
+#pragma unroll
+    for (int j = 0; j < U; ++j) {
+      const unsigned w = w0 + j * step;
+      unsigned q;
+      na_quad(w < n ? w : w0, T, B, C4, uq[j], zq[j], q);
+      gv[j] = g[w < n ? w : w0];
+      zv[j] = z[zq[j]];
+      y[j] = u[uq[j] + 2 * C4];
+    }
+#pragma unroll
+    for (int j = 0; j < U; ++j)
+      if (w0 + j * step < n) {
+        dz[zq[j]] = make_float4(gv[j].x * y[j].x, gv[j].y * y[j].y, gv[j].z * y[j].z, gv[j].w * y[j].w);
+        du[uq[j] + 2 * C4] =
+            make_float4(gv[j].x * zv[j].x, gv[j].y * zv[j].y, gv[j].z * zv[j].z, gv[j].w * zv[j].w);
+      }
+  }
+}
+
+template <int U, bool BAL>
+__global__ __launch_bounds__(256) void nonlin_gate_bwd16_kernel(const float4* __restrict__ dxs, const float4* __restrict__ u,
+                                                                unsigned T, unsigned B, unsigned C4,
+                                                                float4* __restrict__ du, const float4* __restrict__ coef) {
+  const unsigned n = T * B * C4, step = gridDim.x * 256;
+  for (unsigned w0 = blockIdx.x * 256 + threadIdx.x; w0 < n; w0 += U * step) {
+    long uq[U];
+    float4 d[U], s[U], x[U], a[U], b[U];
+#pragma unroll
+    for (int j = 0; j < U; ++j) {
+      const unsigned w = w0 + j * step;
+      long zq;
+      unsigned q;
+      na_quad(w < n ? w : w0, T, B, C4, uq[j], zq, q);
+      d[j] = dxs[zq];
+      s[j] = u[uq[j]];
+      x[j] = u[uq[j] + C4];
+      if (BAL) {
+        a[j] = coef[q];
+        b[j] = coef[256 + q];
+      }
+    }
+#pragma unroll
+    for (int j = 0; j < U; ++j)
+      if (w0 + j * step < n) {
+        float4 ds, dx;
+        na_gate_bwd(d[j].x, s[j].x, x[j].x, ds.x, dx.x);
+        na_gate_bwd(d[j].y, s[j].y, x[j].y, ds.y, dx.y);
+        na_gate_bwd(d[j].z, s[j].z, x[j].z, ds.z, dx.z);
+        na_gate_bwd(d[j].w, s[j].w, x[j].w, ds.w, dx.w);
+        if (BAL) ds = bal_update4(ds, s[j], a[j], b[j]);
+        du[uq[j]] = ds;
+        du[uq[j] + C4] = dx;
+      }
   }
 }
 
@@ -702,10 +837,26 @@
   return 0;
 }
 
+static bool na16(int T, int B, int C, std::initializer_list<const void*> ps) {
+  uintptr_t al = 0;
+  for (const void* p : ps) al |= reinterpret_cast<uintptr_t>(p);
+  return (C & 3) == 0 && (al & 15) == 0 && (long)T * B * 3 * C < (1L << 31) &&
+         (s2t_layer_fused() & S2T_FUSED_NONLIN16) != 0;
+}
+static unsigned grid16(int T, int B, int C, int U) {
+  const long g = ((long)T * B * (C >> 2) + 256L * U - 1) / (256L * U);
+  return (unsigned)(g > 2048 ? 2048 : (g < 1 ? 1 : g));
+}
+#define NA4(p) reinterpret_cast<const float4*>(p)
+
 extern "C" int s2t_nonlin_gate_fwd(const float* u, int T, int B, int C, float* xs, void* stream) {
   if (T <= 0 || B <= 0 || C <= 0) return 0;
-  hipLaunchKernelGGL(nonlin_gate_fwd_kernel, dim3(grid1((long)T * B * C)), dim3(256), 0,
-                     (hipStream_t)stream, u, T, B, C, xs);
+  if (na16(T, B, C, {u, xs}))
+    hipLaunchKernelGGL(nonlin_gate_fwd16_kernel<4>, dim3(grid16(T, B, C, 4)), dim3(256), 0, (hipStream_t)stream,
+                       NA4(u), (unsigned)T, (unsigned)B, (unsigned)(C >> 2), reinterpret_cast<float4*>(xs));
+  else
+    hipLaunchKernelGGL(nonlin_gate_fwd_kernel, dim3(grid1((long)T * B * C)), dim3(256), 0,
+                       (hipStream_t)stream, u, T, B, C, xs);
   S2T_CHECK_LAUNCH();
   return 0;
 }
@@ -713,8 +864,12 @@
 extern "C" int s2t_nonlin_out_fwd(const float* z, const float* u, int T, int B, int C, float* o,
                                   void* stream) {
   if (T <= 0 || B <= 0 || C <= 0) return 0;
-  hipLaunchKernelGGL(nonlin_out_fwd_kernel, dim3(grid1((long)T * B * C)), dim3(256), 0,
-                     (hipStream_t)stream, z, u, T, B, C, o);
+  if (na16(T, B, C, {z, u, o}))
+    hipLaunchKernelGGL(nonlin_out_fwd16_kernel<4>, dim3(grid16(T, B, C, 4)), dim3(256), 0, (hipStream_t)stream,
+                       NA4(z), NA4(u), (unsigned)T, (unsigned)B, (unsigned)(C >> 2), reinterpret_cast<float4*>(o));
+  else
+    hipLaunchKernelGGL(nonlin_out_fwd_kernel, dim3(grid1((long)T * B * C)), dim3(256), 0,
+                       (hipStream_t)stream, z, u, T, B, C, o);
   S2T_CHECK_LAUNCH();
   return 0;
 }
@@ -722,17 +877,47 @@
 extern "C" int s2t_nonlin_out_bwd(const float* g, const float* z, const float* u, int T, int B,
                                   int C, float* dz, float* du, void* stream) {
   if (T <= 0 || B <= 0 || C <= 0) return 0;
-  hipLaunchKernelGGL(nonlin_out_bwd_kernel, dim3(grid1((long)T * B * C)), dim3(256), 0,
-                     (hipStream_t)stream, g, z, u, T, B, C, dz, du);
-  S2T_CHECK_LAUNCH();
-  return 0;
-}
+  if (na16(T, B, C, {g, z, u, dz, du}))
+    hipLaunchKernelGGL(nonlin_out_bwd16_kernel<2>, dim3(grid16(T, B, C, 2)), dim3(256), 0, (hipStream_t)stream,
+                       NA4(g), NA4(z), NA4(u), (unsigned)T, (unsigned)B, (unsigned)(C >> 2),
+                       reinterpret_cast<float4*>(dz), reinterpret_cast<float4*>(du));
+  else
+    hipLaunchKernelGGL(nonlin_out_bwd_kernel, dim3(grid1((long)T * B * C)), dim3(256), 0,
+                       (hipStream_t)stream, g, z, u, T, B, C, dz, du);
+  S2T_CHECK_LAUNCH();
+  return 0;
+}
+
+static int nonlin_gate_bwd_launch(const float* dxs, const float* u, int T, int B, int C, float* du,
+                                  const float* coef, hipStream_t st) {
+  if (T <= 0 || B <= 0 || C <= 0) return 0;
+  if (coef && C > 1024) return -1;
+  const unsigned T_ = (unsigned)T, B_ = (unsigned)B, C4 = (unsigned)(C >> 2);
+  if (na16(T, B, C, {dxs, u, du, coef})) {
+    if (coef)
+      hipLaunchKernelGGL((nonlin_gate_bwd16_kernel<2, true>), dim3(grid16(T, B, C, 2)), dim3(256), 0, st, NA4(dxs),
+                         NA4(u), T_, B_, C4, reinterpret_cast<float4*>(du), NA4(coef));
+    else
+      hipLaunchKernelGGL((nonlin_gate_bwd16_kernel<2, false>), dim3(grid16(T, B, C, 2)), dim3(256), 0, st, NA4(dxs),
+                         NA4(u), T_, B_, C4, reinterpret_cast<float4*>(du), NA4(coef));
+  } else if (coef) {
+    hipLaunchKernelGGL(nonlin_gate_bwd_kernel<true>, dim3(grid1((long)T * B * C)), dim3(256), 0, st, dxs, u, T, B, C,
+                       du, coef);
+  } else {
+    hipLaunchKernelGGL(nonlin_gate_bwd_kernel<false>, dim3(grid1((long)T * B * C)), dim3(256), 0, st, dxs, u, T, B, C,
+                       du, coef);
+  }
+  S2T_CHECK_LAUNCH();
+  return 0;
+}
+#undef NA4
 
 extern "C" int s2t_nonlin_gate_bwd(const float* dxs, const float* u, int T, int B, int C,
                                    float* du, void* stream) {
-  if (T <= 0 || B <= 0 || C <= 0) return 0;
-  hipLaunchKernelGGL(nonlin_gate_bwd_kernel, dim3(grid1((long)T * B * C)), dim3(256), 0,
-                     (hipStream_t)stream, dxs, u, T, B, C, du);
-  S2T_CHECK_LAUNCH();
-  return 0;
-}
+  return nonlin_gate_bwd_launch(dxs, u, T, B, C, du, nullptr, (hipStream_t)stream);
+}
+
+extern "C" int s2t_nonlin_gate_bwd_bal(const float* dxs, const float* u, int T, int B, int C, float* du,
+                                       const float* coef, void* stream) {
+  return nonlin_gate_bwd_launch(dxs, u, T, B, C, du, coef, (hipStream_t)stream);
+}
diff --git a/speech2text_amd/csrc/zip_layer.hip b/speech2text_amd/csrc/zip_layer.hip
--- a/speech2text_amd/csrc/zip_layer.hip
+++ b/speech2text_amd/csrc/zip_layer.hip
@@ -572,7 +572,7 @@
   e.bias = m.in.b;
   TRY(lt_matmul(c, 0, x_in, D, R, m.in, e, sv.u));
   c.s.bst[10] = c.s.bst[11] = nullptr;
-  if (dec(c, 7)) TRY(bal_stats_fwd(c, 11, sv.u, 3 * C, R, C));
+  if (dec(c, 7)) TRY(bal_stats_fwd(c, 11, sv.u, 3 * C, R, C, 4096, &m.bal));
   sv.xs = c.ar.alloc(R * C);
   RUN(s2t_nonlin_gate_fwd(sv.u, T, B, C, sv.xs, (void*)c.st));
   sv.z = c.ar.alloc(R * C);
@@ -645,7 +645,7 @@
   TRY(sa_fwd(c, 1, 19, s.x[6], &s.x[7]));
   TRY(conv_fwd(c, 1, 20, s.x[7], &s.x[8]));
   TRY(ff_fwd(c, 2, 23, s.x[8], &s.x[9]));
-  if (dec(c, 26)) TRY(bal_stats_fwd(c, 12, s.x[9], D, R, D));
+  if (dec(c, 26)) TRY(bal_stats_fwd(c, 12, s.x[9], D, R, D, 4096, &d.bal1));
   s.nscales = c.ar.alloc(R);
   s.x[10] = nullptr;
   s.x[11] = c.c.out;
@@ -813,8 +813,10 @@
   TRY(bmm(c, 2, c.s.W, dz, dxs, B, T, C, T));
   c.s.dW0 = c.ar.alloc((long)B * T * T);
   TRY(bmm(c, 0, dz, sv.xs, c.s.dW0, B, T, T, C));
-  RUN(s2t_nonlin_gate_bwd(dxs, sv.u, T, B, C, du, (void*)c.st));
-  if (fb) TRY(balancer_bwd(c, m.bal, sv.u, 3 * C, du, 3 * C, R, C, du, 3 * C, -1.0f, c.s.bst[11]));
+  const float* bcoef = fb && c.s.bst[11] && C <= 1024 && (s2t_layer_fused() & S2T_FUSED_BAL_STORE)
+                           ? c.s.bst[11] + 2048 : nullptr;
+  RUN(s2t_nonlin_gate_bwd_bal(dxs, sv.u, T, B, C, du, bcoef, (void*)c.st));
+  if (fb && !bcoef) TRY(balancer_bwd(c, m.bal, sv.u, 3 * C, du, 3 * C, R, C, du, 3 * C, -1.0f, c.s.bst[11]));
   if (fw1) {
     float* gc = c.ar.alloc(R * C);
     TRY(copy2d(c, gc, C, du + C, 3 * C, C, R));
@@ -861,13 +863,24 @@
     float* acc = c.c.layer_acc;
     float* d0 = c.ar.alloc(R * D);
     float* g9w = c.ar.alloc(R * D);
-    RUN(s2t_norm_bypass_bwd(s.x[9], d.norm_bias.x, s.nscales, s.x[0], d.byp.x, g, s.fm_fused ? c.c.fm : nullptr, B,
-                            R, D, g9w, d0, acc, acc + 2 * D, acc + 3 * D, (void*)c.st));
+    bool shaped = false;
+    if (dec(c, 26) && s.bst[12] && !c.dry && (s2t_layer_fused() & S2T_FUSED_BAL_STORE)) {
+      const int rc = s2t_norm_bypass_bwd_bal(s.x[9], d.norm_bias.x, s.nscales, s.x[0], d.byp.x, g,
+                                             s.fm_fused ? c.c.fm : nullptr, B, R, D, g9w, d0, acc, acc + 2 * D,
+                                             acc + 3 * D, s.bst[12] + 2048, (void*)c.st);
+      if (rc != 0 && rc != -2) return fail(rc, "s2t_norm_bypass_bwd_bal");
+      shaped = rc == 0;
+    }
+    if (!shaped)
+      RUN(s2t_norm_bypass_bwd(s.x[9], d.norm_bias.x, s.nscales, s.x[0], d.byp.x, g, s.fm_fused ? c.c.fm : nullptr, B,
+                              R, D, g9w, d0, acc, acc + 2 * D, acc + 3 * D, (void*)c.st));
     const float* g9 = g9w;
     if (dec(c, 26)) {
       float* o = c.ar.alloc(R * D);
-      TRY(balancer_bwd(c, d.bal1, s.x[9], D, g9, D, R, D, o, D, -1.0f, s.bst[12]));
-      g9 = o;
+      if (!shaped) {
+        TRY(balancer_bwd(c, d.bal1, s.x[9], D, g9, D, R, D, o, D, -1.0f, s.bst[12]));
+        g9 = o;
+      }
     }
     const float *g8, *g7, *g6, *g4, *g3, *g2, *g1, *g0;
     TRY(ff_bwd(c, 2, 23, s.x[8], g9, &g8));
```

After: 18430 audio-seconds/sec. About the same (-0.0%).
